# andrei-ace/EdgeStyle

Hardware: AMD Instinct MI355X
Metric: 512x512 try-on images/sec @ 50 DDIM steps (6-cond ControlNet) (higher is better)
Workload: dtype f16; 1 GPU; BASELINE configs[1]: full 6-cond edgestyle_multicontrolnet + controllora, 512x512, 50 DDIM steps, CFG 7.5, batch=1/GPU, hipGraph-captured step, cond embedding + VAE decode included; images_per_gpu=1, ddim_steps=50, parallelism=dp1 (independent images, one RCCL gather)

## Files before the change

### edgestyle_amd/csrc/builder.hip

```cpp
#include <hip/hip_runtime.h>
#include <math.h>
#include <stdio.h>
#include <stdlib.h>
#include <string.h>

#include <algorithm>
#include <deque>
#include <functional>
#include <map>
#include <memory>
#include <stdexcept>
#include <string>
#include <thread>
#include <unordered_map>
#include <vector>

#include "../../include/edgestyle_hip.h"
#include "plan.h"

extern "C" void es_set_error(const char* msg);
extern "C" int es_plan_set_dry(int on);

namespace {

// ... 175 lines not shown
  ~Blk() { if (heap) heap->release(off, bytes); }
};

struct T {
  unsigned long long p = 0;
  int n = 0, h = 0, w = 0, c = 0;
  long long ld = 0;
  int es = 2;
  std::shared_ptr<Blk> b;
  unsigned long long lo = 0;
  std::shared_ptr<Blk> lo_b;
  unsigned long long gnp = 0;
  std::shared_ptr<Blk> gnp_b;
  int gnp_groups = 0;
  explicit operator bool() const { return p != 0; }
  long long hw() const { return (long long)h * w; }
  long long numel() const { return (long long)n * h * w * c; }
  bool contig() const { return ld == c; }
  long long bstride() const { return hw() * ld; }
  size_t bytes() const { return (size_t)numel() * es; }
  T batch(int a, int cnt = -1) const {
    T t = *this;
    t.p += (unsigned long long)a * (unsigned long long)bstride() * es;
    if (t.lo) t.lo += (unsigned long long)a * (unsigned long long)bstride() * es;
    t.gnp = 0; t.gnp_b.reset(); t.gnp_groups = 0;
    t.n = cnt < 0 ? n - a : cnt;
    if (a < 0 || t.n < 0 || a + t.n > n) fail("builder: batch slice out of range");
    return t;
  }
  T chan(int c0, int cn) const {
    T t = *this;
    if (c0 < 0 || c0 + cn > c) fail("builder: channel slice out of range");
    t.p += (unsigned long long)c0 * es;
    t.lo = 0; t.lo_b.reset();
    t.gnp = 0; t.gnp_b.reset(); t.gnp_groups = 0;
    t.c = cn;
    return t;
  }
  T view(int n2, int h2, int w2, int c2) const {
    if (!contig() || (long long)n2 * h2 * w2 * c2 != numel()) fail("builder: view of a non-contiguous or differently sized tensor");
    T t = *this;
    t.n = n2; t.h = h2; t.w = w2; t.c = c2; t.ld = c2;
    return t;
  }
  void* ptr() const { return (void*)p; }
};

struct PW {
  unsigned long long w = 0, bias = 0, ln_colsum = 0;
  int cout = 0, cin = 0, ksize = 1, bn = 128, rows_padded = 0, kpad = 0, ctail = 0, korder = 0;
  bool geglu = false;
  float ln_eps = 1e-5f;
  const uint16_t* host_w = nullptr;
  long long w_numel() const { return (long long)rows_padded * kpad; }
};
using PWs = std::vector<const PW*>;
struct Norm { unsigned long long g = 0, b = 0; };

struct CA {
  int stride = 1, pad = -1;
  bool upsample = false;
  T x2, temb, residual, out, out_scale_dev;
  long long temb_stride = 0;
  int act = ES_ACT_NONE;
  float out_scale = 1.f;
  int out_h = 0, out_w = 0;
  std::vector<int> group_n;
  std::vector<T> tails;
  int x_rep = 1;
  bool wide = false;
  int gn_groups = 0;
};

#pragma clang fp contract(off)
constexpr double PLAN_T160 = 1.25, PLAN_ALONE = 0.9, PLAN_TFIX = 2.0, PLAN_RED_FIX = 12.0, PLAN_SLAB_BYTES_PER_UNIT = 4.0e6;
constexpr double PLAN_T320 = 2.3, PLAN_T320_FIX = 3.0;
constexpr double PLAN_T256 = 2.6, PLAN_T256_FIX = 6.0, PLAN_T256_GEGLU = 7.0, PLAN_LN_TK = 1.55, PLAN_T256_MARGIN = 0.93;
constexpr int PLAN_BIG_MIN_M = 2048, PLAN_BIG_MIN_NK = 16;
constexpr double PLAN_T64_ALONE = 0.5, PLAN_T64 = 0.16, PLAN_T64_LONG = 1.5;
constexpr int PLAN_SMALL_MAX_M = 16384, PLAN_MIN_SLICE = 12, PLAN_NK_NOSPLIT = 10, PLAN_RESIDENT = 512;

double plan_env(const char* name, double dflt) { const char* e = getenv(name); return e && *e ? atof(e) : dflt; }
bool plan_gemm(long long M, int rows_padded, int kpad, bool geglu, const int* bns, int nb, bool allow_split, int* o_bn, int* o_sk, int* o_st) {
  static const double PLAN_T320 = plan_env("ES_PLAN_T320", ::PLAN_T320), PLAN_T256_MARGIN = plan_env("ES_PLAN_T256_MARGIN", ::PLAN_T256_MARGIN);
  static const int PLAN_BIG_MIN_NK = (int)plan_env("ES_PLAN_BIG_MIN_NK", ::PLAN_BIG_MIN_NK);
  int others[8], no = 0;
  bool has256 = false;
  for (int bi = 0; bi < nb; ++bi) { if (bns[bi] == 256) has256 = true; else if (no < 8) others[no++] = bns[bi]; }
  if (has256) {
    const int nk = kpad / BK;
    int obn = 0, osk = 1, ost = 2;
    const bool have_other = no > 0 && plan_gemm(M, rows_padded, kpad, geglu, others, no, allow_split, &obn, &osk, &ost);
    if (rows_padded % 256) { if (!have_other) return false; *o_bn = obn; *o_sk = osk; *o_st = ost; return true; }
    const long long t256 = ((M + 255) / 256) * (rows_padded / 256);
    const double c256 = (double)((t256 + 255) / 256) * ((double)nk * PLAN_T256 + PLAN_T256_FIX + (geglu ? PLAN_T256_GEGLU : 0.0));
    bool take = !have_other;
    if (have_other && M >= PLAN_BIG_MIN_M && nk >= PLAN_BIG_MIN_NK && osk == 1 && obn != 64) {
      const long long to = ((M + BM - 1) / BM) * (rows_padded / obn);
      const double co = (double)((to + PLAN_RESIDENT - 1) / PLAN_RESIDENT) * ((double)nk * PLAN_LN_TK * (obn == 160 ? PLAN_T160 : 1.0) + PLAN_T256_FIX);
      take = c256 < PLAN_T256_MARGIN * co;
    }
    if (take) { *o_bn = 256; *o_sk = 1; *o_st = 2; } else { *o_bn = obn; *o_sk = osk; *o_st = ost; }
    return true;
  }
  if (geglu) { *o_bn = 128; *o_sk = 1; *o_st = 2; return true; }
  const int nk = kpad / BK;
  bool have = false;
  double bt = 0; int bbn = 0, bsk = 0; long long bwgs = 0;
  for (int bi = 0; bi < nb; ++bi) {
    const int bn = bns[bi];
    if (rows_padded % bn) continue;
    if (bn == 320 && (M < PLAN_BIG_MIN_M || nk < PLAN_BIG_MIN_NK) && nb > 1) continue;
    if (bn == 64 && M > PLAN_SMALL_MAX_M && nb > 1) continue;
    const int bm = bn == 320 ? 256 : (bn == 64 ? 64 : BM);
    const int resident = bn == 320 ? PLAN_RESIDENT / 2 : (bn == 64 ? 2 * PLAN_RESIDENT : PLAN_RESIDENT);
    const long long tiles = ((M + bm - 1) / bm) * (rows_padded / bn);
    int last = 1;
    if (allow_split && tiles < resident / 2 && nk > PLAN_NK_NOSPLIT) last = std::max(1, std::min(nk / PLAN_MIN_SLICE, 32));
    for (int sk = 1; sk <= last; ++sk) {
      const long long wgs = tiles * sk;
      double tk;
      if (bn == 320) tk = PLAN_T320;
      else if (bn == 64) {
        if (sk > 1 && wgs > PLAN_RESIDENT) continue;
        const double w = (double)wgs / (double)(PLAN_RESIDENT / 2);
        const double ex = std::max(0.0, w - 1.0);
        tk = (PLAN_T64_ALONE + PLAN_T64 * (ex * ex)) * (nk <= 40 ? 1.0 : PLAN_T64_LONG);
      } else tk = (bn == 160 ? PLAN_T160 : 1.0) * (wgs <= PLAN_RESIDENT / 2 ? PLAN_ALONE : 1.0);
      const double rounds = bn == 320 ? std::max((double)wgs / 256.0, 0.9) : (double)((wgs + resident - 1) / resident);
      double t = rounds * (((double)nk / (double)sk) * tk + (bn == 320 ? PLAN_T320_FIX : PLAN_TFIX));
      if (sk > 1) t += PLAN_RED_FIX + (double)sk * (double)M * (double)rows_padded * 8.0 / PLAN_SLAB_BYTES_PER_UNIT;
      if (!have || t < bt) { have = true; bt = t; bbn = bn; bsk = sk; bwgs = wgs; }
    }
  }
  if (!have) return false;
  *o_bn = bbn; *o_sk = bsk;
  if (bbn == 64) *o_st = (bwgs <= PLAN_RESIDENT && nk / bsk >= 6) ? 4 : 2;
  else *o_st = (bbn != 320 && bwgs <= PLAN_RESIDENT / 2 && nk / bsk >= 6) ? 4 : 2;
  return true;
}

constexpr int XS_TARGET_WGS = 256, XS_MIN_M = 8192;
bool xs_shape_fits(int ksize, int kpad, int cin, int ctail, int cout, bool geglu) {
  if (ksize != 1 || (kpad != 320 && kpad != 640) || cin != kpad || ctail) return false;
  const int ch = kpad == 320 ? 64 : 32;
  const int line = ch * (128 / (geglu ? ch : 2 * ch));
  return !(cout % line || cout < 4 * line);
}
bool xs_shape_ok(long long M, int ksize, int kpad, int cin, int ctail, int cout, bool geglu) {
  if (!xs_shape_fits(ksize, kpad, cin, ctail, cout, geglu)) return false;
  if (M < XS_MIN_M || (M < 4 * XS_MIN_M && cout < (kpad == 320 ? 960 : 1920))) return false;
  return true;
}
bool gn_fold_on() { static const bool on = [] { const char* e = getenv("ES_GN_FOLD"); return !e || std::string(e) == "1"; }(); return on; }
int choose_bn(int cout) { return (cout % 160 == 0 && cout % 128 != 0) ? 160 : 128; }
bool big_tile_256() { static const bool on = [] { const char* e = getenv("ES_BIG_TILE_256"); return !e || e[0] != '0'; }(); return on; }

struct Builder {
  Heap heap;
  unsigned long long ws_bytes = 0;
  int dt = ES_F16;
  std::vector<std::pair<unsigned long long, std::vector<char>>> uploads;
  std::deque<PW> pws;
  std::map<std::string, const PW*> pack_cache;
  std::map<const void*, unsigned long long> vec_cache;
  std::map<std::pair<int, int>, unsigned long long> gn_partials, fusion_scratch;
  std::map<int, unsigned long long> zero_bias;

  T empty(int n, int h, int w, int c, int es = 2) {
    T t; t.n = n; t.h = h; t.w = w; t.c = c; t.ld = c; t.es = es;
    auto blk = std::make_shared<Blk>();
    blk->heap = &heap; blk->bytes = std::max<size_t>(t.bytes(), 1); blk->off = heap.alloc(blk->bytes);
    t.b = blk; t.p = FAKE_HEAP + blk->off;
    return t;
  }
  unsigned long long persistent(size_t bytes) { return FAKE_HEAP + heap.alloc(std::max<size_t>(bytes, 1)); }
  T persistent_t(int n, int h, int w, int c, int es = 2) {
    T t; t.n = n; t.h = h; t.w = w; t.c = c; t.ld = c; t.es = es;
    t.p = persistent(t.bytes());
    return t;
  }
  char* staged(unsigned long long addr, size_t bytes) {
    uploads.emplace_back(addr, std::vector<char>(bytes, 0));
    return uploads.back().second.data();
  }
  unsigned long long upload_f32(const std::vector<float>& v) {
    const unsigned long long a = persistent(v.size() * 4);
    memcpy(staged(a, v.size() * 4), v.data(), v.size() * 4);
    return a;
  }
  unsigned long long workspace(unsigned long long bytes) { ws_bytes = std::max(ws_bytes, bytes); return FAKE_WS; }
// ... 60 lines not shown
    }
    return &p;
  }
  const PW* pack_ln(const std::vector<float>& w, int rows, int C, const std::vector<float>* bias, const std::vector<float>& gamma, const std::vector<float>& beta,
                    float eps, bool geglu) {
    std::vector<float> wg((size_t)rows * C), fb((size_t)rows);
    parallel_for(rows, [&](long long a, long long b) {
      for (long long r = a; r < b; ++r) {
        double acc = 0.0;
        for (int j = 0; j < C; ++j) { wg[r * C + j] = w[r * C + j] * gamma[j]; acc += (double)w[r * C + j] * (double)beta[j]; }
        if (bias) acc += (double)(*bias)[r];
        fb[r] = (float)acc;
      }
    });
    PW* p = const_cast<PW*>(pack(wg, rows, C, 1, &fb, geglu));
    const uint16_t* pk = p->host_w;
    std::vector<float> cs((size_t)p->rows_padded);
    for (int r = 0; r < p->rows_padded; ++r) {
      double acc = 0.0;
      for (int j = 0; j < p->kpad; ++j) acc += (double)dec(pk[(size_t)r * p->kpad + j]);
      cs[r] = (float)acc;
    }
    p->ln_colsum = upload_f32(cs);
    p->ln_eps = eps;
    return p;
  }
  unsigned long long norm_vec(const Weights& W, const std::string& key, long long n) {
    const es_tensor* id = nullptr;
    std::vector<float> v = W.vec(key, n, &id);
    auto it = vec_cache.find(id->data);
    if (it != vec_cache.end()) return it->second;
    return vec_cache[id->data] = upload_f32(v);
  }
  Norm norm(const Weights& W, const std::string& p, long long n) { return {norm_vec(W, p + ".weight", n), norm_vec(W, p + ".bias", n)}; }

  const PW* conv(const Weights& W, const std::string& p, int cin_pad = 0, bool geglu = false, int cout_pad = 0) {
    const es_tensor* wt = W.get(p + ".weight");
    if (wt->ndim != 2 && wt->ndim != 4) fail("es_load_weights: '" + p + ".weight' is neither a Linear nor a Conv2d weight");
    const int cout = (int)wt->shape[0], cin = (int)wt->shape[1], k = wt->ndim == 4 ? (int)wt->shape[2] : 1;
    if (wt->ndim == 4 && (wt->shape[3] != k || (k != 1 && k != 3))) fail("es_load_weights: '" + p + ".weight': only 1x1 and 3x3 kernels");
    const es_tensor* bt = W.find(p + ".bias");
    std::string key;
    if (!W.lora(p)) {
      char buf[128];
      snprintf(buf, sizeof(buf), "%p|%p|%d|%d|%d", wt->data, bt ? bt->data : nullptr, (int)geglu, cin_pad, cout_pad);
      key = buf;
      auto it = pack_cache.find(key);
      if (it != pack_cache.end()) return it->second;
    }
    std::vector<float> w = W.matrix(p), b;
    if (bt) b = W.vec(p + ".bias", cout);
    const PW* pw = pack(w, cout, cin, k, bt ? &b : nullptr, geglu, cin_pad, cout_pad);
    if (!key.empty()) pack_cache[key] = pw;
    return pw;
  }
  void stack(const Weights& W, const std::vector<std::string>& ps, bool bias, std::vector<float>& w, std::vector<float>& b, int& rows, int& cols) {
    rows = 0; cols = -1;
    for (const auto& p : ps) {
      const es_tensor* t = W.get(p + ".weight");
      if (t->ndim != 2 || (cols >= 0 && t->shape[1] != cols)) fail("es_load_weights: '" + p + ".weight' does not stack with its neighbours");
      cols = (int)t->shape[1];
      std::vector<float> m = W.matrix(p);
      w.insert(w.end(), m.begin(), m.end());
      if (bias) { std::vector<float> v = W.vec(p + ".bias", t->shape[0]); b.insert(b.end(), v.begin(), v.end()); }
      rows += (int)t->shape[0];
    }
  }
  const PW* cat(const Weights& W, const std::vector<std::string>& ps, bool bias) {
    std::vector<float> w, b; int rows, cols;
    stack(W, ps, bias, w, b, rows, cols);
    return pack(w, rows, cols, 1, bias ? &b : nullptr);
  }
  const PW* cat_ln(const Weights& W, const std::vector<std::string>& ps, bool bias, const std::string& ln, bool geglu = false) {
    std::vector<float> w, b; int rows, cols;
    stack(W, ps, bias, w, b, rows, cols);
    return pack_ln(w, rows, cols, bias ? &b : nullptr, W.vec(ln + ".weight", cols), W.vec(ln + ".bias", cols), 1e-5f, geglu);
  }
  const PW* conv_tail(const Weights& W, const std::string& p, const std::string& pt) {
    const es_tensor* wt = W.get(p + ".weight");
    const es_tensor* tt = W.get(pt + ".weight");
    char buf[96];
    snprintf(buf, sizeof(buf), "%p|%p|tail", wt->data, tt->data);
    auto it = pack_cache.find(buf);
    if (it != pack_cache.end()) return it->second;
    const int cout = (int)wt->shape[0], cin = (int)wt->shape[1], k = (int)wt->shape[2], ct = (int)tt->shape[1];
    if (wt->ndim != 4 || cin % BK || ct % BK || tt->shape[0] != cout) fail("es_load_weights: conv2 + conv_shortcut fold needs 64-aligned channels ('" + p + "')");
    std::vector<float> w = W.matrix(p), tw = W.matrix(pt), b = W.vec(p + ".bias", cout), b2 = W.vec(pt + ".bias", cout);
    for (int i = 0; i < cout; ++i) b[i] = b[i] + b2[i];
    const PW* pw = pack(w, cout, cin, k, &b, false, 0, 0, &tw, ct);
    pack_cache[buf] = pw;
    return pw;
  }

  static void ok(int rc, const char* what) { if (rc) fail(std::string(what) + ": " + es_last_error()); }

  struct GnFront { unsigned long long part = 0; std::vector<Norm> nl; int groups = 0, nchunk = 0, hw = 0; float eps = 0.f; };
  T linear_xs(const T& x, const PWs& pl, long long M, const T& out, const std::vector<long long>& group_rows, const T& residual = T(),
              const GnFront* gn = nullptr) {
    const PW* pw = pl[0];
    const int K = pw->kpad, ch = K == 320 ? 64 : 32;
    const int pline = 128 / (pw->geglu ? ch : 2 * ch);
    const int total = pw->cout / ch, lines = total / pline;
    const long long rbs = (M + 255) / 256;
    const int want = (int)std::max<long long>(1, std::min<long long>(lines, XS_TARGET_WGS / rbs));
    const int lps = cdiv(lines, want), nslices = cdiv(lines, lps);
    es_xs_desc d;
// ... 32 lines not shown

  T conv_gemm(const T& x, const PWs& pl, const CA& a = CA()) {
    const PW* pw = pl[0];
    const bool grouped = pl.size() > 1;
    int N = x.n;
    const int H = x.h, Wd = x.w, C1 = x.c, nsrc = x.n;
    if (!x.contig()) fail("conv_gemm: the source must be contiguous");
    if (a.x_rep > 1) { if (a.x2 || !a.tails.empty()) fail("conv_gemm: x_rep needs a single source"); N *= a.x_rep; }
    const int C2 = a.x2 ? a.x2.c : 0;
    if (C1 + C2 != pw->cin) fail("conv_gemm: input channels " + std::to_string(C1) + "+" + std::to_string(C2) + " != packed " + std::to_string(pw->cin));
    int tsum = 0;
    for (const auto& t : a.tails) tsum += t.c;
    if (tsum != pw->ctail || a.tails.size() > 2) fail("conv_gemm: tail channels do not match the packed weights");
    const int k = pw->ksize, pad = a.pad < 0 ? (k == 3 ? 1 : 0) : a.pad;
    const int Hin = a.upsample ? H * 2 : H, Win = a.upsample ? Wd * 2 : Wd;
    const int Hout = a.out_h ? a.out_h : (Hin + 2 * pad - k) / a.stride + 1, Wout = a.out_w ? a.out_w : (Win + 2 * pad - k) / a.stride + 1;
    const int act_i = pw->geglu ? ES_ACT_GEGLU : a.act;
    const int cstore = pw->geglu ? pw->cout / 2 : pw->cout;
    T out = a.out ? a.out : empty(N, Hout, Wout, cstore);
    if (out.numel() != (long long)N * Hout * Wout * cstore || !out.contig()) fail("conv_gemm: output buffer of another size");
    const long long M = (long long)N * Hout * Wout, hw = (long long)Hout * Wout;
    static const bool xs_residual = [] { const char* e = getenv("ES_XS_RESIDUAL"); return !e || std::string(e) == "1"; }();
    const bool xs_res = !a.residual || (xs_residual && pw->kpad == 320 && !pw->geglu && !pw->ln_colsum && a.residual.contig() &&
                                        a.residual.numel() == (long long)N * Hout * Wout * cstore && !(a.wide && wide_stream()));
    const bool plain = k == 1 && a.stride == 1 && !a.upsample && !a.x2 && !a.temb && xs_res && a.tails.empty() && a.x_rep == 1 &&
                       a.act == ES_ACT_NONE && a.out_scale == 1.f && !a.out_scale_dev;
    if (plain && xs_shape_ok(M, pw->ksize, pw->kpad, pw->cin, pw->ctail, pw->cout, pw->geglu)) {
      bool e = true;
      if (grouped) {
        if (pl.size() > 4) e = false;
        for (int n : a.group_n) if ((n * hw) % 256) e = false;
        for (const PW* q : pl) if ((q->ln_colsum == 0) != (pw->ln_colsum == 0)) e = false;
      }
      if (e) {
        std::vector<long long> rows;
        for (int n : a.group_n) rows.push_back(n * hw);
        T xo = out;
        linear_xs(x, grouped ? pl : PWs{pw}, M, xo, rows, a.residual);
        return out;
      }
    }
    bool big_ok = C1 % BK == 0 && C2 % BK == 0 && !pw->geglu && !pw->ln_colsum;
    if (big_ok && grouped) for (int n : a.group_n) if ((n * hw) % 256) big_ok = false;
    bool ln256_ok = big_tile_256() && (pw->geglu || pw->ln_colsum) && k == 1 && a.stride == 1 && !a.upsample && !a.x2 && a.tails.empty() && !a.temb &&
                    a.x_rep == 1 && C1 % BK == 0 && pw->rows_padded % 256 == 0 && pw->cout % 8 == 0 && !(pw->geglu && a.residual) && !a.wide && a.gn_groups == 0;
    if (ln256_ok && grouped) for (int n : a.group_n) if ((n * hw) % 256) ln256_ok = false;
    const bool small_ok = C1 % BK == 0 && C2 % BK == 0 && !pw->geglu;
    int cand[5], nc = 0;
    if (ln256_ok) cand[nc++] = 256;
    if (big_ok) cand[nc++] = 320;
    cand[nc++] = 160; cand[nc++] = 128;
    if (small_ok) cand[nc++] = 64;
    int bn, splitk, stages;
    if (!plan_gemm(M, pw->rows_padded, pw->kpad, pw->geglu, cand, nc, pw->ln_colsum == 0, &bn, &splitk, &stages)) fail("plan_gemm: rows_padded fits no N tile");
    if (bn == 320 && splitk == 1 && !es_conv_gemm8p_form_ok(act_i, pw->cout, a.temb ? 1 : 0, hw, a.residual ? 1 : 0)) {
      if (!plan_gemm(M, pw->rows_padded, pw->kpad, pw->geglu, cand + 1, nc - 1, pw->ln_colsum == 0, &bn, &splitk, &stages)) fail("plan_gemm: rows_padded fits no N tile");
    }
    es_gemm_desc d;
    memset(&d, 0, sizeof(d));
    d.x = x.ptr(); d.x2 = a.x2 ? a.x2.ptr() : nullptr; d.w = (const void*)pw->w; d.bias = (const float*)pw->bias;
    d.temb = a.temb ? a.temb.ptr() : nullptr; d.residual = a.residual ? a.residual.ptr() : nullptr;
    d.out_scale_dev = a.out_scale_dev ? (const float*)a.out_scale_dev.ptr() : nullptr; d.out = out.ptr();
    d.N = N; d.Hsrc = H; d.Wsrc = Wd; d.C1 = C1; d.C2 = C2; d.Hout = Hout; d.Wout = Wout; d.Cout = pw->cout;
    d.rows_padded = pw->rows_padded; d.Kpad = pw->kpad; d.ksize = k; d.stride = a.stride; d.pad = pad; d.upsample = a.upsample;
    d.temb_stride = a.temb ? (int)a.temb_stride : 0;
    d.act = act_i; d.splitk = splitk; d.bn = bn; d.dtype = dt; d.out_scale = a.out_scale; d.stages = stages;
    const long long src_numel = x.numel() * a.x_rep + (a.x2 ? a.x2.numel() : 0);
    d.xcd_m_fastest = (!grouped && splitk == 1 && M <= 2048 && pw->w_numel() > src_numel) ? 1 : 0;
    d.x_nmod = a.x_rep > 1 ? nsrc : 0;
    d.korder = pw->korder;
    if (a.gn_groups > 0 && gn_handover(hw, cstore, a.gn_groups) && !pw->geglu && !pw->ln_colsum && pw->cout / a.gn_groups <= (bn == 320 ? 160 : bn)) {
      T part = empty(N, (int)(2 * (hw / 64)), 1, a.gn_groups * 2, 4);
      d.gn_part = (float*)part.ptr(); d.gn_groups = a.gn_groups;
      out.gnp = part.p; out.gnp_b = part.b; out.gnp_groups = a.gn_groups;
    }
    if (a.wide && a.residual && wide_stream() && cstore % 8 == 0 && !pw->geglu) {
      if (a.residual.lo) d.residual_lo = (const void*)a.residual.lo;
      T lo = empty(N, Hout, Wout, cstore);
      d.out_lo = lo.ptr();
      out.lo = lo.p; out.lo_b = lo.b;
    }
    if (k == 1 && M <= 65536 && C1 % BK == 0 && C2 % BK == 0 && bn != 64 && bn != 320 && bn != 256 && !(stages == 4 && bn != 128) && stages != 3) d.waves = 8;
    if (splitk > 1) d.workspace = (float*)workspace((unsigned long long)splitk * M * pw->rows_padded * 4);
    if (pw->ln_colsum) {
      for (const PW* q : pl) if (!q->ln_colsum) fail("LayerNorm-folded weights need a plain linear launch (all groups folded)");
      if (a.x2 || k != 1) fail("LayerNorm-folded weights need a plain linear launch");
      d.ln_colsum = (const float*)pw->ln_colsum; d.ln_eps = pw->ln_eps;
    }
    if (!a.tails.empty()) {
      for (const auto& t : a.tails) if (t.n != N || t.h != Hout || t.w != Wout || !t.contig()) fail("conv_gemm: tail sources must be contiguous [N,Hout,Wout,C]");
      d.t1 = a.tails[0].ptr(); d.Ct1 = a.tails[0].c;
      if (a.tails.size() == 2) { d.t2 = a.tails[1].ptr(); d.Ct2 = a.tails[1].c; }
    }
    if (grouped) {
      const int gran = bn == 320 ? 256 : BM;
      int sum = 0;
      for (int n : a.group_n) { sum += n; if ((n * hw) % gran) fail("grouped conv_gemm: groups must cover N in whole tiles"); }
      if (pl.size() > 4 || a.group_n.size() != pl.size() || sum != N) fail("grouped conv_gemm: bad group table");
      d.ngroups = (int)pl.size();
      long long acc = 0;
      for (size_t g = 0; g < pl.size(); ++g) {
        const PW* q = pl[g];
        if (q->rows_padded != pw->rows_padded || q->kpad != pw->kpad || q->cout != pw->cout || q->cin != pw->cin || q->ksize != pw->ksize ||
            q->geglu != pw->geglu || q->ctail != pw->ctail || q->korder != pw->korder) fail("grouped conv_gemm: weight geometry differs between groups");
        acc += a.group_n[g] * hw / BM;
        d.mt_end[g] = (int)acc; d.w_g[g] = (const void*)q->w; d.bias_g[g] = (const float*)q->bias; d.ln_colsum_g[g] = (const float*)q->ln_colsum;
// ... 223 lines not shown
    conv_in = B.conv(W, "conv_in", in_pad);
    t1 = B.conv(W, "time_embedding.linear_1"); t2 = B.conv(W, "time_embedding.linear_2");
    std::vector<std::string> names;
    for (int i = 0; i < c.nb; ++i) for (int j = 0; j < c.lpb; ++j) names.push_back("down_blocks." + std::to_string(i) + ".resnets." + std::to_string(j));
    names.push_back("mid_block.resnets.0"); names.push_back("mid_block.resnets.1");
    names.insert(names.end(), extra_resnets.begin(), extra_resnets.end());
    int o = 0;
    std::vector<std::string> tp;
    for (const auto& nm : names) { temb_offs[nm] = o; o += (int)W.shaped(nm + ".time_emb_proj.weight", {-1, 4 * c.ch[0]})->shape[0]; tp.push_back(nm + ".time_emb_proj"); }
    tproj = B.cat(W, tp, true);
    for (int i = 0; i < c.nb; ++i) {
      down.emplace_back();
      for (int j = 0; j < c.lpb; ++j) {
        const std::string r = "down_blocks." + std::to_string(i) + ".resnets." + std::to_string(j);
        int ti = -1;
        Resnet rs(B, W, r, c.groups, c.eps, temb_offs[r]);
        if (c.has_attn[i]) { tr.emplace_back(B, W, "down_blocks." + std::to_string(i) + ".attentions." + std::to_string(j), c.heads, c.groups); ti = (int)tr.size() - 1; }
        down.back().emplace_back(rs, ti);
      }
      downsample.push_back(i != c.nb - 1 ? B.conv(W, "down_blocks." + std::to_string(i) + ".downsamplers.0.conv") : nullptr);
    }
    mid0 = Resnet(B, W, "mid_block.resnets.0", c.groups, c.eps, temb_offs["mid_block.resnets.0"]);
    tr.emplace_back(B, W, "mid_block.attentions.0", c.heads, c.groups); mid_attn = (int)tr.size() - 1;
    mid1 = Resnet(B, W, "mid_block.resnets.1", c.groups, c.eps, temb_offs["mid_block.resnets.1"]);
    n_enc_tr = (int)tr.size();
  }
  int tproj_width() const { return tproj->cout; }
  T time_proj(Builder& B, const T& t, int n) const {
    T e = B.timestep_embedding(t, n, cfg.ch[0]);
    CA s; s.act = ES_ACT_SILU;
    e = B.linear(e, t1, s);
    e = B.linear(e, t2, s);
    return B.linear(e, tproj);
  }
};

struct UNet : Encoder {
  std::vector<std::vector<std::pair<Resnet, int>>> up;
  std::vector<const PW*> upsample;
  Norm norm_out; const PW* conv_out;
  void init(Builder& B, const Weights& W, const UCfg& c) {
    std::vector<std::string> extra;
    for (int i = 0; i < c.nb; ++i) for (int j = 0; j < c.lpb + 1; ++j) extra.push_back("up_blocks." + std::to_string(i) + ".resnets." + std::to_string(j));
    Encoder::init(B, W, c, extra);
    for (int i = 0; i < c.nb; ++i) {
      up.emplace_back();
      for (int j = 0; j < c.lpb + 1; ++j) {
        const std::string r = "up_blocks." + std::to_string(i) + ".resnets." + std::to_string(j);
        int ti = -1;
        Resnet rs(B, W, r, c.groups, c.eps, temb_offs[r]);
        if (c.has_attn[c.nb - 1 - i]) { tr.emplace_back(B, W, "up_blocks." + std::to_string(i) + ".attentions." + std::to_string(j), c.heads, c.groups); ti = (int)tr.size() - 1; }
        up.back().emplace_back(rs, ti);
      }
      upsample.push_back(i != c.nb - 1 ? B.conv(W, "up_blocks." + std::to_string(i) + ".upsamplers.0.conv") : nullptr);
    }
    W.shaped("conv_out.weight", {c.out_ch, c.ch[0], 3, 3});
    norm_out = B.norm(W, "conv_norm_out", c.ch[0]);
    conv_out = B.conv(W, "conv_out");
  }
};

struct ControlNet : Encoder {
  std::vector<const PW*> zero; const PW* zero_mid = nullptr;
  std::vector<const PW*> cond;
  bool uses_vae = false;
  void init(Builder& B, const Weights& W, const UCfg& c, bool uses_vae_) {
    Encoder::init(B, W, c, {});
    uses_vae = uses_vae_;
    std::vector<int> rc{c.ch[0]};
    for (int i = 0; i < c.nb; ++i) { for (int j = 0; j < c.lpb; ++j) rc.push_back(c.ch[i]); if (i != c.nb - 1) rc.push_back(c.ch[i]); }
    for (size_t i = 0; i < rc.size(); ++i) {
      W.shaped("controlnet_down_blocks." + std::to_string(i) + ".weight", {rc[i], rc[i], 1, 1});
      zero.push_back(B.conv(W, "controlnet_down_blocks." + std::to_string(i)));
    }
    W.shaped("controlnet_mid_block.weight", {c.ch[c.nb - 1], c.ch[c.nb - 1], 1, 1});
    zero_mid = B.conv(W, "controlnet_mid_block");
    if (!uses_vae) {
      const std::string p = "controlnet_cond_embedding";
      W.shaped(p + ".conv_in.weight", {c.ce[0], c.cond_ch, 3, 3});
      W.shaped(p + ".conv_out.weight", {c.ch[0], c.ce[c.nce - 1], 3, 3});
      cond.push_back(B.conv(W, p + ".conv_in", 8));
      for (int i = 0; i < 2 * (c.nce - 1); ++i) cond.push_back(B.conv(W, p + ".blocks." + std::to_string(i)));
      cond.push_back(B.conv(W, p + ".conv_out"));
    }
  }
  T embed_cond(Builder& B, const T& img) const {
    CA s; s.act = ES_ACT_SILU;
    T h = B.conv_gemm(img, cond[0], s);
    for (size_t i = 1; i + 1 < cond.size(); ++i) { CA a; a.act = ES_ACT_SILU; a.stride = ((i - 1) % 2 == 1) ? 2 : 1; h = B.conv_gemm(h, cond[i], a); }
    return B.conv_gemm(h, cond.back());
  }
};

struct FusionParams { unsigned long long w1, b1, g1, be1, w2, b2, g2, be2, w3, b3; int c, s; };

struct VAE {
  VCfg cfg; int lat_pad = 8;
  struct Mid { Resnet r0, r1; Norm gn; const PW *qkv, *o; };
  const PW *e_in, *e_out, *quant, *post_quant_scaled, *d_in, *d_out;
  std::vector<std::pair<std::vector<Resnet>, const PW*>> e_down, d_up;
  Mid e_mid, d_mid; Norm e_norm, d_norm;
  Mid mid(Builder& B, const Weights& W, const std::string& side) {
    const std::string a = side + ".mid_block.attentions.0";
    const int c = cfg.ch[cfg.nb - 1];
    Mid m;
    m.r0 = Resnet(B, W, side + ".mid_block.resnets.0", cfg.groups, cfg.eps, -1);
    m.gn = B.norm(W, a + ".group_norm", c);
    m.qkv = B.cat(W, {a + ".to_q", a + ".to_k", a + ".to_v"}, true);
    m.o = B.conv(W, a + ".to_out.0");
    m.r1 = Resnet(B, W, side + ".mid_block.resnets.1", cfg.groups, cfg.eps, -1);
    return m;
  }
  void init(Builder& B, const Weights& W, const VCfg& c) {
    cfg = c;
    lat_pad = round_up(c.latent, 8);
    const int n = c.nb;
    W.shaped("encoder.conv_in.weight", {c.ch[0], 3, 3, 3}); W.shaped("encoder.conv_out.weight", {2 * c.latent, c.ch[n - 1], 3, 3});
    W.shaped("quant_conv.weight", {2 * c.latent, 2 * c.latent, 1, 1}); W.shaped("post_quant_conv.weight", {c.latent, c.latent, 1, 1});
    W.shaped("decoder.conv_in.weight", {c.ch[n - 1], c.latent, 3, 3}); W.shaped("decoder.conv_out.weight", {3, c.ch[0], 3, 3});
    for (const char* side : {"encoder", "decoder"})
      for (const char* q : {".to_q", ".to_k", ".to_v", ".to_out.0"}) W.shaped(std::string(side) + ".mid_block.attentions.0" + q + ".weight", {c.ch[n - 1], c.ch[n - 1]});
    e_in = B.conv(W, "encoder.conv_in", 8);
    for (int i = 0; i < n; ++i) {
      std::vector<Resnet> rs;
      for (int j = 0; j < c.lpb; ++j) rs.emplace_back(B, W, "encoder.down_blocks." + std::to_string(i) + ".resnets." + std::to_string(j), c.groups, c.eps, -1);
      e_down.emplace_back(rs, i != n - 1 ? B.conv(W, "encoder.down_blocks." + std::to_string(i) + ".downsamplers.0.conv") : nullptr);
    }
    e_mid = mid(B, W, "encoder");
    e_norm = B.norm(W, "encoder.conv_norm_out", c.ch[n - 1]);
    e_out = B.conv(W, "encoder.conv_out");
    quant = B.conv(W, "quant_conv");
    {
      const es_tensor* wt = W.get("post_quant_conv.weight");
      std::vector<float> w = W.matrix("post_quant_conv"), b;
      for (auto& v : w) v = (float)((double)v / (double)c.scaling);
      const bool hb = W.has("post_quant_conv.bias");
      if (hb) b = W.vec("post_quant_conv.bias", wt->shape[0]);
      post_quant_scaled = B.pack(w, (int)wt->shape[0], (int)wt->shape[1], 1, hb ? &b : nullptr, false, lat_pad, 8);
    }
    d_in = B.conv(W, "decoder.conv_in", 8);
    d_mid = mid(B, W, "decoder");
    for (int i = 0; i < n; ++i) {
      std::vector<Resnet> rs;
      for (int j = 0; j < c.lpb + 1; ++j) rs.emplace_back(B, W, "decoder.up_blocks." + std::to_string(i) + ".resnets." + std::to_string(j), c.groups, c.eps, -1);
      d_up.emplace_back(rs, i != n - 1 ? B.conv(W, "decoder.up_blocks." + std::to_string(i) + ".upsamplers.0.conv") : nullptr);
    }
    d_norm = B.norm(W, "decoder.conv_norm_out", c.ch[0]);
    d_out = B.conv(W, "decoder.conv_out");
  }
  T run_mid(Builder& B, const Mid& m, T h) const {
    h = m.r0.run(B, h, T());
    const int N = h.n, H = h.h, Wd = h.w, C = h.c;
    T n = B.group_norm(h, m.gn, cfg.groups, cfg.eps, false).view(N, H * Wd, 1, C);
    T qkv = B.linear(n, m.qkv);
    T a = B.attention(qkv.chan(0, C), qkv.chan(C, C), qkv.chan(2 * C, C), 1);
    CA r; r.residual = h.view(N, H * Wd, 1, C);
    h = B.linear(a, m.o, r).view(N, H, Wd, C);
    return m.r1.run(B, h, T());
  }
  T encode_moments(Builder& B, const T& img) const {
    T h = B.conv_gemm(img, e_in);
    for (const auto& blk : e_down) {
      for (const auto& r : blk.first) h = r.run(B, h, T());
      if (blk.second) { CA a; a.stride = 2; a.pad = 0; a.out_h = h.h / 2; a.out_w = h.w / 2; h = B.conv_gemm(h, blk.second, a); }
    }
    h = run_mid(B, e_mid, h);
    h = B.group_norm(h, e_norm, cfg.groups, cfg.eps, true);
    h = B.conv_gemm(h, e_out);
    return B.conv_gemm(h, quant);
  }
  T decode(Builder& B, const T& z) const {
    T h = B.conv_gemm(z, post_quant_scaled);
    h = B.conv_gemm(h, d_in);
    h = run_mid(B, d_mid, h);
    for (const auto& blk : d_up) {
      for (const auto& r : blk.first) h = r.run(B, h, T());
      if (blk.second) { CA a; a.upsample = true; h = B.conv_gemm(h, blk.second, a); }
    }
    h = B.group_norm(h, d_norm, cfg.groups, cfg.eps, true);
    return B.conv_gemm(h, d_out);
  }
};

struct Model {
  Builder B;
  UCfg ucfg; VCfg vcfg;
  es_ctx_geometry geo;
  Dict d_unet, d_vae, d_fusion, d_cn[6];
  UNet unet;
  VAE vae;
  std::vector<std::unique_ptr<ControlNet>> nets;
  std::vector<int> net_of_cond;
  std::vector<std::pair<int, std::vector<int>>> groups;
  std::vector<FusionParams> fusion;
  std::vector<std::pair<int, int>> table;
  std::vector<const Encoder*> encs; std::vector<int> counts; int ntot = 0, width = 0, ncn = 0;
  int B_ = 1, N = 2, T_ = 50, h = 64, w = 64, nn = 6, kmax = 3;
  T latents, model_in, noise, ehs, step_idx, t_rows, scales_cur, t_table, scale_table, coef, ts_dev, image;
  std::vector<T> conds, cond_img, cond_noise, gbufs, hist;
  std::vector<T> ctx_grouped, ctx_unet; std::vector<std::vector<T>> ctx_nets;
  T cond_cat, tproj_table, tproj_cur, tproj_gen;
  std::vector<T> fused_zero, fz_zero, fz_u;
  bool guess = false;
  int Bc = 2;
  std::vector<std::vector<T>> ctx_guess;

  std::vector<Norm> norms(const std::vector<const Resnet*>& rs, int which) const { std::vector<Norm> v; for (auto r : rs) v.push_back(which == 1 ? r->n1 : r->n2); return v; }

  T g_resnet(const std::vector<const Resnet*>& rs, const T& x, const T& tproj) {
    const Resnet* r0 = rs[0];
    T hh = B.group_norm(x, norms(rs, 1), r0->groups, r0->eps, true, T(), counts);
    PWs c1, c2, c2s, sh; bool all_s = true;
    for (auto r : rs) { c1.push_back(r->conv1); c2.push_back(r->conv2); c2s.push_back(r->conv2s); sh.push_back(r->shortc); if (!r->conv2s) all_s = false; }
    CA a; a.temb = tproj.chan(r0->temb_off, tproj.c - r0->temb_off); a.temb_stride = tproj.ld; a.group_n = counts; a.gn_groups = r0->groups;
    hh = B.conv_gemm(hh, c1, a);
    hh = B.group_norm(hh, norms(rs, 2), r0->groups, r0->eps, true, T(), counts);
    if (all_s) { CA t; t.tails.push_back(x); t.group_n = counts; t.gn_groups = r0->groups; return B.conv_gemm(hh, c2s, t); }
    for (auto r : rs) if (r->conv2s) fail("builder: grouped resnets must fold conv_shortcut all alike");
    T xs = x;
    if (r0->shortc) { CA s; s.group_n = counts; xs = B.conv_gemm(x, sh, s); }
    CA r; r.residual = xs; r.group_n = counts; r.wide = true; r.gn_groups = r0->groups;
    return B.conv_gemm(hh, c2, r);
  }
  T g_transformer(const std::vector<const Transformer*>& ts, const T& x, const T& kv) {
    const Transformer* t0 = ts[0];
    const int Nn = x.n, H = x.h, Wd = x.w, C = x.c;
    std::vector<int> rows;
    for (int n : counts) rows.push_back(n * H * Wd);
    std::vector<Norm> nl; PWs pin, qkv, o1, q2, o2, ff1, ffo;
    for (auto t : ts) { nl.push_back(t->norm); pin.push_back(t->proj_in); qkv.push_back(t->qkv_ln); o1.push_back(t->o1); q2.push_back(t->q2_ln); o2.push_back(t->o2); ff1.push_back(t->ff1_ln); ffo.push_back(t->ffo); }
// ... 121 lines not shown
    const int c0 = unet.conv_in->cout;
    T h0 = B.empty(ntot, x.h, x.w, c0);
    {
      PWs ci; for (auto e : encs) ci.push_back(e->conv_in);
      CA a; a.residual = cond_cat; a.group_n = counts; a.out = h0; a.x_rep = ntot / N; a.wide = true; a.gn_groups = ucfg.groups;
      h0 = B.conv_gemm(x, ci, a);
    }
    T tproj;
    if (table_driven) {
      B.gather_row(tproj_table, T_, step_idx, tproj_cur, (int)((long long)ntot * width * 2 / 4));
      tproj = tproj_cur;
    } else tproj = time_proj_generic();
    std::vector<T> skips; T mid;
    g_run(h0, tproj, skips, mid);
    h0 = T();
    std::vector<T> srcs = skips; srcs.push_back(mid);
    std::vector<T> enc;
    for (const auto& s : srcs) enc.push_back(s.batch(ncn));
    std::vector<T> fused;
    if (nn == 1) {
      const ControlNet* cn = (const ControlNet*)encs[0];
      for (size_t lvl = 0; lvl < srcs.size(); ++lvl) {
        CA a; a.residual = enc[lvl]; a.out_scale = 1.f; a.out_scale_dev = scales_cur.chan(0, 1);
        fused.push_back(B.conv_gemm(srcs[lvl].batch(0, ncn), lvl + 1 < srcs.size() ? cn->zero[lvl] : cn->zero_mid, a));
      }
    } else {
    std::vector<int> cn_counts(counts.begin(), counts.end() - 1);
    std::vector<T> res;
    for (size_t lvl = 0; lvl < srcs.size(); ++lvl) {
      PWs z; for (size_t e = 0; e + 1 < encs.size(); ++e) { const ControlNet* cn = (const ControlNet*)encs[e]; z.push_back(lvl + 1 < srcs.size() ? cn->zero[lvl] : cn->zero_mid); }
      CA a; a.group_n = cn_counts;
      res.push_back(B.conv_gemm(srcs[lvl].batch(0, ncn), z, a));
    }
    std::vector<int> first(nn, 0);
    { int a = 0; for (const auto& g : groups) for (int p : g.second) { first[p] = a; a += N; } }
    std::vector<std::vector<T>> rpn(nn);
    for (int i = 0; i < nn; ++i) for (size_t k = 0; k < srcs.size(); ++k) rpn[i].push_back(res[k].batch(first[i]));
    fused = fuse(rpn, N, &enc);
    }
    srcs.clear(); skips.clear(); enc.clear(); mid = T();
    unet_decoder(fused, tproj.batch(ncn));
  }
  void unet_decoder(std::vector<T>& fused, const T& tp) {
    T hh = fused.back();
    fused.pop_back();
    int ci = unet.n_enc_tr;
    for (size_t i = 0; i < unet.up.size(); ++i) {
      for (const auto& ra : unet.up[i]) {
        T skip = fused.back();
        fused.pop_back();
        hh = ra.first.run(B, hh, tp, skip);
        if (ra.second >= 0) { hh = transformer(unet.tr[ra.second], hh, ctx_unet[ci]); ++ci; }
      }
      if (unet.upsample[i]) { CA a; a.upsample = true; hh = B.conv_gemm(hh, unet.upsample[i], a); }
    }
    hh = B.group_norm(hh, unet.norm_out, ucfg.groups, ucfg.eps, true);
    CA o; o.out = noise;
    B.conv_gemm(hh, unet.conv_out, o);
  }
  void enc_run(const Encoder& e, T hh, const T& tp, const std::vector<T>& ctx, std::vector<T>& skips, T& mid) {
    skips.push_back(hh);
    int ci = 0;
    for (size_t i = 0; i < e.down.size(); ++i) {
      for (size_t j = 0; j < e.down[i].size(); ++j) {
        hh = e.down[i][j].first.run(B, hh, tp);
        if (e.down[i][j].second >= 0) { hh = transformer(e.tr[e.down[i][j].second], hh, ctx[ci]); ++ci; }
        skips.push_back(hh);
      }
      if (e.downsample[i]) { CA a; a.stride = 2; a.gn_groups = ucfg.groups; hh = B.conv_gemm(hh, e.downsample[i], a); skips.push_back(hh); }
    }
    hh = e.mid0.run(B, hh, tp);
    hh = transformer(e.tr[e.mid_attn], hh, ctx[ci]);
    mid = e.mid1.run(B, hh, tp);
  }
  void set_context_guess() {
    for (size_t ti = 0; ti < unet.tr.size(); ++ti) unet.tr[ti].context(B, ehs, ctx_unet[ti], 1);
    const T ehs_c = ehs.batch(N - Bc);
    size_t gi = 0;
    for (const auto& g : groups) {
      const ControlNet& net = *nets[g.first];
      for (int ti = 0; ti < net.n_enc_tr; ++ti) net.tr[ti].context(B, ehs_c, ctx_guess[gi][ti], (int)g.second.size());
      ++gi;
    }
  }
  static std::vector<float> guess_level_scales(int n) {
    std::vector<float> ls((size_t)n);
    const double step = (0.0 - (-1.0)) / (double)(n - 1);
    for (int i = 0; i < n; ++i) ls[i] = (float)(i < n / 2 ? pow(10.0, -1.0 + step * (double)i) : pow(10.0, 0.0 - step * (double)(n - i - 1)));
    return ls;
  }
  void step_guess() {
    const T& x = model_in;
    const int Bh = N - Bc;
    const T xc = x.batch(Bh);
    const std::vector<float> ls = guess_level_scales((int)table.size());
    std::vector<std::vector<T>> rpn(nn);
    size_t gi = 0;
    for (const auto& g : groups) {
      const ControlNet& cn = *nets[g.first];
      const int k = (int)g.second.size();
      T tp = cn.time_proj(B, t_rows, k * Bc);
      const int c0 = cn.conv_in->cout;
      T h0 = B.empty(k * Bc, x.h, x.w, c0);
      for (int i = 0; i < k; ++i) { CA a; a.residual = conds[g.second[i]]; a.out = h0.batch(i * Bc, Bc); B.conv_gemm(xc, cn.conv_in, a); }
      std::vector<T> skips; T mid;
      enc_run(cn, h0, tp, ctx_guess[gi], skips, mid);
      std::vector<T> res;
// ... 66 lines not shown
          B.memcpy_t(conds[i], B.conv_gemm(z, net.conv_in));
        }
      } else {
        T emb = nets[g.net]->embed_cond(B, x8);
        for (size_t k = 0; k < g.idx.size(); ++k) {
          const int i = g.idx[k];
          T e = emb.batch((int)k * B_, B_);
          B.memcpy_t(conds[i].batch(0, B_), e);
          if (rep > 1) B.memcpy_t(conds[i].batch(B_, B_), e);
        }
      }
    }
  }

  void pack_fusion(const Weights& W) {
    for (size_t i = 0; i < table.size(); ++i) {
      const std::string p = i + 1 < table.size() ? "multi_controlnet_down_blocks." + std::to_string(i) : "multi_controlnet_mid_block";
      const int c = table[i].first, s = table[i].second, hw = s * s;
      FusionParams f; f.c = c; f.s = s;
      f.w1 = B.upload_f32(to_f32(W.shaped(p + ".first_conv.weight", {3 * c, 2, 1, 1})));
      f.b1 = B.upload_f32(to_f32(W.shaped(p + ".first_conv.bias", {3 * c})));
      f.w2 = B.upload_f32(to_f32(W.shaped(p + ".second_conv.weight", {c, 3, 1, 1})));
      f.b2 = B.upload_f32(to_f32(W.shaped(p + ".second_conv.bias", {c})));
      f.w3 = B.upload_f32(to_f32(W.shaped(p + ".third_conv.weight", {c, 1, 1, 1})));
      f.b3 = B.upload_f32(to_f32(W.shaped(p + ".third_conv.bias", {c})));
      auto plane = [&](const std::string& key, int per) {
        const std::vector<float> t = to_f32(W.shaped(key, {(long long)per * c, s, s}));
        const unsigned long long a = B.persistent((size_t)hw * c * per * 2);
        uint16_t* d = (uint16_t*)B.staged(a, (size_t)hw * c * per * 2);
        parallel_for(hw, [&](long long x0, long long x1) {
          for (long long px = x0; px < x1; ++px)
            for (int cc = 0; cc < c * per; ++cc) d[(size_t)px * c * per + cc] = B.enc(t[(size_t)cc * hw + px]);
        });
        return a;
      };
      f.g1 = plane(p + ".first_normalization.weight", 3); f.be1 = plane(p + ".first_normalization.bias", 3);
      f.g2 = plane(p + ".second_normalization.weight", 1); f.be2 = plane(p + ".second_normalization.bias", 1);
      fusion.push_back(f);
    }
  }
};

struct Recording {
  es_plan* p;
  explicit Recording(es_plan* pl) : p(pl) { if (es_plan_begin_record(p)) fail(std::string("es_load_weights: ") + es_last_error()); es_plan_set_dry(1); }
  ~Recording() { es_plan_set_dry(0); es_plan_end_record(p); }
};

}

extern "C" int es_plan_gemm_choice(long long M, int rows_padded, int kpad, int geglu, const int* bns, int n_bns, int allow_split, int* bn, int* splitk, int* stages) {
  if (!bns || n_bns < 1 || !bn || !splitk || !stages) { es_set_error("es_plan_gemm_choice: null argument"); return -1; }
  if (!plan_gemm(M, rows_padded, kpad, geglu != 0, bns, n_bns, allow_split != 0, bn, splitk, stages)) { es_set_error("es_plan_gemm_choice: rows_padded fits no N tile"); return -1; }
  return 0;
}
extern "C" int es_linear_xs_eligible(long long M, int ksize, int kpad, int cin, int ctail, int cout, int geglu) {
  return xs_shape_ok(M, ksize, kpad, cin, ctail, cout, geglu != 0) ? 1 : 0;
}

extern "C" int es_load_weights(const es_weights* wts, const es_model_config* mc, const es_ctx_geometry* g, int device, es_ctx** out) {
  if (!wts || !mc || !g || !out) { es_set_error("es_load_weights: null argument"); return -1; }
  es_ctx* ctx = nullptr;
  es_plan* plans[ES_PLAN_COUNT] = {};
  void* arena = nullptr;
  try {
    auto m = std::make_unique<Model>();
    Model& M = *m;
    Builder& B = M.B;
    if (mc->n_blocks < 2 || mc->n_blocks > 4 || mc->vae_n_blocks < 2 || mc->vae_n_blocks > 4) fail("es_load_weights: 2..4 resolution levels");
    if (g->n_conds != 6 && g->n_conds != 1) fail("es_load_weights: n_conds is 6 (the reference's fused multi-ControlNet model, MC:66-114) or 1 (a single ControlNet, PL:338-351)");
    if (g->n_conds == 1 && wts->n_controlnets != 1) fail("es_load_weights: a single-ControlNet context takes exactly one ControlNet");
    if (g->dtype != ES_F16 && g->dtype != ES_BF16) fail("es_load_weights: dtype must be ES_F16 or ES_BF16");
    if (g->B < 1 || g->h < 1 || g->w < 1 || g->n_steps < 1) fail("es_load_weights: bad geometry");
    if (wts->n_controlnets < 1 || wts->n_controlnets > 6) fail("es_load_weights: 1..6 distinct ControlNets");
    UCfg& u = M.ucfg;
    u.in_ch = mc->in_channels; u.out_ch = mc->out_channels; u.nb = mc->n_blocks; u.lpb = mc->layers_per_block; u.heads = mc->num_heads;
    u.cross = mc->cross_attention_dim; u.groups = mc->norm_num_groups; u.eps = mc->norm_eps; u.nce = mc->n_cond_embed; u.cond_ch = mc->conditioning_channels;
    for (int i = 0; i < 4; ++i) { u.ch[i] = mc->block_out_channels[i]; u.has_attn[i] = mc->down_has_attn[i]; u.ce[i] = mc->cond_embed_channels[i]; }
    VCfg& v = M.vcfg;
    v.nb = mc->vae_n_blocks; v.lpb = mc->vae_layers_per_block; v.latent = mc->vae_latent_channels; v.groups = mc->vae_norm_num_groups;
    v.eps = mc->vae_norm_eps; v.scaling = mc->vae_scaling_factor;
    for (int i = 0; i < 4; ++i) v.ch[i] = mc->vae_block_out_channels[i];
    if (u.in_ch != v.latent) fail("es_load_weights: the UNet's in_channels must equal the VAE's latent_channels");
    if (u.cond_ch != 3 || u.nce < 2 || u.nce > 4) fail("es_load_weights: conditioning embedding of 3 input channels, 2..4 widths");
    M.geo = *g;
    B.dt = g->dtype;
    M.B_ = g->B; M.N = g->cfg ? 2 * g->B : g->B; M.T_ = g->n_steps; M.h = g->h; M.w = g->w; M.nn = g->n_conds;
    M.guess = g->guess_mode != 0;
    M.Bc = M.guess ? g->B : M.N;
    const int N = M.N, TS = M.T_, h = g->h, w = g->w, Bn = g->B, NN = g->n_conds, Nc = M.Bc;
    if (!M.guess) {
      int cnt[6] = {};
      for (int p = 0; p < NN; ++p) {
        const int ni = wts->net_of_cond[p];
        if (ni < 0 || ni >= wts->n_controlnets) fail("es_load_weights: net_of_cond names a ControlNet that was not given");
        ++cnt[ni];
      }
      const int hw_min = (h >> (u.nb - 1)) * (w >> (u.nb - 1));
      for (int i = 0; i <= wts->n_controlnets; ++i) {
        const long long n = (i < wts->n_controlnets ? (long long)cnt[i] : 1) * N;
        if (n && (n * hw_min) % BM) fail("es_load_weights: the groups of the lockstep pass do not tile in 128-pixel units at this latent size (the Python host falls back to serial chains; this builder does not)");
      }
    }
    M.d_unet.init(wts->unet, "UNet"); M.d_vae.init(wts->vae, "VAE"); M.d_fusion.init(wts->fusion, "fusion");
    for (int i = 0; i < wts->n_controlnets; ++i) M.d_cn[i].init(wts->controlnet[i], ("ControlNet " + std::to_string(i)).c_str());
    Weights Wu; Wu.own = &M.d_unet; Wu.who = "UNet";
// ... 203 lines not shown
```

### edgestyle_amd/csrc/gemm_conv.hip

```cpp
#ifndef ES_WT_STORES
#define ES_WT_STORES 1
#endif
#include "common.h"
#include "../../include/edgestyle_hip.h"
#include "plan.h"

#ifndef ES_W_AUX
#define ES_W_AUX 0
#endif

int es_conv_gemm8p_launch(const es_gemm_desc& d, hipStream_t st);
bool es_conv_gemm8p_takes(const es_gemm_desc& d);

unsigned long long es_operand_limit_v = 0x7FFFFFFFull;

namespace {

constexpr int BK = 64;

#ifndef ES_ABLATE
#define ES_ABLATE 0
#endif
#ifndef ES_STAMPS
#define ES_STAMPS 0
#endif

typedef __attribute__((address_space(3))) void* lptr_t;

template <typename T>
ES_DEVICE void store_elems(T* o, const float* v, int n) {
  for (int r = 0; r < n; ++r) o[r] = from_f32<T>(v[r]);
}

template <int XI>
ES_DEVICE void row_offsets_fn(unsigned (&voff)[XI], const int (&iy0)[XI], const int (&ix0)[XI], const int (&nb)[XI],
                              const int tp, const int cs, const int chan, const int ksize, const int KK, const int pad,
                              const int Hin, const int Win, const int upsample, const int Wsrc) {
  int ky = 0, kx = 0;
  if (ksize == 3) { ky = (tp * 11) >> 5; kx = tp - ky * 3; }
  if (tp >= KK) { ky = pad; kx = pad; }
#pragma unroll
  for (int i = 0; i < XI; ++i) {
    const int iy = iy0[i] + ky, ix = ix0[i] + kx;
    const bool ok = (unsigned)iy < (unsigned)Hin && (unsigned)ix < (unsigned)Win;
    const int pix = nb[i] + (iy >> upsample) * Wsrc + (ix >> upsample);
    voff[i] = ok ? (unsigned)(((size_t)pix * cs + chan) * 2) : 0xFFFFFF00u;
  }
}

template <typename T, int BM, int BN, bool ALIGNED, int STAGES, int FM = 4 ,
          bool LN = false ,
          bool KO = false >
__global__ __launch_bounds__(BM * 8 / FM, (STAGES == 2 && BM == 128) ? (FM == 2 ? 4 : 2) : 1) void conv_gemm_kernel(
    const es_gemm_desc p, const int M, const int nk, const void* const tail1, const void* const tail2, const int tailC1,
    const int tailC2) {
  constexpr int BKT = BK;
  constexpr int RB = BKT * 2;
  constexpr int CPR = BKT / 8;
  constexpr int RPP = 1024 / RB;
  constexpr int WM = BM / (16 * FM);
  constexpr int NW = WM * 2;
  constexpr int NT = NW * 64;
  constexpr int XI = (BM / RPP) / NW;
  constexpr int FN = BN / 32;
  constexpr int WP = BN / RPP;
  constexpr int WI = (WP + NW - 1) / NW;
  constexpr int XT = BM * RB;
  constexpr int WT = BN * RB;
  static_assert((size_t)BM * (BN * 2 + 16) <= (size_t)STAGES * (BM + BN) * RB, "the epilogue tile must fit the stage ring");
  static_assert(LN || (size_t)BM * (BN * 2 + 16) + (size_t)(BM / 8 + BM / 64) * BN * 8 <= (size_t)STAGES * (BM + BN) * RB,
                "the GroupNorm-statistics scratch (gn_emit_partials) must fit behind the epilogue tile");
  constexpr int BNP = BN;
  constexpr int EROW = BNP * 2 + 16;
  constexpr int NI = XI + WI;
  extern __shared__ __attribute__((aligned(16))) char smem[];

  const int tid = threadIdx.x;
  const int lane = tid & 63;
  const int wave = __builtin_amdgcn_readfirstlane(tid >> 6);
  const int wm = wave % WM, wn = wave / WM;
  int tile_m, tile_n, z;
  {
    const int tm = (M + BM - 1) / BM, tn = p.rows_padded / BN;
    const int nwg = gridDim.x, b = blockIdx.x;
    const int q = nwg >> 3, r = nwg & 7, xcd = b & 7;
    const int w = (xcd < r ? xcd * (q + 1) : r * (q + 1) + (xcd - r) * q) + (b >> 3);
    const float inv_tm = __builtin_amdgcn_rcpf((float)tm), inv_tn = __builtin_amdgcn_rcpf((float)tn);
    if (p.xcd_m_fastest) { const int t = fast_div(w, tm, inv_tm); tile_m = w - t * tm; z = fast_div(t, tn, inv_tn); tile_n = t - z * tn; }
    else                 { const int t = fast_div(w, tn, inv_tn); tile_n = w - t * tn; z = fast_div(t, tm, inv_tm); tile_m = t - z * tm; }
  }
#if ES_STAMPS
  const int sblk = blockIdx.x == 40 ? 0 : (blockIdx.x == 333 ? 1 : -1);
  auto stamp = [&](int ks, int what) __attribute__((always_inline)) {
    if (p.prof && sblk >= 0 && lane == 0 && wave < 4 && ks >= 8 && ks < 16)
      p.prof[((sblk * 4 + wave) * 8 + (ks - 8)) * 4 + what] = __builtin_amdgcn_s_memtime();
  };
  auto pstamp = [&](int what) __attribute__((always_inline)) {
    if (p.prof && tid == 0 && (blockIdx.x == 0 || blockIdx.x == gridDim.x - 1))
      p.prof[256 + (blockIdx.x == 0 ? 0 : 1) * 8 + what] = __builtin_amdgcn_s_memtime();
  };
  pstamp(0);
#else
  if (p.prof && tid == 0) atomicMin(p.prof, (unsigned long long)__builtin_amdgcn_s_memrealtime());
#endif

  int ks0 = 0, ks1 = nk;
  if (p.splitk > 1) {
    const float inv_sk = __builtin_amdgcn_rcpf((float)p.splitk);
    ks0 = fast_div(nk * z, p.splitk, inv_sk);
    ks1 = fast_div(nk * (z + 1), p.splitk, inv_sk);
  }

  const int lrow = lane / CPR;
  const int lslot = lane % CPR;
  const int kc = lslot ^ (lrow & 7);
  const int Ctot = p.C1 + p.C2;
  const int KK = p.ksize * p.ksize;
  const int pC1 = p.C1, pC2 = p.C2, pCt1 = tailC1, pCt2 = tailC2;
  const bool has_tail = tail1 != nullptr;
  const int Ctail = has_tail ? pCt1 + pCt2 : 0;
  const int Ktrue = KK * Ctot + Ctail;
  const int Hin = p.Hsrc << p.upsample, Win = p.Wsrc << p.upsample;
  const int HWout = p.Hout * p.Wout;

  constexpr unsigned OOB = 0xFFFFFF00u;
  int iy0[XI], ix0[XI], nb[XI];
  const bool small_m = M < (1 << 24);
  const float inv_hw = __builtin_amdgcn_rcpf((float)HWout), inv_w = __builtin_amdgcn_rcpf((float)p.Wout);
#pragma unroll
  for (int i = 0; i < XI; ++i) {
    const int m = tile_m * BM + RPP * (wave * XI + i) + lrow;
    iy0[i] = -(1 << 20); ix0[i] = -(1 << 20); nb[i] = 0;
    if (m < M) {
      int n, oy, ox;
      if (HWout == 1) {
        n = m; oy = 0; ox = 0;
      } else if (small_m) {
        n = fast_div(m, HWout, inv_hw);
        const int rem = m - n * HWout;
        oy = fast_div(rem, p.Wout, inv_w);
        ox = rem - oy * p.Wout;
      } else {
        n = m / HWout;
        const int rem = m - n * HWout;
        oy = rem / p.Wout; ox = rem - oy * p.Wout;
      }
      iy0[i] = oy * p.stride - p.pad;
      ix0[i] = ox * p.stride - p.pad;
      if (p.x_nmod) n -= (n / p.x_nmod) * p.x_nmod;
      nb[i] = n * p.Hsrc * p.Wsrc;
    }
  }
  int pix0[KO ? XI : 1];
  unsigned tmask[KO ? XI : 1];
  if constexpr (KO) {
#pragma unroll
    for (int i = 0; i < XI; ++i) {
      const int ay = iy0[i], ax = ix0[i];
      unsigned vy = 0, vx = 0;
#pragma unroll
      for (int k = 0; k < 3; ++k) {
        vy |= ((unsigned)(ay + k) < (unsigned)Hin ? 1u : 0u) << k;
        vx |= ((unsigned)(ax + k) < (unsigned)Win ? 1u : 0u) << k;
      }
      unsigned mk = ((vy & 1) ? vx : 0u) | ((vy & 2) ? vx << 3 : 0u) | ((vy & 4) ? vx << 6 : 0u);
      mk |= ay > -(1 << 19) ? 1u << 9 : 0u;
      mk |= (unsigned)(ay & p.upsample) << 10 | (unsigned)(ax & p.upsample) << 11;
      tmask[i] = mk;
      pix0[i] = nb[i] + (ay >> p.upsample) * p.Wsrc + (ax >> p.upsample);
    }
  }
  int grp = 0;
  if (p.ngroups > 1) {
    const int t128 = (tile_m * BM) / 128;
    grp = (t128 >= p.mt_end[0]) + (t128 >= p.mt_end[1]) + (t128 >= p.mt_end[2]);
  }
  const void* wsel = p.ngroups > 1 ? p.w_g[grp] : p.w;
  const float* bsel = p.ngroups > 1 ? p.bias_g[grp] : p.bias;
  const float* lnsel = LN ? (p.ngroups > 1 ? p.ln_colsum_g[grp] : p.ln_colsum) : nullptr;
  const auto rW = __builtin_amdgcn_make_buffer_rsrc(
      (void*)wsel, (short)0, (int)((size_t)p.rows_padded * p.Kpad * 2), 0x00020000);
  const int Nsrc = p.x_nmod ? p.x_nmod : p.N;
  const auto rX1 = __builtin_amdgcn_make_buffer_rsrc(
      (void*)p.x, (short)0, (int)((size_t)Nsrc * p.Hsrc * p.Wsrc * p.C1 * 2), 0x00020000);
  const void* const pt1 = tail1 ? tail1 : p.x;
  const void* const pt2 = tail2 ? tail2 : p.x;
  const void* const px = p.x;
  const void* const px2 = p.x2 ? p.x2 : p.x;
  const int nX1 = (int)((size_t)Nsrc * p.Hsrc * p.Wsrc * pC1 * 2);
  const int nX2 = (int)((size_t)Nsrc * p.Hsrc * p.Wsrc * (p.x2 ? pC2 : pC1) * 2);
  const int nT1 = has_tail ? (int)((size_t)p.N * p.Hout * p.Wout * pCt1 * 2) : 0;
  const int nT2 = tail2 ? (int)((size_t)p.N * p.Hout * p.Wout * pCt2 * 2) : 0;
  unsigned woff[WI];
#pragma unroll
  for (int i = 0; i < WI; ++i) {
    const int piece = wave * WI + i;
    woff[i] = piece < WP ? (unsigned)(((size_t)(tile_n * BN + RPP * piece + lrow) * p.Kpad + kc * 8) * 2) : OOB;
  }

  int tap, cpos;
  {
    const int kg = ks0 * BKT + (ALIGNED ? 0 : kc * 8);
    tap = kg == 0 ? 0 : fast_div(kg, Ctot, __builtin_amdgcn_rcpf((float)Ctot));
    cpos = kg - tap * Ctot;
    if (ALIGNED && tap >= KK) { tap = KK; cpos = kg - KK * Ctot; }
    if constexpr (KO) {
      const int kt = (KK * Ctot) / BKT;
      if (ks0 >= kt) { tap = KK; cpos = (ks0 - kt) * BKT; }
      else { const int ch = fast_div(ks0, 9, 1.0f / 9.0f); tap = ks0 - ch * 9; cpos = ch * BKT; }
    }
  }
  unsigned voff[XI];
#pragma unroll
  for (int i = 0; i < XI; ++i) voff[i] = OOB;
  const void* xbase = p.x;
  int xrec = 0, soff_x = 0, seg_left = 0;
  const int ks_tail = (KK * Ctot) / BKT;
  const int pk_ksize = p.ksize, pk_pad = p.pad, pk_up = p.upsample, pk_wsrc = p.Wsrc;
#define row_offsets(tp, cs, chan) \
  row_offsets_fn<XI>(voff, iy0, ix0, nb, (tp), (cs), (chan), pk_ksize, KK, pk_pad, Hin, Win, pk_up, pk_wsrc)
  auto issue_tile = [&](int ks, int stage) __attribute__((always_inline)) {
    char* xs = smem + stage * (XT + WT);
    char* ws = xs + XT;
    const int soff_w = ks * RB;
#pragma unroll
    for (int i = 0; i < WI; ++i)
      if (!(ES_ABLATE & 32) && wave * WI + i < WP)
        __builtin_amdgcn_raw_ptr_buffer_load_lds(rW, (lptr_t)(ws + (wave * WI + i) * 1024), 16,
                                                 (ES_ABLATE & 64) ? (int)OOB : (int)woff[i], soff_w, 0, ES_W_AUX);
    if constexpr ((ES_ABLATE & 16) != 0) {
    } else if constexpr (ALIGNED) {
      bool fast = false;
      if constexpr (!KO) fast = seg_left > 0;
      if (fast) {
        soff_x += 128; --seg_left;
      } else {
      const bool tail = KO ? ks >= ks_tail : tap >= KK;
      int q0 = pC1, q1 = pC2, q2 = pCt1, q3 = pCt2;
      asm("" : "+s"(q0), "+s"(q1), "+s"(q2), "+s"(q3));
      const int c1 = tail ? q2 : q0;
      const int second = cpos >= c1 ? 1 : 0;
      const int cs = second ? (tail ? q3 : q1) : c1;
      const int cc = second ? cpos - c1 : cpos;
      if constexpr (KO) {
        int ky = (tap * 11) >> 5, kx = tap - ky * 3;
        if (tail) { ky = pk_pad; kx = pk_pad; }
        const unsigned tb = 1u << tap, cs2 = (unsigned)cs * 2u;
        const int dsc = ky * pk_wsrc + kx;
#pragma unroll
        for (int i = 0; i < XI; ++i) {
          int pix = pix0[i] + dsc;
          if (pk_up) pix = pix0[i] + ((int)(((tmask[i] >> 10) & 1) + ky) >> 1) * pk_wsrc + ((int)(((tmask[i] >> 11) & 1) + kx) >> 1);
          voff[i] = (tmask[i] & tb) ? __umul24((unsigned)pix, cs2) + (unsigned)(kc * 16) : 0xFFFFFF00u;
        }
      } else {
        row_offsets(tap, cs, kc * 8);
      }
#if ES_ABLATE & 64
#pragma unroll
      for (int i = 0; i < XI; ++i) voff[i] = OOB;
#endif
      const void *b0 = px, *b1 = px2, *b2 = pt1, *b3 = pt2;
      int n0 = nX1, n1 = nX2, n2 = nT1, n3 = nT2;
      asm("" : "+s"(b0), "+s"(b1), "+s"(b2), "+s"(b3), "+s"(n0), "+s"(n1), "+s"(n2), "+s"(n3));
      xbase = tail ? (second ? b3 : b2) : (second ? b1 : b0);
      xrec = tail ? (second ? n3 : n2) : (second ? n1 : n0);
      soff_x = cc * 2;
      if constexpr (KO) {
        if (tap < KK) {
          if (++tap == KK) { cpos += BKT; if (cpos >= Ctot) cpos = 0; else tap = 0; }
        } else {
// ... 263 lines not shown
          if constexpr (FN % 2 == 0) {
#pragma unroll
            for (int i = 0; i < FN; i += 2) {
              typename Traits<T>::vec4 pk;
#pragma unroll
              for (int r = 0; r < 4; ++r) {
                float ah = acc[i][j][r], ag = acc[i + 1][j][r];
                if constexpr (LN) {
                  ah = ln_rstd * (ah - ln_mean * lncs[i][r]);
                  ag = ln_rstd * (ag - ln_mean * lncs[i + 1][r]);
                }
                const float hv = ah + bias[i][r], gv = ag + bias[i + 1][r];
                pk[r] = from_f32<T>(hv * gelu_f(gv) * scale);
              }
              *(typename Traits<T>::vec4*)(et + (prow + j * 16) * EROW + ((wn * (BN / 2) + i * 16) / 2 + fq * 4) * 2) = pk;
            }
          }
        } else {
#pragma unroll
          for (int i = 0; i < FN; ++i) {
            const int c = tile_n * BN + pcol + i * 16;
            float tv[4] = {0.f, 0.f, 0.f, 0.f};
            if (p.temb && c < p.Cout) {
              const T* tp = (const T*)p.temb + (size_t)n * p.temb_stride + c;
              if (c + 3 < p.Cout) {
                const auto t4 = *(const typename Traits<T>::vec4*)tp;
#pragma unroll
                for (int r = 0; r < 4; ++r) tv[r] = to_f32(t4[r]);
              } else {
                for (int r = 0; r < 4 && c + r < p.Cout; ++r) tv[r] = to_f32(tp[r]);
              }
            }
            typename Traits<T>::vec4 pk;
#pragma unroll
            for (int r = 0; r < 4; ++r) {
              float a = acc[i][j][r];
              if constexpr (LN) a = ln_rstd * (a - ln_mean * lncs[i][r]);
              float x = a + bias[i][r] + tv[r];
              if (p.act == ES_ACT_SILU) x = silu_f(x);
              pk[r] = from_f32<T>(x * scale);
            }
            *(typename Traits<T>::vec4*)(et + (prow + j * 16) * EROW + (pcol + i * 16) * 2) = pk;
          }
        }
      }
    }
    __syncthreads();

    const int BNo = geglu ? BN / 2 : BNP;
    const int c_tile = tile_n * (geglu ? BN / 2 : BN);
    if (vec_store) {
      const int CH = BNo / 8;
      const float inv_ch = __builtin_amdgcn_rcpf((float)CH);
      auto store_rows = [&](auto mode_c) __attribute__((always_inline)) {
        constexpr int MODE = decltype(mode_c)::value;
#pragma unroll
        for (int k = 0; k < RPF; ++k) {
          const int idx = tid + k * NT;
          const int row = fast_div(idx, CH, inv_ch), ch = idx - row * CH;
          const int m = tile_m * BM + row, c = c_tile + ch * 8;
          if (idx < BM * CH && m < M && c < Cstore) {
            auto v = as_vec8<T>(*(const u32x4*)(et + row * EROW + ch * 16));
            const size_t o = (size_t)m * Cstore + c;
            if constexpr (MODE >= 2) {
              const auto rv = as_vec8<T>(rpre[k]);
              typename Traits<T>::vec8 lv, lo;
              if constexpr (MODE == 3) lv = as_vec8<T>(*(const u32x4*)((const T*)p.residual_lo + o));
#pragma unroll
              for (int e = 0; e < 8; ++e) {
                float sum = to_f32(v[e]) + to_f32(rv[e]);
                if constexpr (MODE == 3) sum += to_f32(lv[e]);
                v[e] = from_f32<T>(sum);
                lo[e] = from_f32<T>(sum - to_f32(v[e]));
              }
              store16((T*)p.out_lo + o, __builtin_bit_cast(u32x4, lo));
            } else if constexpr (MODE == 1) {
              const auto rv = as_vec8<T>(rpre[k]);
#pragma unroll
              for (int e = 0; e < 8; ++e) v[e] = from_f32<T>(to_f32(v[e]) + to_f32(rv[e]));
            }
            store16(outp + o, __builtin_bit_cast(u32x4, v));
            if (p.gn_part) *(u32x4*)(et + row * EROW + ch * 16) = __builtin_bit_cast(u32x4, v);
          }
        }
      };
      if (p.out_lo) { if (p.residual_lo) store_rows(std::integral_constant<int, 3>{}); else store_rows(std::integral_constant<int, 2>{}); }
      else if (resp) store_rows(std::integral_constant<int, 1>{});
      else store_rows(std::integral_constant<int, 0>{});
      if (p.gn_part) {
        __syncthreads();
        gn_emit_partials<T, NT>(et, EROW, BM, BNo, (float*)(et + BM * EROW), p.gn_part, tile_m * BM, M, c_tile, Cstore, HWout, p.gn_groups, tid);
      }
    } else {
      const float inv_bno = __builtin_amdgcn_rcpf((float)BNo);
      for (int idx = tid; idx < BM * BNo; idx += NT) {
        const int row = fast_div(idx, BNo, inv_bno), cc = idx - row * BNo;
        const int m = tile_m * BM + row, c = c_tile + cc;
        if (m < M && c < Cstore) {
          float x = to_f32(*(const T*)(et + row * EROW + cc * 2));
          if (resp) x += to_f32(resp[(size_t)m * Cstore + c]);
          outp[(size_t)m * Cstore + c] = from_f32<T>(x);
        }
      }
    }
  }
#if !ES_STAMPS
  if (p.prof && tid == 0) atomicMax(p.prof + 1, (unsigned long long)__builtin_amdgcn_s_memrealtime());
#else
  pstamp(4);
#endif
}

template <typename T>
__global__ __launch_bounds__(256) void splitk_reduce_kernel(const es_gemm_desc p, const int M) {
  const int oct = p.rows_padded / 8;
  const int idx = blockIdx.x * 256 + threadIdx.x;
// ... 12 lines not shown
  }
  float bv[8] = {0.f, 0.f, 0.f, 0.f, 0.f, 0.f, 0.f, 0.f}, tv[8] = {0.f, 0.f, 0.f, 0.f, 0.f, 0.f, 0.f, 0.f};
  float rv[8] = {0.f, 0.f, 0.f, 0.f, 0.f, 0.f, 0.f, 0.f};
  if (bsel) {
    const f32x4 b0 = *(const f32x4*)(bsel + c0), b1 = *(const f32x4*)(bsel + c0 + 4);
#pragma unroll
    for (int r = 0; r < 4; ++r) { bv[r] = b0[r]; bv[4 + r] = b1[r]; }
  }
  if (p.temb) {
    const T* tp = (const T*)p.temb + (size_t)n * p.temb_stride + c0;
    if (full && (p.temb_stride & 7) == 0 && (((size_t)p.temb) & 15) == 0) {
      const auto t8 = as_vec8<T>(*(const u32x4*)tp);
#pragma unroll
      for (int r = 0; r < 8; ++r) tv[r] = to_f32(t8[r]);
    } else {
      for (int r = 0; r < nv; ++r) tv[r] = to_f32(tp[r]);
    }
  }
  if (p.residual) {
    const T* rp = (const T*)p.residual + (size_t)m * p.Cout + c0;
    if (full) {
      const auto r8 = as_vec8<T>(*(const u32x4*)rp);
#pragma unroll
      for (int r = 0; r < 8; ++r) rv[r] = to_f32(r8[r]);
    } else {
      for (int r = 0; r < nv; ++r) rv[r] = to_f32(rp[r]);
    }
  }
  float scale = p.out_scale;
  if (p.out_scale_dev) scale *= *p.out_scale_dev;
  f32x4 s0 = {0.f, 0.f, 0.f, 0.f}, s1 = {0.f, 0.f, 0.f, 0.f};
  const size_t zstride = (size_t)M * p.rows_padded;
  const float* w = p.workspace + (size_t)m * p.rows_padded + c0;
  int z = 0;
  for (; z + 4 <= p.splitk; z += 4) {
    f32x4 a[4], b[4];
#pragma unroll
    for (int u = 0; u < 4; ++u) { a[u] = *(const f32x4*)(w + (z + u) * zstride); b[u] = *(const f32x4*)(w + (z + u) * zstride + 4); }
#pragma unroll
    for (int u = 0; u < 4; ++u) { s0 += a[u]; s1 += b[u]; }
  }
  for (; z < p.splitk; ++z) {
    s0 += *(const f32x4*)(w + z * zstride);
    s1 += *(const f32x4*)(w + z * zstride + 4);
  }
  float v[8] = {s0[0], s0[1], s0[2], s0[3], s1[0], s1[1], s1[2], s1[3]};
#pragma unroll
  for (int r = 0; r < 8; ++r) {
    float x = v[r] + bv[r] + tv[r];
    if (p.act == ES_ACT_SILU) x = silu_f(x);
    x = to_f32(from_f32<T>(x * scale));
    v[r] = x + rv[r];
  }
  T* o = (T*)p.out + (size_t)m * p.Cout + c0;
  if (full && p.out_lo) {
    typename Traits<T>::vec8 pk, lo;
    if (p.residual_lo) {
      const auto l8 = as_vec8<T>(*(const u32x4*)((const T*)p.residual_lo + (size_t)m * p.Cout + c0));
#pragma unroll
      for (int r = 0; r < 8; ++r) v[r] += to_f32(l8[r]);
    }
#pragma unroll
    for (int r = 0; r < 8; ++r) { pk[r] = from_f32<T>(v[r]); lo[r] = from_f32<T>(v[r] - to_f32(pk[r])); }
    store16(o, __builtin_bit_cast(u32x4, pk));
    store16((T*)p.out_lo + (size_t)m * p.Cout + c0, __builtin_bit_cast(u32x4, lo));
  } else if (full) {
    typename Traits<T>::vec8 pk;
#pragma unroll
    for (int r = 0; r < 8; ++r) pk[r] = from_f32<T>(v[r]);
    store16(o, __builtin_bit_cast(u32x4, pk));
  } else {
    store_elems<T>(o, v, nv);
  }
}

template <typename T, int CB>
__global__ __launch_bounds__(64 * (CB / 8)) void splitk_reduce_gn_kernel(const es_gemm_desc p, const int M) {
  constexpr int OCT = CB / 8, NTH = 64 * OCT, ITEMS = 1, EROW = CB * 2 + 16;
  __shared__ __attribute__((aligned(16))) char smem[64 * EROW + (8 + 1) * CB * 8];
  const int tid = threadIdx.x;
  const int nct = p.rows_padded / CB;
  const int mb = blockIdx.x / nct, ct = blockIdx.x - mb * nct;
  const int HW = p.Hout * p.Wout;
  float scale = p.out_scale;
  if (p.out_scale_dev) scale *= *p.out_scale_dev;
  const size_t zstride = (size_t)M * p.rows_padded;
#pragma unroll
  for (int it = 0; it < ITEMS; ++it) {
    const int idx = tid + it * NTH;
    const int row = idx / OCT, o = idx - row * OCT;
    const int m = mb * 64 + row, c0 = ct * CB + o * 8;
    u32x4 res = {0u, 0u, 0u, 0u};
    if (c0 < p.Cout) {
      const int n = m / HW;
      const float* bsel = p.bias;
      if (p.ngroups > 1) {
        const int tm = m >> 7;
        bsel = p.bias_g[(tm >= p.mt_end[0]) + (tm >= p.mt_end[1]) + (tm >= p.mt_end[2])];
      }
      float bv[8] = {0.f, 0.f, 0.f, 0.f, 0.f, 0.f, 0.f, 0.f}, tv[8] = {0.f, 0.f, 0.f, 0.f, 0.f, 0.f, 0.f, 0.f};
      float rv[8] = {0.f, 0.f, 0.f, 0.f, 0.f, 0.f, 0.f, 0.f};
      if (bsel) {
        const f32x4 b0 = *(const f32x4*)(bsel + c0), b1 = *(const f32x4*)(bsel + c0 + 4);
#pragma unroll
        for (int r = 0; r < 4; ++r) { bv[r] = b0[r]; bv[4 + r] = b1[r]; }
      }
      if (p.temb) {
// ... 106 lines not shown
    else if (stages == 3) ES_LAUNCH(128, BNV, true, 3);                                                     \
    else ES_LAUNCH(128, BNV, true, 4);                                                                      \
  } while (0)
  if (d.bn == 256) { if (es_conv_gemm8p_launch(d, st)) return -2; }
  else if (d.ln_colsum) {
    const bool w8 = d.waves == 8;
    if (d.bn == 64)            { if (stages == 4) ES_LAUNCH_LN(64, 64, 4, 2); else ES_LAUNCH_LN(64, 64, 2, 2); }
    else if (d.bn == 128 && w8) { if (stages == 4) ES_LAUNCH_LN(128, 128, 4, 2); else ES_LAUNCH_LN(128, 128, 2, 2); }
    else if (d.bn == 128)       { if (stages == 4) ES_LAUNCH_LN(128, 128, 4, 4); else ES_LAUNCH_LN(128, 128, 2, 4); }
    else if (w8)                { ES_LAUNCH_LN(128, 160, 2, 2); }
    else                        { if (stages == 4) ES_LAUNCH_LN(128, 160, 4, 4); else ES_LAUNCH_LN(128, 160, 2, 4); }
  }
  else if (d.bn == 64)  { if (stages == 4) ES_LAUNCH_F(64, 64, true, 4, 2); else ES_LAUNCH_F(64, 64, true, 2, 2); }
  else if (d.bn == 320) { if (es_conv_gemm8p_launch(d, st)) return -2; }
  else if (d.bn == 128) { if (aligned) ES_LAUNCH_ST(128); else ES_LAUNCH(128, 128, false, 2); }
  else                  { if (aligned) ES_LAUNCH_ST(160); else ES_LAUNCH(128, 160, false, 2); }
#undef ES_LAUNCH_ST
#undef ES_LAUNCH
#undef ES_LAUNCH_F
#undef ES_LAUNCH_K
#undef ES_LAUNCH_LN
  if (d.splitk > 1 && d.gn_part) {
    const int cb = (d.bn == 320 || d.bn == 160) ? 80 : (d.bn == 128 ? 128 : 64);
    dim3 grid((unsigned)((M / 64) * (d.rows_padded / cb)));
    if (cb == 80) hipLaunchKernelGGL((splitk_reduce_gn_kernel<T, 80>), grid, dim3(64 * 10), 0, st, d, M);
    else if (cb == 128) hipLaunchKernelGGL((splitk_reduce_gn_kernel<T, 128>), grid, dim3(64 * 16), 0, st, d, M);
    else hipLaunchKernelGGL((splitk_reduce_gn_kernel<T, 64>), grid, dim3(64 * 8), 0, st, d, M);
  } else if (d.splitk > 1) {
    const long long total = (long long)M * (d.rows_padded / 8);
    hipLaunchKernelGGL(splitk_reduce_kernel<T>, dim3((unsigned)((total + 255) / 256)), dim3(256), 0, st, d, M);
  }
  return hipGetLastError() == hipSuccess ? 0 : -2;
}

#define ES_OPERAND_LIMIT es_operand_limit_v

unsigned long long sample_bytes(const es_gemm_desc& d) {
  const unsigned long long cs = d.act == ES_ACT_GEGLU ? d.Cout / 2 : d.Cout;
  unsigned long long b = d.x_nmod ? 0ull : (unsigned long long)d.Hsrc * d.Wsrc * (d.C1 > d.C2 ? d.C1 : d.C2) * 2;
  const unsigned long long o = (unsigned long long)d.Hout * d.Wout * cs * 2;
  b = b > o ? b : o;
  if (d.t1) { const unsigned long long t = (unsigned long long)d.Hout * d.Wout * (d.Ct1 > d.Ct2 ? d.Ct1 : d.Ct2) * 2; b = b > t ? b : t; }
  return b;
}

bool oversize(const es_gemm_desc& d) {
  if (sample_bytes(d) * (unsigned long long)d.N >= ES_OPERAND_LIMIT) return true;
  if (d.x_nmod && (unsigned long long)d.x_nmod * d.Hsrc * d.Wsrc * d.C1 * 2 >= ES_OPERAND_LIMIT) return true;
  return d.splitk > 1 && (long long)d.N * d.Hout * d.Wout * (d.rows_padded / 8) >= (1ll << 31);
}

int launch_in_chunks(const es_gemm_desc& d0, hipStream_t st, const char** why, bool dry) {
  const long long hw = (long long)d0.Hout * d0.Wout;
  const unsigned long long per = sample_bytes(d0);
  if (d0.gn_part) { *why = "es_conv_gemm: a launch larger than 2 GiB per operand cannot hand GroupNorm statistics over (gn_part)"; return -1; }
  if (d0.x_nmod && (unsigned long long)d0.x_nmod * d0.Hsrc * d0.Wsrc * d0.C1 * 2 >= ES_OPERAND_LIMIT) { *why = "es_conv_gemm: source larger than 2 GiB (32-bit buffer offsets)"; return -1; }
  long long ns = (long long)((ES_OPERAND_LIMIT - 1) / (per ? per : 1));
  if (d0.splitk > 1) { const long long cap = ((1ll << 31) - 1) / (hw * (d0.rows_padded / 8)); ns = ns < cap ? ns : cap; }
  if (hw == 1 && ns >= 256) ns -= ns % 256;
  if (d0.x_nmod) ns -= ns % d0.x_nmod;
  if (ns < 1) { *why = "es_conv_gemm: one sample's operands exceed 2 GiB (32-bit buffer offsets)"; return -1; }
  const int ng = d0.ngroups > 1 ? d0.ngroups : 1;
  const long long cs = d0.act == ES_ACT_GEGLU ? d0.Cout / 2 : d0.Cout;
  long long g0 = 0;
  for (int g = 0; g < ng; ++g) {
    long long g1 = d0.N;
    if (d0.ngroups > 1) {
      const long long px = (long long)d0.mt_end[g] * 128;
      if (px % hw) { *why = "es_conv_gemm: a grouped launch larger than 2 GiB per operand needs groups of whole samples"; return -1; }
      g1 = px / hw;
    }
    if (d0.x_nmod && g0 % d0.x_nmod) { *why = "es_conv_gemm: a launch larger than 2 GiB per operand needs groups that start on a multiple of x_nmod"; return -1; }
    for (long long n0 = g0; n0 < g1; n0 += ns) {
      es_gemm_desc s = d0;
      s.N = (int)((g1 - n0) < ns ? (g1 - n0) : ns);
      if (d0.ngroups > 1) {
        s.w = d0.w_g[g]; s.bias = d0.bias_g[g];
        if (d0.ln_colsum) s.ln_colsum = d0.ln_colsum_g[g];
      }
      s.ngroups = 0;
      for (int k = 0; k < 4; ++k) s.mt_end[k] = 0x7FFFFFFF;
      auto adv = [](const void* p, long long bytes) -> const void* { return p ? (const void*)((const char*)p + bytes) : nullptr; };
      const long long src_px = n0 * d0.Hsrc * d0.Wsrc, out_px = n0 * hw;
      if (!d0.x_nmod) s.x = adv(d0.x, src_px * d0.C1 * 2);
      s.x2 = adv(d0.x2, src_px * d0.C2 * 2);
      s.t1 = adv(d0.t1, out_px * d0.Ct1 * 2);
      s.t2 = adv(d0.t2, out_px * d0.Ct2 * 2);
      s.temb = adv(d0.temb, n0 * d0.temb_stride * 2);
      s.residual = adv(d0.residual, out_px * cs * 2);
      s.residual_lo = adv(d0.residual_lo, out_px * cs * 2);
      s.out = (void*)adv(d0.out, out_px * cs * 2);
      s.out_lo = (void*)adv(d0.out_lo, out_px * cs * 2);
      if (dry) continue;
      const int rc = s.dtype == ES_F16 ? launch<f16>(s, st) : launch<bf16>(s, st);
      if (rc) { *why = "es_conv_gemm: launch failed"; return rc; }
    }
    g0 = g1;
  }
  return 0;
}

}

extern "C" void es_set_error(const char* msg);

extern "C" unsigned long long es_set_operand_limit(unsigned long long bytes) {
  const unsigned long long prev = es_operand_limit_v;
  es_operand_limit_v = bytes && bytes < 0x7FFFFFFFull ? bytes : 0x7FFFFFFFull;
  return prev;
}

extern "C" size_t es_conv_gemm_workspace_bytes(const es_gemm_desc* d) {
  if (d->splitk <= 1) return 0;
  return (size_t)d->splitk * d->N * d->Hout * d->Wout * d->rows_padded * sizeof(float);
}

extern "C" int es_conv_gemm(const es_gemm_desc* d, void* stream) {
  const int Ctot = d->C1 + d->C2;
  const int Ktrue = d->ksize * d->ksize * Ctot + (d->t1 ? d->Ct1 + d->Ct2 : 0);
  if (!d->x || !d->out || (d->ngroups <= 1 && !d->w)) { es_set_error("es_conv_gemm: null pointer"); return -1; }
  if (d->ngroups > 4) { es_set_error("es_conv_gemm: at most 4 groups"); return -1; }
  if (d->ngroups > 1) {
    const int tm = (d->N * d->Hout * d->Wout + 127) / 128;
    for (int g = 0; g < d->ngroups; ++g)
      if (!d->w_g[g] || d->mt_end[g] <= (g ? d->mt_end[g - 1] : 0)) { es_set_error("es_conv_gemm: bad group table"); return -1; }
    if (d->mt_end[d->ngroups - 1] != tm || (d->N * d->Hout * d->Wout) % 128) { es_set_error("es_conv_gemm: groups must tile M in whole 128-pixel tiles"); return -1; }
    if (d->bn == 320 || d->bn == 256)
      for (int g = 0; g < d->ngroups; ++g)
        if (d->mt_end[g] & 1) { es_set_error("es_conv_gemm: 256-pixel tiles need groups of whole 256-pixel tiles"); return -1; }
  }
  if (d->bn != 64 && d->bn != 128 && d->bn != 160 && d->bn != 320 && d->bn != 256) { es_set_error("es_conv_gemm: bn must be 64, 128, 160, 256 or 320"); return -1; }
  if (d->bn == 256 && (d->C1 % BK || d->C2 % BK || (d->stages != 0 && d->stages != 2) || d->waves == 8 || d->korder || d->temb)) {
    es_set_error("es_conv_gemm: bn=256 is the 256-pixel phase-interleaved tile of the LayerNorm-folded / GEGLU linear layers: 64-aligned channels, 2 stages, tap-major K, no time embedding"); return -1; }
  if (d->bn == 64 && (d->C1 % BK || d->C2 % BK || d->stages == 3 || d->waves == 8 || d->act == ES_ACT_GEGLU)) {
    es_set_error("es_conv_gemm: bn=64 is the 64x64 tile: 64-aligned channels, 2 or 4 stages, no GEGLU"); return -1; }
  if (d->bn == 320 && (d->C1 % BK || d->C2 % BK || (d->stages != 0 && d->stages != 2) || d->act == ES_ACT_GEGLU || d->waves == 8)) {
    es_set_error("es_conv_gemm: bn=320 is the 256-pixel phase-interleaved tile: 64-aligned channels, 2 stages, no GEGLU"); return -1; }
  if (d->rows_padded % d->bn || d->rows_padded < d->Cout) { es_set_error("es_conv_gemm: bad rows_padded"); return -1; }
  if (d->Kpad % BK || d->Kpad < Ktrue) { es_set_error("es_conv_gemm: bad Kpad"); return -1; }
  if (d->C1 % 8 || d->C2 % 8 || (d->C2 && !d->x2)) { es_set_error("es_conv_gemm: channels must be multiples of 8"); return -1; }
  if (d->C2 && (d->C1 % BK || d->C2 % BK)) { es_set_error("es_conv_gemm: concatenated sources need C1, C2 multiples of 64"); return -1; }
  if ((size_t)d->rows_padded * d->Kpad * 2 >= 0x7FFFFFFFull) { es_set_error("es_conv_gemm: weights larger than 2 GiB (32-bit buffer offsets)"); return -1; }
  if (d->N < 1 || d->Hout < 1 || d->Wout < 1 || d->Cout < 1) { es_set_error("es_conv_gemm: empty problem"); return -1; }
  const bool chunked = oversize(*d);
  if (chunked) {
    const char* why = nullptr;
    if (launch_in_chunks(*d, nullptr, &why, true)) { es_set_error(why); return -1; }
  }
  if (d->ksize != 1 && d->ksize != 3) { es_set_error("es_conv_gemm: ksize must be 1 or 3"); return -1; }
  if (d->t1 && (d->stride != 1 || d->upsample || d->C1 % BK || d->C2 % BK || d->Ct1 % BK || d->Ct2 % BK || d->Ct1 < BK ||
                (d->Ct2 && !d->t2) || d->ln_colsum || d->Hout != d->Hsrc || d->Wout != d->Wsrc ||
                false)) {
    es_set_error("es_conv_gemm: 1x1 tail sources need stride 1, no upsample, same-size output, 64-aligned channels"); return -1; }
  if (!d->t1 && (d->t2 || d->Ct1 || d->Ct2)) { es_set_error("es_conv_gemm: tail fields set without t1"); return -1; }
  if (d->x_nmod < 0 || (d->x_nmod && (d->x2 || d->t1 || d->x_nmod > d->N))) { es_set_error("es_conv_gemm: x_nmod needs a single source and 0 < x_nmod <= N"); return -1; }
  if (d->out_lo && (!d->residual || (d->Cout & 7) || d->act == ES_ACT_GEGLU)) {
    es_set_error("es_conv_gemm: out_lo (wide residual stream) needs a residual and an output width that is a multiple of 8"); return -1; }
  if (d->residual_lo && !d->out_lo) { es_set_error("es_conv_gemm: residual_lo without out_lo"); return -1; }
  if (d->gn_part) {
    const int hw = d->Hout * d->Wout;
    if (d->gn_groups < 1 || d->Cout % d->gn_groups || (d->Cout & 7) || hw % 64 || d->act == ES_ACT_GEGLU || d->ln_colsum ||
        d->Cout / d->gn_groups > (d->bn == 320 ? 160 : d->bn) || (d->splitk > 1 && d->Cout / d->gn_groups > 64)) {
      es_set_error("es_conv_gemm: gn_part needs H*W % 64 == 0, Cout % 8 == 0 and whole GroupNorm groups no wider than the N tile"); return -1; }
  }
  if (d->korder != 0 && (d->korder != 1 || d->ksize != 3 || d->C1 % BK || d->C2 % BK || d->ln_colsum)) {
    es_set_error("es_conv_gemm: korder 1 (chunk-major K) needs ksize 3 and 64-aligned C1, C2"); return -1; }
  if (d->splitk < 1 || d->splitk > d->Kpad / BK) { es_set_error("es_conv_gemm: bad splitk"); return -1; }
  if (d->splitk > 1 && (!d->workspace || d->act == ES_ACT_GEGLU)) { es_set_error("es_conv_gemm: splitk needs workspace and no GEGLU"); return -1; }
  if (d->act == ES_ACT_GEGLU && ((d->bn != 128 && d->bn != 256) || d->Cout % 32)) { es_set_error("es_conv_gemm: GEGLU needs bn=128 | 256, Cout%32==0"); return -1; }
  if (d->stages != 0 && (d->stages < 2 || d->stages > 4)) { es_set_error("es_conv_gemm: stages must be 0 (auto), 2, 3 or 4"); return -1; }
  if (d->waves != 0 && d->waves != 4 && d->waves != 8) { es_set_error("es_conv_gemm: waves must be 0 (auto), 4 or 8"); return -1; }
  if (d->ln_colsum && (d->ksize != 1 || d->stride != 1 || d->C2 || d->C1 % BK || d->Kpad != d->C1 || d->splitk != 1 ||
                       d->bn == 320 || d->upsample || d->temb || d->stages == 3)) {
    es_set_error("es_conv_gemm: LayerNorm fold needs a plain linear layer: ksize 1, one source, K = C1 (multiple of 64), splitk 1, bn 64|128|160"); return -1; }
  if (d->ln_colsum && d->ngroups > 1)
    for (int g = 0; g < d->ngroups; ++g)
      if (!d->ln_colsum_g[g]) { es_set_error("es_conv_gemm: grouped LayerNorm fold needs ln_colsum_g for every group"); return -1; }
  if (d->waves == 8 && (d->bn == 320 || d->C1 % BK || d->C2 % BK || d->stages == 3 ||
                        (d->stages == 4 && d->bn != 128))) {
    es_set_error("es_conv_gemm: waves=8 is the 128-pixel tile on 8 waves: 64-aligned channels, 2 stages (4 with bn=128)"); return -1; }
  ES_PLAN_RECORD(ES_OP_CONV_GEMM, d, sizeof(*d));
  hipStream_t st = (hipStream_t)stream;
  es_gemm_desc dd = *d;
  for (int g = dd.ngroups > 1 ? dd.ngroups : 0; g < 4; ++g) dd.mt_end[g] = 0x7FFFFFFF;
  if (chunked) {
    const char* why = "es_conv_gemm: launch failed";
    const int rc = launch_in_chunks(*d, st, &why, false);
    if (rc) es_set_error(why);
    return rc;
  }
  int rc = dd.dtype == ES_F16 ? launch<f16>(dd, st) : launch<bf16>(dd, st);
  if (rc) es_set_error("es_conv_gemm: launch failed");
  return rc;
}
```

### edgestyle_amd/engine.py

```python
import os
import weakref
from typing import Dict, List, Optional, Sequence, Tuple

import torch

from . import lib as L
from . import ops
from .config import UNetConfig, VAEConfig

SD = Dict[str, torch.Tensor]


def fold_lora(sd: SD) -> SD:
    out = {k: v for k, v in sd.items() if ".lora_layer." not in k}
    for k in sd:
        if k.endswith(".lora_layer.down.weight"):
            base = k[: -len(".lora_layer.down.weight")]
            up = sd[base + ".lora_layer.up.weight"].double()
            out[base + ".weight"] = (sd[base + ".weight"].double() + up @ sd[k].double()).float()
    return out


_PACK_CACHE = {}


class _Packer:

    def __init__(self, sd: SD, dtype, device):
        self.sd, self.dtype, self.device = sd, dtype, device

    def t(self, key):
        return self.sd[key].to(self.device, torch.float32)

    def conv(self, p: str, cin_pad: Optional[int] = None, geglu=False, cout_pad=None) -> ops.PackedWeight:
        w = self.sd[p + ".weight"]
        b = self.sd.get(p + ".bias")
        key = (id(w), None if b is None else id(b), str(self.dtype), str(self.device), geglu, cin_pad, cout_pad)
        hit = _PACK_CACHE.get(key)
        if hit is not None and hit[0]() is w and (b is None or hit[1]() is b):
            return hit[2]
        pw = ops.pack_weight(self.t(p + ".weight"), None if b is None else b.to(self.device), self.dtype,
                             self.device, geglu=geglu, cin_pad=cin_pad, cout_pad=cout_pad)
        _PACK_CACHE[key] = (weakref.ref(w), None if b is None else weakref.ref(b), pw)
        return pw

    def conv_tail(self, p: str, pt: str) -> ops.PackedWeight:
        w, wt = self.sd[p + ".weight"], self.sd[pt + ".weight"]
        key = (id(w), id(wt), str(self.dtype), str(self.device), "tail")
        hit = _PACK_CACHE.get(key)
        if hit is not None and hit[0]() is w and hit[1]() is wt:
            return hit[2]
        pw = ops.pack_weight_tail(self.t(p + ".weight"), self.t(pt + ".weight"), self.t(p + ".bias") + self.t(pt + ".bias"),
                                  self.dtype, self.device)
        _PACK_CACHE[key] = (weakref.ref(w), weakref.ref(wt), pw)
        return pw

    def cat(self, ps: Sequence[str], bias: bool) -> ops.PackedWeight:
        w = torch.cat([self.t(p + ".weight") for p in ps], 0)
        b = torch.cat([self.t(p + ".bias") for p in ps], 0) if bias else None
        return ops.pack_weight(w, b, self.dtype, self.device)

    def norm(self, p: str) -> Tuple[torch.Tensor, torch.Tensor]:
        return self.t(p + ".weight").contiguous(), self.t(p + ".bias").contiguous()

    def cat_ln(self, ps: Sequence[str], bias: bool, ln: str, geglu: bool = False) -> ops.PackedWeight:
        w = torch.cat([self.t(p + ".weight") for p in ps], 0)
        b = torch.cat([self.t(p + ".bias") for p in ps], 0) if bias else None
        return ops.pack_weight_ln(w, b, self.t(ln + ".weight"), self.t(ln + ".bias"), 1e-5, self.dtype, self.device,
                                  geglu=geglu)


SHORTCUT_FOLD = os.environ.get("ES_SHORTCUT_FOLD", "1") == "1"
FFO_FOLD = os.environ.get("ES_FFO_FOLD", "1") == "1"
LN_FOLD = os.environ.get("ES_LN_FOLD", "1") in ("1", "qk")
LN_FOLD_FF = os.environ.get("ES_LN_FOLD", "1") == "1"


class Resnet:
    def __init__(self, pk: _Packer, p: str, groups: int, eps: float, temb_off: Optional[int]):
        self.n1, self.n2 = pk.norm(p + ".norm1"), pk.norm(p + ".norm2")
        self.conv1, self.conv2 = pk.conv(p + ".conv1"), pk.conv(p + ".conv2")
        self.short = pk.conv(p + ".conv_shortcut") if (p + ".conv_shortcut.weight") in pk.sd else None
        self.groups, self.eps, self.temb_off = groups, eps, temb_off
        self.cout = self.conv1.cout
        self.conv2s = None
        w2, ws_ = pk.sd[p + ".conv2.weight"], pk.sd.get(p + ".conv_shortcut.weight")
        if SHORTCUT_FOLD and ws_ is not None and w2.shape[1] % 64 == 0 and ws_.shape[1] % 64 == 0:
            self.conv2s = pk.conv_tail(p + ".conv2", p + ".conv_shortcut")

    def __call__(self, x, tproj, x2=None):
        h = ops.group_norm(x, self.n1[0], self.n1[1], self.groups, self.eps, True, x2=x2)
        temb = None if self.temb_off is None else tproj[:, self.temb_off:]
        h = ops.conv_gemm(h, self.conv1, temb=temb, gn_groups=self.groups)
        h = ops.group_norm(h, self.n2[0], self.n2[1], self.groups, self.eps, True)
        if self.conv2s is not None and (x2 is None or (x.shape[3] % 64 == 0 and x2.shape[3] % 64 == 0)):
            return ops.conv_gemm(h, self.conv2s, tail=(x, x2), gn_groups=self.groups)
# ... 89 lines not shown
        out = [a for blk in self.down for (_, a) in blk if a is not None]
        return out + [self.mid_attn]

    def context(self, ehs, outs: Optional[List[torch.Tensor]] = None) -> List[torch.Tensor]:
        tr = self.transformers()
        if outs is not None and outs[0].shape[0] == ehs.shape[0]:
            return [t.context(ehs, o) for t, o in zip(tr, outs)]
        return [t.context(ehs) for t in tr]

    def time_proj(self, t_dev: torch.Tensor, step_idx: Optional[torch.Tensor] = None) -> torch.Tensor:
        e = ops.timestep_embedding(t_dev, self.cfg.block_out_channels[0], self.dtype)
        e = ops.linear(e, self.t1, act=L.ACT_SILU)
        e = ops.linear(e, self.t2, act=L.ACT_SILU)
        return ops.linear(e, self.tproj)

    @property
    def tproj_width(self) -> int:
        return self.tproj.cout

    def run(self, h, tproj, ctx: List[torch.Tensor]):
        skips = [h]
        ci = 0
        for i, blk in enumerate(self.down):
            for r, a in blk:
                h = r(h, tproj)
                if a is not None:
                    h = a(h, ctx[ci]); ci += 1
                skips.append(h)
            if self.downsample[i] is not None:
                h = ops.conv_gemm(h, self.downsample[i], stride=2, gn_groups=self.cfg.norm_num_groups)
                skips.append(h)
        h = self.mid0(h, tproj)
        h = self.mid_attn(h, ctx[ci])
        h = self.mid1(h, tproj)
        return skips, h


class UNet(Encoder):
    def __init__(self, sd: SD, cfg: UNetConfig, dtype, device):
        n = len(cfg.block_out_channels)
        extra = [f"up_blocks.{i}.resnets.{j}" for i in range(n) for j in range(cfg.layers_per_block + 1)]
        super().__init__(sd, cfg, dtype, device, extra_resnets=extra)
        pk, g, eps, heads = self.pk, cfg.norm_num_groups, cfg.norm_eps, cfg.num_heads
        self.up: List[List[Tuple[Resnet, Optional[Transformer]]]] = []
        self.upsample: List[Optional[ops.PackedWeight]] = []
        for i in range(n):
            blk = []
            for j in range(cfg.layers_per_block + 1):
                nm = f"up_blocks.{i}.resnets.{j}"
                r = Resnet(pk, nm, g, eps, self.temb_offs[nm])
                a = Transformer(pk, f"up_blocks.{i}.attentions.{j}", heads, g) if cfg.up_has_attn[i] else None
                blk.append((r, a))
            self.up.append(blk)
            self.upsample.append(pk.conv(f"up_blocks.{i}.upsamplers.0.conv") if i != n - 1 else None)
        self.norm_out = pk.norm("conv_norm_out")
        self.conv_out = pk.conv("conv_out")
        del self.pk

    def transformers(self):
        return super().transformers() + [a for blk in self.up for (_, a) in blk if a is not None]

    def encode(self, x, tproj, ctx):
        h = ops.conv_gemm(x, self.conv_in, gn_groups=self.cfg.norm_num_groups)
        return self.run(h, tproj, ctx)

    def forward(self, x, tproj, ctx, down_res: Optional[Sequence] = None, mid_res=None, out=None, encoded=None,
                presummed: bool = False):
        skips, h = encoded if encoded is not None else self.encode(x, tproj, ctx)
        skips = list(skips)
        if presummed:
            skips = [r.reshape(s.shape) for s, r in zip(skips, down_res)]
            h = mid_res.reshape(h.shape)
        else:
            if down_res is not None:
                skips = [ops.add(s, r.reshape(s.shape)) for s, r in zip(skips, down_res)]
            if mid_res is not None:
                h = ops.add(h, mid_res.reshape(h.shape))
        ci = len(super().transformers())
        cfg = self.cfg
        for i, blk in enumerate(self.up):
            for r, a in blk:
                h = r(h, tproj, x2=skips.pop())
                if a is not None:
                    h = a(h, ctx[ci]); ci += 1
            if self.upsample[i] is not None:
                h = ops.conv_gemm(h, self.upsample[i], upsample=True)
        h = ops.group_norm(h, self.norm_out[0], self.norm_out[1], cfg.norm_num_groups, cfg.norm_eps, True)
        return ops.conv_gemm(h, self.conv_out, out=out)


class ControlNet(Encoder):

    def __init__(self, sd: SD, cfg: UNetConfig, dtype, device, uses_vae: bool = False):
        super().__init__(sd, cfg, dtype, device)
        pk = self.pk
        table = cfg.residual_table()
        self.zero = [pk.conv(f"controlnet_down_blocks.{i}") for i in range(len(table) - 1)]
        self.zero_mid = pk.conv("controlnet_mid_block")
        self.uses_vae = uses_vae
        self.cond = None
        if not uses_vae and "controlnet_cond_embedding.conv_in.weight" in pk.sd:
            ce = cfg.conditioning_embedding_out_channels
            p = "controlnet_cond_embedding"
            self.cond = [pk.conv(p + ".conv_in", cin_pad=8)]
            self.cond += [pk.conv(f"{p}.blocks.{i}") for i in range(2 * (len(ce) - 1))]
            self.cond.append(pk.conv(p + ".conv_out"))
        del self.pk

    def embed_cond(self, img):
        h = ops.conv_gemm(img, self.cond[0], act=L.ACT_SILU)
        for i, pw in enumerate(self.cond[1:-1]):
            h = ops.conv_gemm(h, pw, stride=2 if i % 2 == 1 else 1, act=L.ACT_SILU)
        return ops.conv_gemm(h, self.cond[-1])

    def embed_latent(self, z, out=None):
        return ops.conv_gemm(z, self.conv_in, out=out)

    def forward(self, x, tproj, ctx, conds: Sequence[torch.Tensor], out_scale: float = 1.0,
                out_scale_dev=None, level_scales: Optional[Sequence[float]] = None):
        k = len(conds)
        N, H, W, _ = x.shape
        c0 = self.conv_in.cout
        h0 = torch.empty((k * N, H, W, c0), dtype=x.dtype, device=x.device)
        for i, c in enumerate(conds):
            ops.conv_gemm(x, self.conv_in, residual=c, out=h0[i * N:(i + 1) * N])
        skips, h = self.run(h0, tproj, ctx)
        ls = list(level_scales) if level_scales is not None else [1.0] * (len(self.zero) + 1)
        res = [ops.conv_gemm(s, z, out_scale=out_scale * ls[i], out_scale_dev=out_scale_dev)
               for i, (s, z) in enumerate(zip(skips, self.zero))]
        res.append(ops.conv_gemm(h, self.zero_mid, out_scale=out_scale * ls[-1], out_scale_dev=out_scale_dev))
        return res


class Fusion:

    def __init__(self, sd: SD, cfg: UNetConfig, dtype, device, sample_size: Optional[int] = None):
        self.table = cfg.residual_table(sample_size)
        self.params = []
        for i in range(len(self.table)):
            p = f"multi_controlnet_down_blocks.{i}" if i < len(self.table) - 1 else "multi_controlnet_mid_block"
            self.params.append(ops.pack_fusion_params(sd, p, dtype, device))

    def forward(self, res_per_net: Sequence[Sequence[torch.Tensor]], bs: Sequence[Sequence[int]], N: int,
                scales: Sequence[float], scales_dev=None, addends=None, first_level: int = 0):
        nl = len(res_per_net[0])
        table = self.table[first_level:first_level + nl]
        blocks = [([res_per_net[i][k] for i in range(6)], [bs[i][k] for i in range(6)], self.params[first_level + k], s * s, c)
                  for k, (c, s) in enumerate(table)]
        outs = ops.fusion_blocks(blocks, N, scales, scales_dev, addends=addends, first_block=first_level)
        return [o.reshape(N, s, s, c) for o, (c, s) in zip(outs, table)]


class VAE:
    def __init__(self, sd: SD, cfg: VAEConfig, dtype, device, decoder: bool = True, encoder: bool = True):
        self.cfg, self.dtype, self.device = cfg, dtype, device
        pk = _Packer(sd, dtype, device)
        g, eps = cfg.norm_num_groups, cfg.norm_eps
        ch = cfg.block_out_channels
        n = len(ch)
        self.lat_pad = (cfg.latent_channels + 7) // 8 * 8

        def mid(side):
            a = f"{side}.mid_block.attentions.0"
            return dict(r0=Resnet(pk, f"{side}.mid_block.resnets.0", g, eps, None),
                        gn=pk.norm(a + ".group_norm"),
                        qkv=pk.cat([a + ".to_q", a + ".to_k", a + ".to_v"], bias=True),
                        o=pk.conv(a + ".to_out.0"),
                        r1=Resnet(pk, f"{side}.mid_block.resnets.1", g, eps, None))
        if encoder:
            self.e_in = pk.conv("encoder.conv_in", cin_pad=8)
            self.e_down = []
            for i in range(n):
                rs = [Resnet(pk, f"encoder.down_blocks.{i}.resnets.{j}", g, eps, None)
                      for j in range(cfg.layers_per_block)]
                ds = pk.conv(f"encoder.down_blocks.{i}.downsamplers.0.conv") if i != n - 1 else None
                self.e_down.append((rs, ds))
            self.e_mid = mid("encoder")
            self.e_norm = pk.norm("encoder.conv_norm_out")
            self.e_out = pk.conv("encoder.conv_out")
            self.quant = pk.conv("quant_conv")
        if decoder:
            self.post_quant = pk.conv("post_quant_conv", cin_pad=self.lat_pad, cout_pad=8)
            b = sd.get("post_quant_conv.bias")
            self.post_quant_scaled = ops.pack_weight(
                (pk.t("post_quant_conv.weight").double() / cfg.scaling_factor).float(), None if b is None else b.to(device), dtype,
                device, cin_pad=self.lat_pad, cout_pad=8)
            self.d_in = pk.conv("decoder.conv_in", cin_pad=8)
            self.d_mid = mid("decoder")
            self.d_up = []
            for i in range(n):
                rs = [Resnet(pk, f"decoder.up_blocks.{i}.resnets.{j}", g, eps, None)
                      for j in range(cfg.layers_per_block + 1)]
                us = pk.conv(f"decoder.up_blocks.{i}.upsamplers.0.conv") if i != n - 1 else None
                self.d_up.append((rs, us))
            self.d_norm = pk.norm("decoder.conv_norm_out")
            self.d_out = pk.conv("decoder.conv_out")

    def _mid(self, m, h):
        cfg = self.cfg
        h = m["r0"](h, None)
        N, H, W, C = h.shape
        n = ops.group_norm(h, m["gn"][0], m["gn"][1], cfg.norm_num_groups, cfg.norm_eps, False).reshape(N, H * W, C)
        qkv = ops.linear(n, m["qkv"])
        a = ops.attention(qkv[:, :, :C], qkv[:, :, C:2 * C], qkv[:, :, 2 * C:], 1)
        h = ops.linear(a, m["o"], residual=h.reshape(N, H * W, C)).reshape(N, H, W, C)
        return m["r1"](h, None)

    def encode_moments(self, img):
        cfg = self.cfg
        h = ops.conv_gemm(img, self.e_in)
        for rs, ds in self.e_down:
            for r in rs:
                h = r(h, None)
            if ds is not None:
                h = ops.conv_gemm(h, ds, stride=2, pad=0, out_hw=(h.shape[1] // 2, h.shape[2] // 2))
        h = self._mid(self.e_mid, h)
        h = ops.group_norm(h, self.e_norm[0], self.e_norm[1], cfg.norm_num_groups, cfg.norm_eps, True)
        h = ops.conv_gemm(h, self.e_out)
        return ops.conv_gemm(h, self.quant)

    def decode(self, z, unscaled_latents: bool = False):
        cfg = self.cfg
        h = ops.conv_gemm(z, self.post_quant_scaled if unscaled_latents else self.post_quant)
        h = ops.conv_gemm(h, self.d_in)
        h = self._mid(self.d_mid, h)
        for rs, us in self.d_up:
            for r in rs:
                h = r(h, None)
            if us is not None:
                h = ops.conv_gemm(h, us, upsample=True)
        h = ops.group_norm(h, self.d_norm[0], self.d_norm[1], cfg.norm_num_groups, cfg.norm_eps, True)
        return ops.conv_gemm(h, self.d_out)


class GroupedEncoder:

    def __init__(self, encoders: Sequence[Encoder], counts: Sequence[int]):
        self.encs, self.counts = list(encoders), list(counts)
        e0 = self.encs[0]
        self.cfg = e0.cfg
        for e in self.encs[1:]:
            if e.cfg.block_out_channels != e0.cfg.block_out_channels or e.cfg.layers_per_block != e0.cfg.layers_per_block:
                raise L.EdgeStyleHipError("grouped encoders must share the architecture")
        self.ntot = sum(self.counts)
        self.width = max(e.tproj_width for e in self.encs)

    def groupable(self, hw_min: int) -> bool:
        return len(self.encs) <= 4 and all((n * hw_min) % ops.BM == 0 for n in self.counts)

    def time_proj(self, t_rows: torch.Tensor, out: Optional[torch.Tensor] = None) -> torch.Tensor:
        if out is None:
            out = torch.zeros((self.ntot, self.width), dtype=self.encs[0].dtype, device=t_rows.device)
        es = out.element_size()
        a = 0
        for e, n in zip(self.encs, self.counts):
            proj = e.time_proj(t_rows[:n])
            ops.memcpy2d(out[a].data_ptr(), self.width * es, proj.data_ptr(), e.tproj_width * es, e.tproj_width * es, n)
            a += n
        return out

    def _resnet(self, rs, x, tproj):
        c = self.counts
        r0 = rs[0]
        h = ops.group_norm(x, [r.n1[0] for r in rs], [r.n1[1] for r in rs], r0.groups, r0.eps, True, group_n=c)
        h = ops.conv_gemm(h, [r.conv1 for r in rs], temb=tproj[:, r0.temb_off:], group_n=c, gn_groups=r0.groups)
        h = ops.group_norm(h, [r.n2[0] for r in rs], [r.n2[1] for r in rs], r0.groups, r0.eps, True, group_n=c)
        if all(r.conv2s is not None for r in rs):
            return ops.conv_gemm(h, [r.conv2s for r in rs], tail=(x,), group_n=c, gn_groups=r0.groups)
        xs = ops.conv_gemm(x, [r.short for r in rs], group_n=c) if r0.short is not None else x
        return ops.conv_gemm(h, [r.conv2 for r in rs], residual=xs, group_n=c, wide=True, gn_groups=r0.groups)

    def _transformer(self, ts, x, kv):
        c = self.counts
        t0 = ts[0]
        N, H, W, C = x.shape
        rows = [n * H * W for n in c]
        tok = ops.gn_proj_in(x, [t.norm[0] for t in ts], [t.norm[1] for t in ts], t0.groups, 1e-6, [t.proj_in for t in ts], group_n=c).reshape(N, H * W, C)
        fold = all(t.ln_fold for t in ts)

        def ln_linear(k, plain, folded):
            if fold and folded is not None:
                return ops.linear(tok, [getattr(t, folded) for t in ts], group_n=rows)
            n = ops.layer_norm(tok, [getattr(t, k)[0] for t in ts], [getattr(t, k)[1] for t in ts], group_rows=rows)
# ... 32 lines not shown
```

### edgestyle_amd/lib.py

```python
import ctypes as C
import os

_HERE = os.path.dirname(os.path.abspath(__file__))
LIB_PATH = os.environ.get("ES_HIP_LIB") or os.path.join(_HERE, "lib", "libedgestyle_hip.so")

ES_F16, ES_BF16, ES_F32 = 0, 1, 2
ABI_VERSION = 7
ACT_NONE, ACT_SILU, ACT_GEGLU = 0, 1, 2


class GemmDesc(C.Structure):
    _fields_ = [
        ("x", C.c_void_p), ("x2", C.c_void_p), ("w", C.c_void_p), ("bias", C.c_void_p), ("temb", C.c_void_p),
        ("residual", C.c_void_p), ("out_scale_dev", C.c_void_p), ("out", C.c_void_p), ("workspace", C.c_void_p),
        ("prof", C.c_void_p),
        ("N", C.c_int32), ("Hsrc", C.c_int32), ("Wsrc", C.c_int32), ("C1", C.c_int32), ("C2", C.c_int32),
        ("Hout", C.c_int32), ("Wout", C.c_int32), ("Cout", C.c_int32),
        ("rows_padded", C.c_int32), ("Kpad", C.c_int32),
        ("ksize", C.c_int32), ("stride", C.c_int32), ("pad", C.c_int32),
        ("upsample", C.c_int32), ("temb_stride", C.c_int32), ("act", C.c_int32), ("splitk", C.c_int32),
        ("bn", C.c_int32), ("dtype", C.c_int32),
        ("ngroups", C.c_int32), ("mt_end", C.c_int32 * 4), ("w_g", C.c_void_p * 4), ("bias_g", C.c_void_p * 4),
        ("stages", C.c_int32), ("xcd_m_fastest", C.c_int32), ("waves", C.c_int32),
        ("out_scale", C.c_float),
# ... 126 lines not shown
    "es_fusion_block": (C.c_int, [C.POINTER(FusionDesc), _P]),
    "es_fusion_scratch_bytes": (C.c_size_t, [_I]),
    "es_fusion_blocks": (C.c_int, [C.POINTER(FusionDesc), _I, _P]),
    "es_timestep_embedding": (C.c_int, [_P, _P, _I, _I, _I, _P]),
    "es_cfg_ddim_step": (C.c_int, [_P, _P, _P, _P, _P, _F, _I, _I, _I, _I, _I, _I, _I, _P]),
    "es_cfg_unipc_step": (C.c_int, [_P, _P, _P, _P, _P, _P, _P, _P, _F, _I, _I, _I, _I, _I, _I, _I, _P]),
    "es_nchw_f32_to_nhwc": (C.c_int, [_P, _P, _I, _I, _I, _I, _I, _P]),
    "es_nhwc_to_nchw_f32": (C.c_int, [_P, _P, _I, _I, _I, _I, _F, _F, _I, _I, _P]),
    "es_add": (C.c_int, [_P, _P, _P, _L, _I, _P]),
    "es_vae_sample": (C.c_int, [_P, _P, _P, _I, _I, _I, _I, _F, _I, _P]),
    "es_incr": (C.c_int, [_P, _P]),
    "es_clock_probe": (C.c_int, [_P, C.c_uint, _P]),
    "es_gather_row": (C.c_int, [_P, _P, _P, _I, _I, _P]),
    "es_layer_norm_grouped": (C.c_int, [C.POINTER(LnDesc), _P]),
    "es_latents_to_input": (C.c_int, [_P, _P, _I, _I, _I, _I, _I, _I, _P]),
    "es_memcpy": (C.c_int, [_P, _P, C.c_size_t, _P]),
    "es_memcpy2d": (C.c_int, [_P, C.c_size_t, _P, C.c_size_t, C.c_size_t, C.c_size_t, _P]),
    "es_fill_f32": (C.c_int, [_P, _F, C.c_size_t, _P]),
    "es_plan_create": (_P, []),
    "es_plan_destroy": (None, [_P]),
    "es_plan_begin_record": (C.c_int, [_P]),
    "es_plan_end_record": (C.c_int, [_P]),
    "es_plan_size": (C.c_int, [_P]),
    "es_plan_count": (C.c_int, [_P, _I]),
    "es_plan_launch": (C.c_int, [_P, _P]),
    "es_ctx_create": (C.c_int, [_I, C.POINTER(_P)]),
    "es_ctx_destroy": (None, [_P]),
    "es_ctx_set_geometry": (C.c_int, [_P, C.POINTER(CtxGeometry)]),
    "es_ctx_set_plan": (C.c_int, [_P, _I, _P]),
    "es_ctx_bind": (C.c_int, [_P, _I, _P, C.c_size_t]),
    "es_ctx_buffer": (_P, [_P, _I, C.POINTER(C.c_size_t)]),
    "es_ctx_arena_bytes": (C.c_size_t, [_P]),
    "es_ctx_set_options": (C.c_int, [_P, C.POINTER(C.c_float), _F, _F, _I]),
    "es_ctx_set_scheduler": (C.c_int, [_P, _I]),
    "es_ctx_set_alphas_cumprod_f64": (C.c_int, [_P, C.POINTER(C.c_double), _I]),
    "es_unipc_coef_table": (C.c_int, [C.POINTER(C.c_double), _I, C.POINTER(C.c_float), _I, C.POINTER(C.c_float)]),
    "es_ctx_set_alphas_cumprod": (C.c_int, [_P, C.POINTER(C.c_float), _I]),
    "es_ctx_plan_size": (C.c_int, [_P, _I]),
    "es_ctx_plan": (_P, [_P, _I]),
    "es_ctx_load": (C.c_int, [C.c_char_p, _I, C.POINTER(_P)]),
    "es_ctx_save": (C.c_int, [_P, C.c_char_p]),
    "es_plan_export": (C.c_size_t, [_P, _P, C.c_size_t]),
    "es_plan_import": (_P, [_P, C.c_size_t]),
    "es_plan_pointer_fields": (C.c_int, [_I, C.POINTER(C.c_int32), C.POINTER(C.c_int32), _I, C.POINTER(C.c_int32)]),
    "es_ctx_launch_plan": (C.c_int, [_P, _I, C.POINTER(C.c_float), _P]),
    "es_ddim_coef_table": (C.c_int, [C.POINTER(C.c_float), _I, C.POINTER(C.c_float), _I, C.POINTER(C.c_float)]),
    "es_denoise_step": (C.c_int, [_P, _P, _F, _P, C.POINTER(_P), C.POINTER(C.c_float), _P, _P]),
    "es_denoise_loop": (C.c_int, [_P, _P, _P, _F, C.POINTER(C.c_float), _I, _P]),
    "es_vae_decode": (C.c_int, [_P, _P, _P, _P]),
    "es_prepare_conds": (C.c_int, [_P, C.POINTER(_P), C.POINTER(_P), _P]),
    "es_load_weights": (C.c_int, [C.POINTER(Weights), C.POINTER(ModelConfig), C.POINTER(CtxGeometry), _I, C.POINTER(_P)]),
    "es_plan_gemm_choice": (C.c_int, [C.c_longlong, _I, _I, _I, C.POINTER(C.c_int), _I, _I, C.POINTER(C.c_int), C.POINTER(C.c_int),
                                      C.POINTER(C.c_int)]),
    "es_linear_xs_eligible": (C.c_int, [C.c_longlong, _I, _I, _I, _I, _I, _I]),
    "es_conv_gemm8p_form_ok": (C.c_int, [_I, _I, _I, C.c_longlong, _I]),
    "es_ctx_graph_hazard": (C.c_int, []),
    "es_plan_set_dry": (C.c_int, [_I]),
}

_lib = None


FUSION_MAX_BATCH = 13


class EdgeStyleHipError(RuntimeError):
    pass


def load():
    global _lib
    if _lib is not None:
        return _lib
    if not os.path.exists(LIB_PATH):
        raise EdgeStyleHipError(
            f"{LIB_PATH} not found: build it with `python -c 'import __graft_entry__ as g; g.build()'` "
            "(hipcc --offload-arch=gfx950). There is no CPU fallback for the product path.")
    lib = C.CDLL(LIB_PATH)
    for name, (res, args) in SYMBOLS.items():
        fn = getattr(lib, name)
        fn.restype = res
        fn.argtypes = args
    if lib.es_abi_version() != ABI_VERSION:
        raise EdgeStyleHipError("libedgestyle_hip.so ABI version mismatch")
    for i, st in enumerate((GemmDesc, AttnDesc, GnDesc, FusionDesc, LnDesc, XsDesc)):
        if lib.es_sizeof_desc(i) != C.sizeof(st):
            raise EdgeStyleHipError(f"descriptor layout mismatch for {st.__name__}: C {lib.es_sizeof_desc(i)} "
                                    f"vs ctypes {C.sizeof(st)}")
    _lib = lib
    return lib


def check(rc: int, what: str = ""):
    if rc != 0:
        msg = load().es_last_error()
        raise EdgeStyleHipError(f"{what} failed (rc={rc}): {msg.decode() if msg else ''}")
```

### edgestyle_amd/ops.py

```python
import ctypes as C
import math
import os as _os
from dataclasses import dataclass
from typing import Optional, Sequence

import torch

from . import lib as L

_DT = {torch.float16: L.ES_F16, torch.bfloat16: L.ES_BF16}
LANE = 0


class lane:

    def __init__(self, i: int):
        self.i = i

    def __enter__(self):
        global LANE
        self.prev, LANE = LANE, self.i

    def __exit__(self, *a):
        global LANE
# ... 23 lines not shown
        self.slots[:, 0] = 1 << 62
        self.slots[:, 1] = 0

    def next(self, meta) -> int:
        i = len(self.meta)
        if i >= self.slots.shape[0]:
            raise L.EdgeStyleHipError("Profiler capacity exceeded")
        self.meta.append(meta)
        return self.slots[i].data_ptr() if self.stamps else 0

    def replay_gemms(self, only_ksize: int = 0):
        lib = L.load()
        for d in self.descs:
            if only_ksize and (isinstance(d, L.XsDesc) or int(d.ksize) != only_ksize):
                continue
            fn = lib.es_linear_xs if isinstance(d, L.XsDesc) else lib.es_conv_gemm
            L.check(fn(C.byref(d), _stream()), "GEMM replay")

    def results(self, first: int = 0):
        s = self.slots[first:len(self.meta)].cpu().tolist()
        return [(m, (e - b) * 1e-8) for m, (b, e) in zip(self.meta[first:], s) if e > 0]
BK = 64
BM = 128


def _stream():
    return C.c_void_p(torch.cuda.current_stream().cuda_stream)


def _ptr(t: Optional[torch.Tensor]):
    return None if t is None else C.c_void_p(t.data_ptr())


def _dt(t: torch.Tensor) -> int:
    try:
        return _DT[t.dtype]
    except KeyError:
        raise L.EdgeStyleHipError(f"unsupported dtype {t.dtype}: the HIP path computes in fp16 or bf16")


@dataclass
class PackedWeight:
    w: torch.Tensor
    bias: Optional[torch.Tensor]
    cout: int
    cin: int
    ksize: int
    bn: int
    geglu: bool = False
    ln_colsum: Optional[torch.Tensor] = None
    ln_eps: float = 1e-5
    ctail: int = 0
    korder: int = 0

    @property
    def rows_padded(self):
        return self.w.shape[0]

    @property
    def kpad(self):
        return self.w.shape[1]


def choose_bn(cout: int) -> int:
    return 160 if (cout % 160 == 0 and cout % 128 != 0) else 128


CHUNK_MAJOR = _os.environ.get("ES_CHUNK_MAJOR", "0") == "1"


def choose_korder(k: int, cin_padded: int) -> int:
    return 1 if (CHUNK_MAJOR and k == 3 and cin_padded % BK == 0) else 0


def _chunk_major(w: torch.Tensor, k: int, cin: int) -> torch.Tensor:
    cout = w.shape[0]
    return w.reshape(cout, k * k, cin // BK, BK).permute(0, 2, 1, 3).reshape(cout, k * k * cin)


def pack_weight(weight: torch.Tensor, bias: Optional[torch.Tensor], dtype, device, geglu: bool = False,
                cin_pad: Optional[int] = None, cout_pad: Optional[int] = None) -> PackedWeight:
    if weight.dim() == 2:
        weight = weight[:, :, None, None]
    weight = weight.to(device=device, dtype=torch.float32)
    cout, cin, k, _ = weight.shape
    cp = cin_pad or ((cin + 7) // 8 * 8)
    w = weight.permute(0, 2, 3, 1)
    if cp != cin:
        w = torch.nn.functional.pad(w, (0, cp - cin))
    w = w.reshape(cout, k * k * cp)
    korder = choose_korder(k, cp)
    if korder:
        w = _chunk_major(w, k, cp)
    b = None if bias is None else bias.to(device=device, dtype=torch.float32)
    if geglu:
        inner = cout // 2
        assert inner % 16 == 0
        idx = torch.arange(cout, device=device)
        blk, within = idx // 32, idx % 32
        src = torch.where(within < 16, blk * 16 + within, inner + blk * 16 + (within - 16))
        w = w[src]
        if b is not None:
            b = b[src]
    cout_eff = cout_pad or cout
    bn = 128 if geglu else choose_bn(cout_eff)
    rows = (cout_eff + bn - 1) // bn * bn
    ktrue = w.shape[1]
    kpad = (ktrue + BK - 1) // BK * BK
    wp = torch.zeros(rows, kpad, dtype=dtype, device=device)
    wp[:cout, :ktrue] = w.to(dtype)
    bp = None
    if b is not None:
        bp = torch.zeros(rows, dtype=torch.float32, device=device)
        bp[:cout] = b
    return PackedWeight(wp, bp, cout_eff, cp, k, bn, geglu, korder=korder)


def pack_weight_tail(weight: torch.Tensor, tail_weight: torch.Tensor, bias: Optional[torch.Tensor], dtype, device) -> PackedWeight:
    weight = weight.to(device=device, dtype=torch.float32)
    tw = tail_weight.to(device=device, dtype=torch.float32).reshape(tail_weight.shape[0], -1)
    cout, cin, k, _ = weight.shape
    if cin % BK or tw.shape[1] % BK or tw.shape[0] != cout:
        raise L.EdgeStyleHipError("pack_weight_tail: conv and tail channels must be multiples of 64, equal Cout")
    korder = choose_korder(k, cin)
    wm = weight.permute(0, 2, 3, 1).reshape(cout, k * k * cin)
    w = torch.cat([_chunk_major(wm, k, cin) if korder else wm, tw], 1)
    bn = choose_bn(cout)
    rows = (cout + bn - 1) // bn * bn
    wp = torch.zeros(rows, w.shape[1], dtype=dtype, device=device)
    wp[:cout] = w.to(dtype)
    bp = None
    if bias is not None:
        bp = torch.zeros(rows, dtype=torch.float32, device=device)
        bp[:cout] = bias.to(device=device, dtype=torch.float32)
    return PackedWeight(wp, bp, cout, cin, k, bn, False, ctail=tw.shape[1], korder=korder)


def pack_weight_ln(weight: torch.Tensor, bias: Optional[torch.Tensor], gamma: torch.Tensor, beta: torch.Tensor,
                   eps: float, dtype, device, geglu: bool = False) -> PackedWeight:
    w = weight.to(device=device, dtype=torch.float32)
    if w.dim() == 4:
        w = w[:, :, 0, 0]
    g = gamma.to(device=device, dtype=torch.float32)
    b = beta.to(device=device, dtype=torch.float32)
    fb = w.double() @ b.double()
    if bias is not None:
        fb = fb + bias.to(device=device, dtype=torch.float64)
    pw = pack_weight(w * g[None, :], fb.float(), dtype, device, geglu=geglu)
    pw.ln_colsum = pw.w.double().sum(dim=1).float().contiguous()
    pw.ln_eps = float(eps)
    return pw


_workspace = {}
_workspace_retired = []


def _get_workspace(nbytes: int, device) -> torch.Tensor:
    device = (device, LANE)
    ws = _workspace.get(device)
    if ws is None or ws.numel() * 4 < nbytes:
        if torch.cuda.is_current_stream_capturing():
            raise L.EdgeStyleHipError("split-K workspace too small during graph capture; run one eager warm-up first")
        if ws is not None:
            _workspace_retired.append(ws)
        ws = torch.empty(max(nbytes // 4, 1 << 22), dtype=torch.float32, device=device[0])
        _workspace[device] = ws
    return ws
# ... 43 lines not shown
            return other
        t256 = ((M + 255) // 256) * (rows_padded // 256)
        c256 = float(-(-t256 // 256)) * (nk * PLAN_T256 + PLAN_T256_FIX + (PLAN_T256_GEGLU if geglu else 0.0))
        take = other is None
        if other is not None and M >= PLAN_BIG_MIN_M and nk >= PLAN_BIG_MIN_NK and other[1] == 1 and other[0] != 64:
            to = ((M + BM - 1) // BM) * (rows_padded // other[0])
            co = float(-(-to // PLAN_RESIDENT)) * (nk * PLAN_LN_TK * (PLAN_T160 if other[0] == 160 else 1.0) + PLAN_T256_FIX)
            take = c256 < PLAN_T256_MARGIN * co
        return (256, 1, 2) if take else other
    if geglu:
        return 128, 1, 2
    nk = kpad // BK
    best = None
    for bn in bns:
        if rows_padded % bn:
            continue
        if bn == 320 and (M < PLAN_BIG_MIN_M or nk < PLAN_BIG_MIN_NK) and len(bns) > 1:
            continue
        if bn == 64 and M > PLAN_SMALL_MAX_M and len(bns) > 1:
            continue
        bm = {320: 256, 64: 64}.get(bn, BM)
        resident = {320: PLAN_RESIDENT // 2, 64: 2 * PLAN_RESIDENT}.get(bn, PLAN_RESIDENT)
        tiles = ((M + bm - 1) // bm) * (rows_padded // bn)
        cands = [1]
        if allow_split and tiles < resident // 2 and nk > PLAN_NK_NOSPLIT:
            cands += list(range(2, min(nk // PLAN_MIN_SLICE, 32) + 1))
        for sk in cands:
            wgs = tiles * sk
            if bn == 320:
                tk = PLAN_T320
            elif bn == 64:
                if sk > 1 and wgs > PLAN_RESIDENT:
                    continue
                w = wgs / (PLAN_RESIDENT // 2)
                tk = (PLAN_T64_ALONE + PLAN_T64 * max(0.0, w - 1.0) ** 2) * (1.0 if nk <= 40 else PLAN_T64_LONG)
            else:
                tk = (PLAN_T160 if bn == 160 else 1.0) * (PLAN_ALONE if wgs <= PLAN_RESIDENT // 2 else 1.0)
            rounds = max(wgs / 256.0, 0.9) if bn == 320 else float(-(-wgs // resident))
            t = rounds * ((nk / sk) * tk + (PLAN_T320_FIX if bn == 320 else PLAN_TFIX))
            if sk > 1:
                t += PLAN_RED_FIX + sk * M * rows_padded * 8.0 / PLAN_SLAB_BYTES_PER_UNIT
            if best is None or t < best[0]:
                best = (t, bn, sk, wgs)
    if best is None:
        raise L.EdgeStyleHipError(f"plan_gemm: rows_padded {rows_padded} fits no N tile")
    _, bn, sk, wgs = best
    if bn == 64:
        stages = 4 if (DEEP_RING and LANE == 0 and wgs <= PLAN_RESIDENT and nk // sk >= 6) else 2
    else:
        stages = 4 if (bn != 320 and DEEP_RING and LANE == 0 and wgs <= PLAN_RESIDENT // 2 and nk // sk >= 6) else 2
    return bn, sk, stages


def choose_launch_bn(M: int, pw: "PackedWeight") -> int:
    return plan_gemm(M, pw.rows_padded, pw.kpad, pw.geglu)[0]


def choose_splitk(M: int, rows_padded: int, bn: int, kpad: int) -> int:
    return plan_gemm(M, rows_padded, kpad, bns=(bn,))[1]


def plan_launch(M: int, pw: "PackedWeight", bn: int):
    _, sk, st = plan_gemm(M, pw.rows_padded, pw.kpad, pw.geglu, bns=(bn,))
    return sk, st


XS_ENABLED = _os.environ.get("ES_XS", "1") == "1"
XS_RESIDUAL = _os.environ.get("ES_XS_RESIDUAL", "1") == "1"
XS_TARGET_WGS = 256
XS_FORCE_SLICES = 0
XS_MIN_M = int(_os.environ.get("ES_XS_MIN_M", "8192"))
_zero_bias = {}


def xs_shape_reference(M: int, pw: "PackedWeight", min_m: int) -> bool:
    if pw.ksize != 1 or pw.kpad not in (320, 640) or pw.cin != pw.kpad or pw.ctail:
        return False
    ch = 64 if pw.kpad == 320 else 32
    line = ch * (128 // (ch if pw.geglu else 2 * ch))
    if pw.cout % line or pw.cout < 4 * line:
        return False
    if min_m and (M < min_m or (M < 4 * min_m and pw.cout < (960 if pw.kpad == 320 else 1920))):
        return False
    return True


def xs_eligible(M: int, pw: "PackedWeight", pws, group_n, hw: int) -> bool:
    if not XS_ENABLED:
        return False
    if pws is not None:
        if len(pws) > 4 or any((n * hw) % 256 for n in group_n) or any((q.ln_colsum is None) != (pw.ln_colsum is None) for q in pws):
            return False
    if XS_MIN_M != 8192:
        return xs_shape_reference(M, pw, XS_MIN_M)
    return bool(L.load().es_linear_xs_eligible(int(M), int(pw.ksize), int(pw.kpad), int(pw.cin), int(pw.ctail), int(pw.cout), int(pw.geglu)))


def linear_xs(x: torch.Tensor, pw, M: int, out: torch.Tensor, group_rows=None, residual: Optional[torch.Tensor] = None,
              gn: Optional[dict] = None) -> torch.Tensor:
    pws = None
    if isinstance(pw, (list, tuple)):
        pws = list(pw) if len(pw) > 1 else None
        pw = pw[0]
    K = pw.kpad
    ch = 64 if K == 320 else 32
    pline = 128 // (ch if pw.geglu else 2 * ch)
# ... 41 lines not shown
            if (q.rows_padded, q.kpad, q.cout, q.geglu) != (pw.rows_padded, pw.kpad, pw.cout, pw.geglu):
                raise L.EdgeStyleHipError("grouped linear_xs: weight geometry differs between groups")
            acc += n // 128
            d.mt_end[g] = acc
            d.w_g[g] = q.w.data_ptr()
            d.bias_g[g] = bias_of(q)
    if PROFILE is not None:
        d.prof = PROFILE.next((2.0 * M * pw.cout * K, 1, (M, pw.cout, K, 1, 1, 0),
                               dict(N=M, H=1, W=1, C1=K, C2=0, cout=pw.cout, k=1, stride=1, pad=0, upsample=False,
                                    geglu=pw.geglu, splitk=1, Hout=1, Wout=1, residual=residual is not None, temb=False, bn=0, stages=3,
                                    group_n=list(group_rows) if pws is not None else None, ctail=0, kernel="linear_xs",
                                    algorithmic_bytes=_algorithmic_bytes(x, None, pw, pws, out, residual))))
        dd = L.XsDesc()
        C.memmove(C.byref(dd), C.byref(d), C.sizeof(L.XsDesc))
        dd.prof = None
        PROFILE.descs.append(dd)
    L.check(L.load().es_linear_xs(C.byref(d), _stream()), "es_linear_xs")
    return out


WIDE_STREAM = _os.environ.get("ES_WIDE_STREAM", "auto")


GN_HANDOVER = _os.environ.get("ES_GN_HANDOVER", "0") in ("1", "all")


def gn_handover(hw: int, c: int, groups: int) -> bool:
    if not GN_HANDOVER or c % 8 or hw % 64 or c % groups or c // groups > 64:
        return False
    return GN_HANDOVER_ALL or not L.load().es_group_norm_is_slab(hw, c, groups)


GN_HANDOVER_ALL = _os.environ.get("ES_GN_HANDOVER", "0") == "all"


def wide_stream(dtype) -> bool:
    return WIDE_STREAM == "1" or (WIDE_STREAM == "auto" and dtype == torch.bfloat16)


def carry_lo(dst: torch.Tensor, src: torch.Tensor, shape=None) -> torch.Tensor:
    lo = getattr(src, "_lo", None)
    if lo is not None:
        dst._lo = lo.reshape(dst.shape if shape is None else shape)
    return dst


def conv_gemm(x: torch.Tensor, pw: PackedWeight, *, stride: int = 1, pad: Optional[int] = None,
              upsample: bool = False, x2: Optional[torch.Tensor] = None, temb: Optional[torch.Tensor] = None,
              residual: Optional[torch.Tensor] = None, act: int = L.ACT_NONE, out_scale: float = 1.0,
              out_scale_dev: Optional[torch.Tensor] = None, out: Optional[torch.Tensor] = None,
              out_hw=None, splitk: Optional[int] = None, stages: int = 0,
              group_n: Optional[Sequence[int]] = None, tail: Optional[Sequence[torch.Tensor]] = None,
              x_rep: int = 1, wide: bool = False, out_lo: Optional[torch.Tensor] = None, gn_groups: int = 0,
              gn_part: Optional[torch.Tensor] = None):
    pws = None
    if isinstance(pw, (list, tuple)):
        pws = list(pw)
        pw = pws[0]
        if len(pws) == 1:
            pws = None
    N, H, W, C1 = x.shape
    nsrc = N
    if x_rep > 1:
        if x2 is not None or tail:
            raise L.EdgeStyleHipError("conv_gemm: x_rep needs a single source")
        N = N * x_rep
    C2 = 0 if x2 is None else x2.shape[3]
    if C1 + C2 != pw.cin:
        raise L.EdgeStyleHipError(f"conv_gemm: input channels {C1}+{C2} != packed {pw.cin}")
    tails = [t for t in (tail or ()) if t is not None]
    if sum(t.shape[3] for t in tails) != pw.ctail or len(tails) > 2:
        raise L.EdgeStyleHipError(f"conv_gemm: tail channels {[t.shape[3] for t in tails]} != packed {pw.ctail}")
    k = pw.ksize
    if pad is None:
        pad = 1 if k == 3 else 0
    Hin, Win = (H * 2, W * 2) if upsample else (H, W)
    if out_hw is None:
        Hout = (Hin + 2 * pad - k) // stride + 1
        Wout = (Win + 2 * pad - k) // stride + 1
    else:
        Hout, Wout = out_hw
    act_i = L.ACT_GEGLU if pw.geglu else act
    cstore = pw.cout // 2 if pw.geglu else pw.cout
    if out is None:
        out = torch.empty((N, Hout, Wout, cstore), dtype=x.dtype, device=x.device)
    M = N * Hout * Wout
    xs_res = residual is None or (XS_RESIDUAL and pw.kpad == 320 and not pw.geglu and pw.ln_colsum is None and residual.is_contiguous()
                                  and residual.numel() == M * cstore and not (wide and wide_stream(x.dtype)))
    if (k == 1 and stride == 1 and not upsample and x2 is None and temb is None and xs_res and not tails
            and x_rep == 1 and act == L.ACT_NONE and out_scale == 1.0 and out_scale_dev is None and splitk is None and FORCE_BN == 0
            and x.is_contiguous() and out.is_contiguous()
            and xs_eligible(M, pw, pws, group_n, Hout * Wout)):
        linear_xs(x.reshape(M, C1), pws if pws is not None else pw, M, out.reshape(M, cstore),
                  None if pws is None else [n * Hout * Wout for n in group_n], residual=residual)
        return out
    big_ok = BIG_TILE and C1 % BK == 0 and C2 % BK == 0 and not pw.geglu and pw.ln_colsum is None and \
        (group_n is None or all((n * Hout * Wout) % 256 == 0 for n in group_n))
    small_ok = SMALL_TILE and C1 % BK == 0 and C2 % BK == 0 and not pw.geglu and FORCE_WAVES != 8
    ln256_ok = BIG_TILE_256 and (pw.geglu or pw.ln_colsum is not None) and k == 1 and stride == 1 and not upsample and x2 is None \
        and not tails and temb is None and x_rep == 1 and C1 % BK == 0 and pw.rows_padded % 256 == 0 and pw.cout % 8 == 0 \
        and not (pw.geglu and residual is not None) and not wide and gn_groups == 0 and FORCE_WAVES != 8 \
        and (group_n is None or all((n * Hout * Wout) % 256 == 0 for n in group_n))
    cand = ((256,) if ln256_ok else ()) + ((320,) if big_ok else ()) + (160, 128) + ((64,) if small_ok else ())
    bn, auto_splitk, auto_stages = plan_gemm(M, pw.rows_padded, pw.kpad, pw.geglu,
                                             bns=cand if FORCE_BN == 0 else (FORCE_BN,), allow_split=pw.ln_colsum is None)
    if bn == 320 and FORCE_BN == 0 and (auto_splitk if splitk is None else splitk) == 1 and not L.load().es_conv_gemm8p_form_ok(
            int(act_i), int(pw.cout), int(temb is not None), int(Hout * Wout), int(residual is not None)):
        bn, auto_splitk, auto_stages = plan_gemm(M, pw.rows_padded, pw.kpad, pw.geglu, bns=tuple(b for b in cand if b != 320),
                                                 allow_split=pw.ln_colsum is None)
    if splitk is None:
        splitk = auto_splitk
        stages = stages or auto_stages
    d = L.GemmDesc()
    d.x, d.x2, d.w = x.data_ptr(), (x2.data_ptr() if x2 is not None else None), pw.w.data_ptr()
    d.bias = pw.bias.data_ptr() if pw.bias is not None else None
    d.temb = temb.data_ptr() if temb is not None else None
    d.residual = residual.data_ptr() if residual is not None else None
    d.out_scale_dev = out_scale_dev.data_ptr() if out_scale_dev is not None else None
    d.out = out.data_ptr()
    d.N, d.Hsrc, d.Wsrc, d.C1, d.C2 = N, H, W, C1, C2
    d.Hout, d.Wout, d.Cout = Hout, Wout, pw.cout
    d.rows_padded, d.Kpad = pw.rows_padded, pw.kpad
    d.ksize, d.stride, d.pad = k, stride, pad
    d.upsample = 1 if upsample else 0
    d.temb_stride = temb.stride(0) if temb is not None else 0
    d.act, d.splitk, d.bn, d.dtype, d.out_scale = act_i, splitk, bn, _dt(x), out_scale
    d.stages = stages or FORCE_STAGES
    d.korder = pw.korder
    if (gn_groups > 0 and gn_handover(Hout * Wout, cstore, gn_groups) and not pw.geglu and pw.ln_colsum is None
            and pw.cout // gn_groups <= (160 if bn == 320 else bn)):
        shape = (N, 2 * (Hout * Wout // 64), gn_groups, 2)
        part = gn_part if gn_part is not None else torch.empty(shape, dtype=torch.float32, device=x.device)
        if tuple(part.shape) != shape or part.dtype != torch.float32 or not part.is_contiguous():
            raise L.EdgeStyleHipError(f"conv_gemm: gn_part must be a contiguous fp32 {shape}")
        d.gn_part, d.gn_groups = part.data_ptr(), gn_groups
        out._gnp = (part, gn_groups)
    if wide and residual is not None and wide_stream(x.dtype) and cstore % 8 == 0 and not pw.geglu:
        lo_in = getattr(residual, "_lo", None)
        if lo_in is not None:
            if lo_in.numel() != residual.numel() or not lo_in.is_contiguous():
                raise L.EdgeStyleHipError("conv_gemm: the residual's low part does not match it")
            d.residual_lo = lo_in.data_ptr()
        if out_lo is None:
            out_lo = torch.empty_like(out)
        elif out_lo.shape != out.shape or out_lo.dtype != out.dtype or not out_lo.is_contiguous():
            raise L.EdgeStyleHipError("conv_gemm: out_lo must match out")
        d.out_lo = out_lo.data_ptr()
        out._lo = out_lo
    d.xcd_m_fastest = (1 if (pws is None and splitk == 1 and M <= 2048 and pw.w.numel() > x.numel() * x_rep + (x2.numel() if x2 is not None else 0)) else 0) \
        if XCD_ORDER < 0 else XCD_ORDER
    d.x_nmod = nsrc if x_rep > 1 else 0
    if FORCE_WAVES:
        d.waves = FORCE_WAVES
    elif EIGHT_WAVES and k == 1 and M <= 65536 and C1 % BK == 0 and C2 % BK == 0 and bn not in (64, 320, 256) \
            and not (int(d.stages) == 4 and bn != 128) and int(d.stages) != 3:
        d.waves = 8
# ... 379 lines not shown
```

### include/edgestyle_hip.h

```cpp
#ifndef EDGESTYLE_HIP_H
#define EDGESTYLE_HIP_H
#include <stddef.h>
#include <stdint.h>

#ifdef __cplusplus
extern "C" {
#endif

enum { ES_F16 = 0, ES_BF16 = 1, ES_F32 = 2  };
enum { ES_ACT_NONE = 0, ES_ACT_SILU = 1, ES_ACT_GEGLU = 2 };

#define ES_ABI_VERSION 7
int es_abi_version(void);
size_t es_sizeof_desc(int which);
const char* es_last_error(void);

typedef struct {
  const void* x;
  const void* x2;
  const void* w;
  const float* bias;
  const void* temb;
  const void* residual;
  const float* out_scale_dev;
// ... 187 lines not shown
  int32_t n_steps;
  int32_t dtype;
  int32_t guess_mode;
} es_ctx_geometry;
int es_ctx_create(int device, es_ctx** out);
void es_ctx_destroy(es_ctx* c);
int es_ctx_set_geometry(es_ctx* c, const es_ctx_geometry* g);
int es_ctx_set_plan(es_ctx* c, int which, es_plan* p);
int es_ctx_bind(es_ctx* c, int slot, void* dev, size_t bytes);
void* es_ctx_buffer(const es_ctx* c, int slot, size_t* bytes);
size_t es_ctx_arena_bytes(const es_ctx* c);
int es_ctx_set_options(es_ctx* c, const float* cond_scales, float control_guidance_start, float control_guidance_end,
                       int use_graphs);
int es_ctx_set_alphas_cumprod(es_ctx* c, const float* alphas_cumprod, int n);
int es_ctx_set_scheduler(es_ctx* c, int scheduler);
int es_ctx_set_alphas_cumprod_f64(es_ctx* c, const double* alphas_cumprod, int n);
int es_unipc_coef_table(const double* alphas_cumprod, int n_alphas, const float* timesteps, int n, float* out);
int es_ctx_plan_size(const es_ctx* c, int which);
es_plan* es_ctx_plan(es_ctx* c, int which);
int es_ctx_load(const char* path, int device, es_ctx** out);
int es_ctx_save(const es_ctx* c, const char* path);
typedef struct {
  const char* key;
  const void* data;
  int64_t shape[4];
  int32_t ndim;
  int32_t dtype;
} es_tensor;
typedef struct { const es_tensor* tensors; int32_t count; } es_state_dict;
enum { ES_NET_CONTROLNET = 0,
       ES_NET_CONTROL_LORA_VAE = 1,
       ES_NET_CONTROL_LORA = 2 };
typedef struct {
  es_state_dict unet, vae, fusion;
  es_state_dict controlnet[6];
  int32_t controlnet_kind[6];
  int32_t n_controlnets;
  int32_t net_of_cond[6];
} es_weights;
typedef struct {
  int32_t in_channels, out_channels;
  int32_t n_blocks, block_out_channels[4], down_has_attn[4];
  int32_t layers_per_block, num_heads, cross_attention_dim, norm_num_groups;
  float norm_eps;
  int32_t n_cond_embed, cond_embed_channels[4], conditioning_channels;
  int32_t text_tokens;
  int32_t vae_n_blocks, vae_block_out_channels[4], vae_layers_per_block, vae_latent_channels, vae_norm_num_groups;
  float vae_norm_eps, vae_scaling_factor;
} es_model_config;
int es_load_weights(const es_weights* w, const es_model_config* cfg, const es_ctx_geometry* g, int device, es_ctx** out);
int es_plan_gemm_choice(long long M, int rows_padded, int kpad, int geglu, const int* bns, int n_bns, int allow_split,
                        int* bn, int* splitk, int* stages);
int es_linear_xs_eligible(long long M, int ksize, int kpad, int cin, int ctail, int cout, int geglu);
int es_conv_gemm8p_form_ok(int act, int cout, int has_temb, long long out_hw, int has_residual);
int es_ctx_graph_hazard(void);
int es_plan_set_dry(int on);

int es_ctx_launch_plan(es_ctx* c, int which, const float* guidance_scale, void* stream);
int es_ddim_coef_table(const float* alphas_cumprod, int n_alphas, const float* timesteps, int n, float* out);
int es_denoise_step(es_ctx* c, const void* sample, float t, const void* ehs, const void* const* cond_embeds,
                    const float* scales, void* out_noise, void* stream);
int es_denoise_loop(es_ctx* c, float* latents_inout, const void* ehs, float guidance_scale, const float* timesteps,
                    int n_steps, void* stream);
int es_vae_decode(es_ctx* c, const float* latents, float* out_img, void* stream);
int es_prepare_conds(es_ctx* c, const float* const* images, const float* const* noise, void* stream);

#ifdef __cplusplus
}
#endif
#endif
```

Before: 2.229 images/s.

## Fold nearest-upsample + 3x3 conv into four 2x2 sub-pixel phase GEMMs

```diff
diff --git a/edgestyle_amd/csrc/builder.hip b/edgestyle_amd/csrc/builder.hip
--- a/edgestyle_amd/csrc/builder.hip
+++ b/edgestyle_amd/csrc/builder.hip
@@ -251,6 +251,7 @@
   bool geglu = false;
   float ln_eps = 1e-5f;
   const uint16_t* host_w = nullptr;
+  const struct PW* sub = nullptr;
   long long w_numel() const { return (long long)rows_padded * kpad; }
 };
 using PWs = std::vector<const PW*>;
@@ -259,6 +260,7 @@
 struct CA {
   int stride = 1, pad = -1;
   bool upsample = false;
+  bool subpixel = false;
   T x2, temb, residual, out, out_scale_dev;
   long long temb_stride = 0;
   int act = ES_ACT_NONE;
@@ -280,7 +282,7 @@
 constexpr int PLAN_SMALL_MAX_M = 16384, PLAN_MIN_SLICE = 12, PLAN_NK_NOSPLIT = 10, PLAN_RESIDENT = 512;
 
 double plan_env(const char* name, double dflt) { const char* e = getenv(name); return e && *e ? atof(e) : dflt; }
-bool plan_gemm(long long M, int rows_padded, int kpad, bool geglu, const int* bns, int nb, bool allow_split, int* o_bn, int* o_sk, int* o_st) {
+bool plan_gemm(long long M, int rows_padded, int kpad, bool geglu, const int* bns, int nb, bool allow_split, int* o_bn, int* o_sk, int* o_st, double* o_t = nullptr) {
   static const double PLAN_T320 = plan_env("ES_PLAN_T320", ::PLAN_T320), PLAN_T256_MARGIN = plan_env("ES_PLAN_T256_MARGIN", ::PLAN_T256_MARGIN);
   static const int PLAN_BIG_MIN_NK = (int)plan_env("ES_PLAN_BIG_MIN_NK", ::PLAN_BIG_MIN_NK);
   int others[8], no = 0;
@@ -334,8 +336,24 @@
   }
   if (!have) return false;
   *o_bn = bbn; *o_sk = bsk;
+  if (o_t) *o_t = bt;
   if (bbn == 64) *o_st = (bwgs <= PLAN_RESIDENT && nk / bsk >= 6) ? 4 : 2;
   else *o_st = (bbn != 320 && bwgs <= PLAN_RESIDENT / 2 && nk / bsk >= 6) ? 4 : 2;
+  return true;
+}
+
+constexpr double PLAN_SUBPIX_MARGIN = 0.9;
+bool subpixel_fits(long long M, int cin, int cout) { return M % 512 == 0 && cin >= BK && cin % BK == 0 && cout % 8 == 0 && M > 0; }
+bool plan_upsample(long long M, int rows_padded, int cin, int cout, const int* bns, int nb, int* o_sub, int* o_bn, int* o_sk, int* o_st) {
+  double td = 0, ts = 0;
+  int dbn = 0, dsk = 1, dst = 2, sbn = 0, ssk = 1, sst = 2;
+  if (!plan_gemm(M, rows_padded, round_up(9 * cin, BK), false, bns, nb, true, &dbn, &dsk, &dst, &td)) return false;
+  *o_sub = 0; *o_bn = dbn; *o_sk = dsk; *o_st = dst;
+  if (!subpixel_fits(M, cin, cout)) return true;
+  int sb[8], ns = 0;
+  for (int i = 0; i < nb; ++i) if (bns[i] != 320 && bns[i] != 256 && ns < 8) sb[ns++] = bns[i];
+  if (!ns || !plan_gemm(M, rows_padded, 4 * cin, false, sb, ns, true, &sbn, &ssk, &sst, &ts)) return true;
+  if (ts < PLAN_SUBPIX_MARGIN * td) { *o_sub = 1; *o_bn = sbn; *o_sk = ssk; *o_st = sst; }
   return true;
 }
 
@@ -502,6 +520,46 @@
     if (bt) b = W.vec(p + ".bias", cout);
     const PW* pw = pack(w, cout, cin, k, bt ? &b : nullptr, geglu, cin_pad, cout_pad);
     if (!key.empty()) pack_cache[key] = pw;
+    return pw;
+  }
+  const PW* pack_subpixel(const std::vector<float>& w, int cout, int cin, const PW* direct) {
+    if ((long long)w.size() != (long long)cout * cin * 9) fail("builder: sub-pixel pack of a weight that is not 3x3");
+    const int bn = choose_bn(cout), rows = round_up(cout, bn), kpad = 4 * cin;
+    if (cin % BK) fail("builder: sub-pixel pack needs 64-aligned input channels");
+    pws.emplace_back();
+    PW& p = pws.back();
+    p.cout = cout; p.cin = cin; p.ksize = 3; p.bn = bn; p.rows_padded = rows; p.kpad = kpad; p.bias = direct->bias;
+    p.w = persistent((size_t)4 * rows * kpad * 2);
+    uint16_t* dst = (uint16_t*)staged(p.w, (size_t)4 * rows * kpad * 2);
+    p.host_w = dst;
+    parallel_for(cout, [&](long long a, long long b) {
+      for (long long r = a; r < b; ++r) {
+        const float* s = w.data() + (size_t)r * cin * 9;
+        for (int ph = 0; ph < 4; ++ph) {
+          const int py = ph >> 1, px = ph & 1;
+          uint16_t* d = dst + ((size_t)ph * rows + r) * kpad;
+          for (int ty = 0; ty < 2; ++ty)
+            for (int tx = 0; tx < 2; ++tx)
+              for (int ci = 0; ci < cin; ++ci) {
+                double acc = 0.0;
+                for (int ky = 0; ky < 3; ++ky) {
+                  if (((py + ky + 1) >> 1) - 1 + (1 - py) != ty) continue;
+                  for (int kx = 0; kx < 3; ++kx)
+                    if (((px + kx + 1) >> 1) - 1 + (1 - px) == tx) acc += (double)s[(size_t)ci * 9 + ky * 3 + kx];
+                }
+                d[(ty * 2 + tx) * cin + ci] = enc((float)acc);
+              }
+        }
+      }
+    });
+    return &p;
+  }
+  const PW* conv_up(const Weights& W, const std::string& p) {
+    const PW* pw = conv(W, p);
+    if (pw->sub || pw->ksize != 3 || pw->cin % BK || pw->cout % 8 || pw->korder) return pw;
+    const es_tensor* wt = W.get(p + ".weight");
+    if ((int)wt->shape[1] != pw->cin) return pw;
+    const_cast<PW*>(pw)->sub = pack_subpixel(W.matrix(p), pw->cout, pw->cin, pw);
     return pw;
   }
   void stack(const Weights& W, const std::vector<std::string>& ps, bool bias, std::vector<float>& w, std::vector<float>& b, int& rows, int& cols) {
@@ -640,6 +698,23 @@
     cand[nc++] = 160; cand[nc++] = 128;
     if (small_ok) cand[nc++] = 64;
     int bn, splitk, stages;
+    if (a.upsample && a.subpixel && pw->sub && !grouped && k == 3 && a.stride == 1 && pad == 1 && !a.x2 && !a.temb && !a.residual && a.tails.empty() &&
+        a.x_rep == 1 && a.act == ES_ACT_NONE && a.out_scale == 1.f && !a.out_scale_dev && !a.out_h && a.gn_groups == 0) {
+      int sub = 0;
+      if (!plan_upsample(M, pw->rows_padded, pw->cin, pw->cout, cand, nc, &sub, &bn, &splitk, &stages)) fail("plan_gemm: rows_padded fits no N tile");
+      if (sub) {
+        const PW* q = pw->sub;
+        es_gemm_desc d;
+        memset(&d, 0, sizeof(d));
+        d.x = x.ptr(); d.w = (const void*)q->w; d.bias = (const float*)q->bias; d.out = out.ptr();
+        d.N = N; d.Hsrc = H; d.Wsrc = Wd; d.C1 = C1; d.Hout = Hout; d.Wout = Wout; d.Cout = q->cout;
+        d.rows_padded = q->rows_padded; d.Kpad = q->kpad; d.ksize = 3; d.stride = 1; d.pad = 1; d.upsample = 2;
+        d.act = ES_ACT_NONE; d.splitk = splitk; d.bn = bn; d.dtype = dt; d.out_scale = 1.f; d.stages = stages;
+        if (splitk > 1) d.workspace = (float*)workspace((unsigned long long)splitk * M * q->rows_padded * 4);
+        ok(es_conv_gemm(&d, nullptr), "es_conv_gemm");
+        return out;
+      }
+    }
     if (!plan_gemm(M, pw->rows_padded, pw->kpad, pw->geglu, cand, nc, pw->ln_colsum == 0, &bn, &splitk, &stages)) fail("plan_gemm: rows_padded fits no N tile");
     if (bn == 320 && splitk == 1 && !es_conv_gemm8p_form_ok(act_i, pw->cout, a.temb ? 1 : 0, hw, a.residual ? 1 : 0)) {
       if (!plan_gemm(M, pw->rows_padded, pw->kpad, pw->geglu, cand + 1, nc - 1, pw->ln_colsum == 0, &bn, &splitk, &stages)) fail("plan_gemm: rows_padded fits no N tile");
@@ -969,7 +1044,7 @@
         if (c.has_attn[c.nb - 1 - i]) { tr.emplace_back(B, W, "up_blocks." + std::to_string(i) + ".attentions." + std::to_string(j), c.heads, c.groups); ti = (int)tr.size() - 1; }
         up.back().emplace_back(rs, ti);
       }
-      upsample.push_back(i != c.nb - 1 ? B.conv(W, "up_blocks." + std::to_string(i) + ".upsamplers.0.conv") : nullptr);
+      upsample.push_back(i != c.nb - 1 ? B.conv_up(W, "up_blocks." + std::to_string(i) + ".upsamplers.0.conv") : nullptr);
     }
     W.shaped("conv_out.weight", {c.out_ch, c.ch[0], 3, 3});
     norm_out = B.norm(W, "conv_norm_out", c.ch[0]);
@@ -1060,7 +1135,7 @@
     for (int i = 0; i < n; ++i) {
       std::vector<Resnet> rs;
       for (int j = 0; j < c.lpb + 1; ++j) rs.emplace_back(B, W, "decoder.up_blocks." + std::to_string(i) + ".resnets." + std::to_string(j), c.groups, c.eps, -1);
-      d_up.emplace_back(rs, i != n - 1 ? B.conv(W, "decoder.up_blocks." + std::to_string(i) + ".upsamplers.0.conv") : nullptr);
+      d_up.emplace_back(rs, i != n - 1 ? B.conv_up(W, "decoder.up_blocks." + std::to_string(i) + ".upsamplers.0.conv") : nullptr);
     }
     d_norm = B.norm(W, "decoder.conv_norm_out", c.ch[0]);
     d_out = B.conv(W, "decoder.conv_out");
@@ -1092,7 +1167,7 @@
     h = run_mid(B, d_mid, h);
     for (const auto& blk : d_up) {
       for (const auto& r : blk.first) h = r.run(B, h, T());
-      if (blk.second) { CA a; a.upsample = true; h = B.conv_gemm(h, blk.second, a); }
+      if (blk.second) { CA a; a.upsample = true; a.subpixel = true; h = B.conv_gemm(h, blk.second, a); }
     }
     h = B.group_norm(h, d_norm, cfg.groups, cfg.eps, true);
     return B.conv_gemm(h, d_out);
@@ -1320,7 +1395,7 @@
         hh = ra.first.run(B, hh, tp, skip);
         if (ra.second >= 0) { hh = transformer(unet.tr[ra.second], hh, ctx_unet[ci]); ++ci; }
       }
-      if (unet.upsample[i]) { CA a; a.upsample = true; hh = B.conv_gemm(hh, unet.upsample[i], a); }
+      if (unet.upsample[i]) { CA a; a.upsample = true; a.subpixel = true; hh = B.conv_gemm(hh, unet.upsample[i], a); }
     }
     hh = B.group_norm(hh, unet.norm_out, ucfg.groups, ucfg.eps, true);
     CA o; o.out = noise;
@@ -1493,6 +1568,11 @@
 extern "C" int es_plan_gemm_choice(long long M, int rows_padded, int kpad, int geglu, const int* bns, int n_bns, int allow_split, int* bn, int* splitk, int* stages) {
   if (!bns || n_bns < 1 || !bn || !splitk || !stages) { es_set_error("es_plan_gemm_choice: null argument"); return -1; }
   if (!plan_gemm(M, rows_padded, kpad, geglu != 0, bns, n_bns, allow_split != 0, bn, splitk, stages)) { es_set_error("es_plan_gemm_choice: rows_padded fits no N tile"); return -1; }
+  return 0;
+}
+extern "C" int es_plan_upsample_choice(long long M, int rows_padded, int cin, int cout, const int* bns, int n_bns, int* subpixel, int* bn, int* splitk, int* stages) {
+  if (!bns || n_bns < 1 || !subpixel || !bn || !splitk || !stages || cin < 1) { es_set_error("es_plan_upsample_choice: null argument"); return -1; }
+  if (!plan_upsample(M, rows_padded, cin, cout, bns, n_bns, subpixel, bn, splitk, stages)) { es_set_error("es_plan_upsample_choice: rows_padded fits no N tile"); return -1; }
   return 0;
 }
 extern "C" int es_linear_xs_eligible(long long M, int ksize, int kpad, int cin, int ctail, int cout, int geglu) {
diff --git a/edgestyle_amd/csrc/gemm_conv.hip b/edgestyle_amd/csrc/gemm_conv.hip
--- a/edgestyle_amd/csrc/gemm_conv.hip
+++ b/edgestyle_amd/csrc/gemm_conv.hip
@@ -38,6 +38,7 @@
                               const int Hin, const int Win, const int upsample, const int Wsrc) {
   int ky = 0, kx = 0;
   if (ksize == 3) { ky = (tp * 11) >> 5; kx = tp - ky * 3; }
+  if (ksize == 2) { ky = tp >> 1; kx = tp & 1; }
   if (tp >= KK) { ky = pad; kx = pad; }
 #pragma unroll
   for (int i = 0; i < XI; ++i) {
@@ -120,8 +121,19 @@
   const bool has_tail = tail1 != nullptr;
   const int Ctail = has_tail ? pCt1 + pCt2 : 0;
   const int Ktrue = KK * Ctot + Ctail;
-  const int Hin = p.Hsrc << p.upsample, Win = p.Wsrc << p.upsample;
+  const int up = p.upsample & 1;
+  const int Hin = p.Hsrc << up, Win = p.Wsrc << up;
   const int HWout = p.Hout * p.Wout;
+  int grp = 0;
+  if (p.ngroups > 1) {
+    const int t128 = (tile_m * BM) / 128;
+    grp = (t128 >= p.mt_end[0]) + (t128 >= p.mt_end[1]) + (t128 >= p.mt_end[2]);
+  }
+  int sp_py = 0, sp_px = 0;
+  if (p.upsample & 2) {
+    const int ph = p.ngroups > 1 ? grp : (p.upsample >> 2) & 3;
+    sp_py = ph >> 1; sp_px = ph & 1;
+  }
 
   constexpr unsigned OOB = 0xFFFFFF00u;
   int iy0[XI], ix0[XI], nb[XI];
@@ -145,8 +157,8 @@
         const int rem = m - n * HWout;
         oy = rem / p.Wout; ox = rem - oy * p.Wout;
       }
-      iy0[i] = oy * p.stride - p.pad;
-      ix0[i] = ox * p.stride - p.pad;
+      iy0[i] = oy * p.stride - p.pad + sp_py;
+      ix0[i] = ox * p.stride - p.pad + sp_px;
       if (p.x_nmod) n -= (n / p.x_nmod) * p.x_nmod;
       nb[i] = n * p.Hsrc * p.Wsrc;
     }
@@ -165,15 +177,10 @@
       }
       unsigned mk = ((vy & 1) ? vx : 0u) | ((vy & 2) ? vx << 3 : 0u) | ((vy & 4) ? vx << 6 : 0u);
       mk |= ay > -(1 << 19) ? 1u << 9 : 0u;
-      mk |= (unsigned)(ay & p.upsample) << 10 | (unsigned)(ax & p.upsample) << 11;
+      mk |= (unsigned)(ay & up) << 10 | (unsigned)(ax & up) << 11;
       tmask[i] = mk;
-      pix0[i] = nb[i] + (ay >> p.upsample) * p.Wsrc + (ax >> p.upsample);
-    }
-  }
-  int grp = 0;
-  if (p.ngroups > 1) {
-    const int t128 = (tile_m * BM) / 128;
-    grp = (t128 >= p.mt_end[0]) + (t128 >= p.mt_end[1]) + (t128 >= p.mt_end[2]);
+      pix0[i] = nb[i] + (ay >> up) * p.Wsrc + (ax >> up);
+    }
   }
   const void* wsel = p.ngroups > 1 ? p.w_g[grp] : p.w;
   const float* bsel = p.ngroups > 1 ? p.bias_g[grp] : p.bias;
@@ -216,7 +223,7 @@
   const void* xbase = p.x;
   int xrec = 0, soff_x = 0, seg_left = 0;
   const int ks_tail = (KK * Ctot) / BKT;
-  const int pk_ksize = p.ksize, pk_pad = p.pad, pk_up = p.upsample, pk_wsrc = p.Wsrc;
+  const int pk_ksize = p.ksize, pk_pad = p.pad, pk_up = up, pk_wsrc = p.Wsrc;
 #define row_offsets(tp, cs, chan) \
   row_offsets_fn<XI>(voff, iy0, ix0, nb, (tp), (cs), (chan), pk_ksize, KK, pk_pad, Hin, Win, pk_up, pk_wsrc)
   auto issue_tile = [&](int ks, int stage) __attribute__((always_inline)) {
@@ -586,6 +593,18 @@
     if (vec_store) {
       const int CH = BNo / 8;
       const float inv_ch = __builtin_amdgcn_rcpf((float)CH);
+      int sp_phase = -1, sp_n0 = 0;
+      {
+        typedef const __attribute__((address_space(4))) es_gemm_desc* kdesc_t;
+        kdesc_t q = (kdesc_t)__builtin_amdgcn_kernarg_segment_ptr();
+        asm volatile("" : "+s"(q));
+        const int ups = q->upsample;
+        if (ups & 2) {
+          const int t128 = (tile_m * BM) / 128;
+          sp_phase = q->ngroups > 1 ? (t128 >= q->mt_end[0]) + (t128 >= q->mt_end[1]) + (t128 >= q->mt_end[2]) : (ups >> 2) & 3;
+          sp_n0 = sp_phase * q->x_nmod;
+        }
+      }
       auto store_rows = [&](auto mode_c) __attribute__((always_inline)) {
         constexpr int MODE = decltype(mode_c)::value;
 #pragma unroll
@@ -595,7 +614,15 @@
           const int m = tile_m * BM + row, c = c_tile + ch * 8;
           if (idx < BM * CH && m < M && c < Cstore) {
             auto v = as_vec8<T>(*(const u32x4*)(et + row * EROW + ch * 16));
-            const size_t o = (size_t)m * Cstore + c;
+            size_t o = (size_t)m * Cstore + c;
+            if (sp_phase >= 0) {
+              const int nn = small_m ? fast_div(m, HWout, inv_hw) : m / HWout;
+              const int rem = m - nn * HWout;
+              const int sy = small_m ? fast_div(rem, p.Wout, inv_w) : rem / p.Wout;
+              const int sx = rem - sy * p.Wout;
+              const int orow = ((nn - sp_n0) * 2 * p.Hout + 2 * sy + (sp_phase >> 1)) * 2 * p.Wout + 2 * sx + (sp_phase & 1);
+              o = (size_t)orow * Cstore + c;
+            }
             if constexpr (MODE >= 2) {
               const auto rv = as_vec8<T>(rpre[k]);
               typename Traits<T>::vec8 lv, lo;
@@ -714,7 +741,15 @@
     x = to_f32(from_f32<T>(x * scale));
     v[r] = x + rv[r];
   }
-  T* o = (T*)p.out + (size_t)m * p.Cout + c0;
+  size_t orow = (size_t)m;
+  if (p.upsample & 2) {
+    int ph = (p.upsample >> 2) & 3;
+    if (p.ngroups > 1) { const int tm = m >> 7; ph = (tm >= p.mt_end[0]) + (tm >= p.mt_end[1]) + (tm >= p.mt_end[2]); }
+    const int rem = m - n * (p.Hout * p.Wout);
+    const int sy = div_any(rem, p.Wout, 1.0f / (float)p.Wout, small), sx = rem - sy * p.Wout;
+    orow = (size_t)(((n - ph * p.x_nmod) * 2 * p.Hout + 2 * sy + (ph >> 1)) * 2 * p.Wout + 2 * sx + (ph & 1));
+  }
+  T* o = (T*)p.out + orow * p.Cout + c0;
   if (full && p.out_lo) {
     typename Traits<T>::vec8 pk, lo;
     if (p.residual_lo) {
@@ -927,13 +962,18 @@
 
 int launch_in_chunks(const es_gemm_desc& d0, hipStream_t st, const char** why, bool dry) {
   const long long hw = (long long)d0.Hout * d0.Wout;
-  const unsigned long long per = sample_bytes(d0);
+  const bool subpix = (d0.upsample & 2) != 0;
+  unsigned long long per = sample_bytes(d0);
+  if (subpix) {
+    const unsigned long long src = (unsigned long long)d0.Hsrc * d0.Wsrc * d0.C1 * 2;
+    per = per * 4 > src ? per * 4 : src;
+  }
   if (d0.gn_part) { *why = "es_conv_gemm: a launch larger than 2 GiB per operand cannot hand GroupNorm statistics over (gn_part)"; return -1; }
-  if (d0.x_nmod && (unsigned long long)d0.x_nmod * d0.Hsrc * d0.Wsrc * d0.C1 * 2 >= ES_OPERAND_LIMIT) { *why = "es_conv_gemm: source larger than 2 GiB (32-bit buffer offsets)"; return -1; }
+  if (!subpix && d0.x_nmod && (unsigned long long)d0.x_nmod * d0.Hsrc * d0.Wsrc * d0.C1 * 2 >= ES_OPERAND_LIMIT) { *why = "es_conv_gemm: source larger than 2 GiB (32-bit buffer offsets)"; return -1; }
   long long ns = (long long)((ES_OPERAND_LIMIT - 1) / (per ? per : 1));
   if (d0.splitk > 1) { const long long cap = ((1ll << 31) - 1) / (hw * (d0.rows_padded / 8)); ns = ns < cap ? ns : cap; }
   if (hw == 1 && ns >= 256) ns -= ns % 256;
-  if (d0.x_nmod) ns -= ns % d0.x_nmod;
+  if (d0.x_nmod && !subpix) ns -= ns % d0.x_nmod;
   if (ns < 1) { *why = "es_conv_gemm: one sample's operands exceed 2 GiB (32-bit buffer offsets)"; return -1; }
   const int ng = d0.ngroups > 1 ? d0.ngroups : 1;
   const long long cs = d0.act == ES_ACT_GEGLU ? d0.Cout / 2 : d0.Cout;
@@ -957,6 +997,16 @@
       for (int k = 0; k < 4; ++k) s.mt_end[k] = 0x7FFFFFFF;
       auto adv = [](const void* p, long long bytes) -> const void* { return p ? (const void*)((const char*)p + bytes) : nullptr; };
       const long long src_px = n0 * d0.Hsrc * d0.Wsrc, out_px = n0 * hw;
+      if (subpix) {
+        s.x_nmod = 0;
+        s.upsample = 2 | (g << 2);
+        s.x = adv(d0.x, (n0 - g0) * d0.Hsrc * d0.Wsrc * d0.C1 * 2);
+        s.out = (void*)adv(d0.out, (n0 - g0) * hw * 4 * cs * 2);
+        if (dry) continue;
+        const int rc = s.dtype == ES_F16 ? launch<f16>(s, st) : launch<bf16>(s, st);
+        if (rc) { *why = "es_conv_gemm: launch failed"; return rc; }
+        continue;
+      }
       if (!d0.x_nmod) s.x = adv(d0.x, src_px * d0.C1 * 2);
       s.x2 = adv(d0.x2, src_px * d0.C2 * 2);
       s.t1 = adv(d0.t1, out_px * d0.Ct1 * 2);
@@ -990,7 +1040,40 @@
   return (size_t)d->splitk * d->N * d->Hout * d->Wout * d->rows_padded * sizeof(float);
 }
 
-extern "C" int es_conv_gemm(const es_gemm_desc* d, void* stream) {
+static const char* subpixel_expand(const es_gemm_desc& d, es_gemm_desc* e) {
+  if (d.x2 || d.C2 || d.t1 || d.t2 || d.Ct1 || d.Ct2 || d.temb || d.residual || d.residual_lo || d.out_lo || d.act != ES_ACT_NONE ||
+      d.gn_part || d.ln_colsum || d.ngroups > 1 || d.x_nmod || d.korder || d.out_scale_dev)
+    return "es_conv_gemm: the sub-pixel form (upsample = 2) is bias only: no x2, tail sources, temb, residual, out_lo, activation, gn_part, ln_colsum, weight groups, x_nmod or korder";
+  if (d.ksize != 3 || d.stride != 1 || d.pad != 1 || d.N < 1 || d.Hsrc < 1 || d.Wsrc < 1 || d.Hout != 2 * d.Hsrc || d.Wout != 2 * d.Wsrc)
+    return "es_conv_gemm: the sub-pixel form (upsample = 2) needs ksize 3, stride 1, pad 1 and a 2 Hsrc x 2 Wsrc output";
+  if (d.C1 < BK || d.C1 % BK || (d.Cout & 7) || d.Cout < 1 || d.bn == 256 || d.Kpad != 4 * d.C1 || !d.w)
+    return "es_conv_gemm: the sub-pixel form (upsample = 2) needs C1 % 64 == 0, Cout % 8 == 0, Kpad = 4 C1 (four packed phases) and no 256-wide tile";
+  const long long Mp = (long long)d.N * d.Hsrc * d.Wsrc;
+  if (Mp % 128 || Mp * 4 >= (1ll << 31)) return "es_conv_gemm: the sub-pixel form (upsample = 2) needs N * Hsrc * Wsrc in whole 128-pixel tiles";
+  *e = d;
+  e->x_nmod = d.N; e->N = 4 * d.N; e->Hout = d.Hsrc; e->Wout = d.Wsrc; e->ksize = 2; e->pad = 1; e->upsample = 2;
+  if (e->bn == 320) { e->bn = 160; e->stages = 2; }
+  e->ngroups = 4;
+  for (int g = 0; g < 4; ++g) {
+    e->mt_end[g] = (int)((g + 1) * (Mp / 128));
+    e->w_g[g] = (const char*)d.w + (size_t)g * d.rows_padded * d.Kpad * 2;
+    e->bias_g[g] = d.bias;
+    e->ln_colsum_g[g] = nullptr;
+  }
+  e->w = e->w_g[0];
+  return nullptr;
+}
+
+extern "C" int es_conv_gemm(const es_gemm_desc* d_in, void* stream) {
+  es_gemm_desc sub_e;
+  const es_gemm_desc* d = d_in;
+  if (d_in->upsample != 0 && d_in->upsample != 1 && d_in->upsample != 2) { es_set_error("es_conv_gemm: upsample must be 0, 1 (nearest-2x, direct) or 2 (nearest-2x, sub-pixel form)"); return -1; }
+  if (d_in->upsample == 2) {
+    if (!d_in->x || !d_in->out) { es_set_error("es_conv_gemm: null pointer"); return -1; }
+    const char* why = subpixel_expand(*d_in, &sub_e);
+    if (why) { es_set_error(why); return -1; }
+    d = &sub_e;
+  }
   const int Ctot = d->C1 + d->C2;
   const int Ktrue = d->ksize * d->ksize * Ctot + (d->t1 ? d->Ct1 + d->Ct2 : 0);
   if (!d->x || !d->out || (d->ngroups <= 1 && !d->w)) { es_set_error("es_conv_gemm: null pointer"); return -1; }
@@ -1022,7 +1105,7 @@
     const char* why = nullptr;
     if (launch_in_chunks(*d, nullptr, &why, true)) { es_set_error(why); return -1; }
   }
-  if (d->ksize != 1 && d->ksize != 3) { es_set_error("es_conv_gemm: ksize must be 1 or 3"); return -1; }
+  if (d->ksize != 1 && d->ksize != 3 && !(d->ksize == 2 && d->upsample == 2)) { es_set_error("es_conv_gemm: ksize must be 1 or 3"); return -1; }
   if (d->t1 && (d->stride != 1 || d->upsample || d->C1 % BK || d->C2 % BK || d->Ct1 % BK || d->Ct2 % BK || d->Ct1 < BK ||
                 (d->Ct2 && !d->t2) || d->ln_colsum || d->Hout != d->Hsrc || d->Wout != d->Wsrc ||
                 false)) {
@@ -1054,7 +1137,7 @@
   if (d->waves == 8 && (d->bn == 320 || d->C1 % BK || d->C2 % BK || d->stages == 3 ||
                         (d->stages == 4 && d->bn != 128))) {
     es_set_error("es_conv_gemm: waves=8 is the 128-pixel tile on 8 waves: 64-aligned channels, 2 stages (4 with bn=128)"); return -1; }
-  ES_PLAN_RECORD(ES_OP_CONV_GEMM, d, sizeof(*d));
+  ES_PLAN_RECORD(ES_OP_CONV_GEMM, d_in, sizeof(*d_in));
   hipStream_t st = (hipStream_t)stream;
   es_gemm_desc dd = *d;
   for (int g = dd.ngroups > 1 ? dd.ngroups : 0; g < 4; ++g) dd.mt_end[g] = 0x7FFFFFFF;
diff --git a/edgestyle_amd/engine.py b/edgestyle_amd/engine.py
--- a/edgestyle_amd/engine.py
+++ b/edgestyle_amd/engine.py
@@ -42,6 +42,13 @@
         pw = ops.pack_weight(self.t(p + ".weight"), None if b is None else b.to(self.device), self.dtype,
                              self.device, geglu=geglu, cin_pad=cin_pad, cout_pad=cout_pad)
         _PACK_CACHE[key] = (weakref.ref(w), None if b is None else weakref.ref(b), pw)
+        return pw
+
+    def conv_up(self, p: str) -> ops.PackedWeight:
+        pw = self.conv(p)
+        if pw.sub is None and pw.ksize == 3 and pw.cin % 64 == 0 and pw.cout % 8 == 0 and not pw.korder \
+                and self.sd[p + ".weight"].shape[1] == pw.cin:
+            pw.sub = ops.pack_weight_subpixel(self.t(p + ".weight"), None, self.dtype, self.device, bias_packed=pw.bias)
         return pw
 
     def conv_tail(self, p: str, pt: str) -> ops.PackedWeight:
@@ -237,7 +244,7 @@
                 a = Transformer(pk, f"up_blocks.{i}.attentions.{j}", heads, g) if cfg.up_has_attn[i] else None
                 blk.append((r, a))
             self.up.append(blk)
-            self.upsample.append(pk.conv(f"up_blocks.{i}.upsamplers.0.conv") if i != n - 1 else None)
+            self.upsample.append(pk.conv_up(f"up_blocks.{i}.upsamplers.0.conv") if i != n - 1 else None)
         self.norm_out = pk.norm("conv_norm_out")
         self.conv_out = pk.conv("conv_out")
         del self.pk
@@ -269,7 +276,7 @@
                 if a is not None:
                     h = a(h, ctx[ci]); ci += 1
             if self.upsample[i] is not None:
-                h = ops.conv_gemm(h, self.upsample[i], upsample=True)
+                h = ops.conv_gemm(h, self.upsample[i], upsample=True, subpixel="auto")
         h = ops.group_norm(h, self.norm_out[0], self.norm_out[1], cfg.norm_num_groups, cfg.norm_eps, True)
         return ops.conv_gemm(h, self.conv_out, out=out)
 
@@ -376,7 +383,7 @@
             for i in range(n):
                 rs = [Resnet(pk, f"decoder.up_blocks.{i}.resnets.{j}", g, eps, None)
                       for j in range(cfg.layers_per_block + 1)]
-                us = pk.conv(f"decoder.up_blocks.{i}.upsamplers.0.conv") if i != n - 1 else None
+                us = pk.conv_up(f"decoder.up_blocks.{i}.upsamplers.0.conv") if i != n - 1 else None
                 self.d_up.append((rs, us))
             self.d_norm = pk.norm("decoder.conv_norm_out")
             self.d_out = pk.conv("decoder.conv_out")
@@ -413,7 +420,7 @@
             for r in rs:
                 h = r(h, None)
             if us is not None:
-                h = ops.conv_gemm(h, us, upsample=True)
+                h = ops.conv_gemm(h, us, upsample=True, subpixel="auto")
         h = ops.group_norm(h, self.d_norm[0], self.d_norm[1], cfg.norm_num_groups, cfg.norm_eps, True)
         return ops.conv_gemm(h, self.d_out)
 
diff --git a/edgestyle_amd/lib.py b/edgestyle_amd/lib.py
--- a/edgestyle_amd/lib.py
+++ b/edgestyle_amd/lib.py
@@ -202,6 +202,8 @@
     "es_load_weights": (C.c_int, [C.POINTER(Weights), C.POINTER(ModelConfig), C.POINTER(CtxGeometry), _I, C.POINTER(_P)]),
     "es_plan_gemm_choice": (C.c_int, [C.c_longlong, _I, _I, _I, C.POINTER(C.c_int), _I, _I, C.POINTER(C.c_int), C.POINTER(C.c_int),
                                       C.POINTER(C.c_int)]),
+    "es_plan_upsample_choice": (C.c_int, [C.c_longlong, _I, _I, _I, C.POINTER(C.c_int), _I, C.POINTER(C.c_int), C.POINTER(C.c_int),
+                                          C.POINTER(C.c_int), C.POINTER(C.c_int)]),
     "es_linear_xs_eligible": (C.c_int, [C.c_longlong, _I, _I, _I, _I, _I, _I]),
     "es_conv_gemm8p_form_ok": (C.c_int, [_I, _I, _I, C.c_longlong, _I]),
     "es_ctx_graph_hazard": (C.c_int, []),
diff --git a/edgestyle_amd/ops.py b/edgestyle_amd/ops.py
--- a/edgestyle_amd/ops.py
+++ b/edgestyle_amd/ops.py
@@ -99,10 +99,12 @@
     ln_eps: float = 1e-5
     ctail: int = 0
     korder: int = 0
+    phases: int = 1
+    sub: Optional["PackedWeight"] = None
 
     @property
     def rows_padded(self):
-        return self.w.shape[0]
+        return self.w.shape[0] // self.phases
 
     @property
     def kpad(self):
@@ -161,6 +163,81 @@
         bp = torch.zeros(rows, dtype=torch.float32, device=device)
         bp[:cout] = b
     return PackedWeight(wp, bp, cout_eff, cp, k, bn, geglu, korder=korder)
+
+
+def fold_subpixel(weight: torch.Tensor) -> torch.Tensor:
+    w = weight.double()
+    cout, cin = w.shape[:2]
+    out = torch.zeros(4, cout, cin, 2, 2, dtype=torch.float64, device=w.device)
+    for py in (0, 1):
+        for px in (0, 1):
+            for ky in range(3):
+                ty = (py + ky + 1) // 2 - py
+                for kx in range(3):
+                    tx = (px + kx + 1) // 2 - px
+                    out[2 * py + px, :, :, ty, tx] += w[:, :, ky, kx]
+    return out
+
+
+def pack_weight_subpixel(weight: torch.Tensor, bias: Optional[torch.Tensor], dtype, device,
+                         bias_packed: Optional[torch.Tensor] = None) -> PackedWeight:
+    weight = weight.to(device=device, dtype=torch.float32)
+    cout, cin, k, _ = weight.shape
+    if k != 3 or cin % BK:
+        raise L.EdgeStyleHipError("pack_weight_subpixel: a 3x3 convolution over a multiple of 64 input channels")
+    f = fold_subpixel(weight).permute(0, 1, 3, 4, 2).reshape(4, cout, 4 * cin)
+    bn = choose_bn(cout)
+    rows = (cout + bn - 1) // bn * bn
+    wp = torch.zeros(4, rows, 4 * cin, dtype=dtype, device=device)
+    wp[:, :cout] = f.float().to(dtype)
+    bp = bias_packed
+    if bp is None and bias is not None:
+        bp = torch.zeros(rows, dtype=torch.float32, device=device)
+        bp[:cout] = bias.to(device=device, dtype=torch.float32)
+    return PackedWeight(wp.reshape(4 * rows, 4 * cin), bp, cout, cin, 3, bn, False, phases=4)
+
+
+def plan_upsample(M: int, pw: "PackedWeight", bns) -> tuple:
+    arr = (C.c_int * len(bns))(*[int(b) for b in bns])
+    sub, bn, sk, st = C.c_int(), C.c_int(), C.c_int(), C.c_int()
+    if L.load().es_plan_upsample_choice(int(M), int(pw.rows_padded), int(pw.cin), int(pw.cout), arr, len(bns),
+                                        C.byref(sub), C.byref(bn), C.byref(sk), C.byref(st)) != 0:
+        raise L.EdgeStyleHipError(f"plan_upsample: rows_padded {pw.rows_padded} fits no N tile")
+    stages = st.value
+    if stages == 4 and not (DEEP_RING and LANE == 0):
+        stages = 2
+    return bool(sub.value), bn.value, sk.value, stages
+
+
+def _conv_gemm_subpixel(x: torch.Tensor, q: PackedWeight, out: torch.Tensor, bn: int, splitk: int, stages: int) -> torch.Tensor:
+    N, H, W, C1 = x.shape
+    M = N * 4 * H * W
+    d = L.GemmDesc()
+    d.x, d.w, d.out = x.data_ptr(), q.w.data_ptr(), out.data_ptr()
+    d.bias = q.bias.data_ptr() if q.bias is not None else None
+    d.N, d.Hsrc, d.Wsrc, d.C1, d.C2 = N, H, W, C1, 0
+    d.Hout, d.Wout, d.Cout = 2 * H, 2 * W, q.cout
+    d.rows_padded, d.Kpad = q.rows_padded, q.kpad
+    d.ksize, d.stride, d.pad, d.upsample = 3, 1, 1, 2
+    d.act, d.splitk, d.bn, d.dtype, d.out_scale = L.ACT_NONE, splitk, bn, _dt(x), 1.0
+    d.stages = stages or FORCE_STAGES
+    if FORCE_WAVES:
+        d.waves = FORCE_WAVES
+    if splitk > 1:
+        d.workspace = _get_workspace(splitk * M * q.rows_padded * 4, x.device).data_ptr()
+    if PROFILE is not None:
+        d.prof = PROFILE.next((2.0 * M * q.cout * 9 * C1, 3, (M, q.cout, 9 * C1, 1, splitk, bn),
+                               dict(N=N, H=H, W=W, C1=C1, C2=0, cout=q.cout, k=3, stride=1, pad=1, upsample=True, geglu=False,
+                                    splitk=splitk, Hout=2 * H, Wout=2 * W, residual=False, temb=False, bn=bn, stages=int(d.stages),
+                                    group_n=None, ctail=0, subpixel=True,
+                                    algorithmic_bytes=int(x.numel() * x.element_size() + q.rows_padded * 9 * C1 * 2
+                                                          + out.numel() * out.element_size()))))
+        dd = L.GemmDesc()
+        C.memmove(C.byref(dd), C.byref(d), C.sizeof(L.GemmDesc))
+        dd.prof = None
+        PROFILE.descs.append(dd)
+    L.check(L.load().es_conv_gemm(C.byref(d), _stream()), "es_conv_gemm")
+    return out
 
 
 def pack_weight_tail(weight: torch.Tensor, tail_weight: torch.Tensor, bias: Optional[torch.Tensor], dtype, device) -> PackedWeight:
@@ -310,6 +387,44 @@
     return bn, sk, stages
 
 
+PLAN_SUBPIX_MARGIN = 0.9
+
+
+def plan_cost_reference(M: int, rows_padded: int, kpad: int, bn: int, sk: int) -> float:
+    nk = kpad // BK
+    bm = {320: 256, 64: 64}.get(bn, BM)
+    resident = {320: PLAN_RESIDENT // 2, 64: 2 * PLAN_RESIDENT}.get(bn, PLAN_RESIDENT)
+    wgs = ((M + bm - 1) // bm) * (rows_padded // bn) * sk
+    if bn == 320:
+        tk = PLAN_T320
+    elif bn == 64:
+        w = wgs / (PLAN_RESIDENT // 2)
+        tk = (PLAN_T64_ALONE + PLAN_T64 * max(0.0, w - 1.0) ** 2) * (1.0 if nk <= 40 else PLAN_T64_LONG)
+    else:
+        tk = (PLAN_T160 if bn == 160 else 1.0) * (PLAN_ALONE if wgs <= PLAN_RESIDENT // 2 else 1.0)
+    rounds = max(wgs / 256.0, 0.9) if bn == 320 else float(-(-wgs // resident))
+    t = rounds * ((nk / sk) * tk + (PLAN_T320_FIX if bn == 320 else PLAN_TFIX))
+    if sk > 1:
+        t += PLAN_RED_FIX + sk * M * rows_padded * 8.0 / PLAN_SLAB_BYTES_PER_UNIT
+    return t
+
+
+def plan_upsample_reference(M: int, rows_padded: int, cin: int, cout: int, bns) -> tuple:
+    kd = (9 * cin + BK - 1) // BK * BK
+    dbn, dsk, dst = plan_gemm_reference(M, rows_padded, kd, False, bns)
+    if M <= 0 or M % 512 or cin < BK or cin % BK or cout % 8:
+        return False, dbn, dsk, dst
+    sb = tuple(b for b in bns if b not in (320, 256))
+    try:
+        sbn, ssk, sst = plan_gemm_reference(M, rows_padded, 4 * cin, False, sb)
+    except L.EdgeStyleHipError:
+        return False, dbn, dsk, dst
+    ts = plan_cost_reference(M, rows_padded, 4 * cin, sbn, ssk)
+    if ts < PLAN_SUBPIX_MARGIN * plan_cost_reference(M, rows_padded, kd, dbn, dsk):
+        return True, sbn, ssk, sst
+    return False, dbn, dsk, dst
+
+
 def choose_launch_bn(M: int, pw: "PackedWeight") -> int:
     return plan_gemm(M, pw.rows_padded, pw.kpad, pw.geglu)[0]
 
@@ -457,7 +572,7 @@
               out_hw=None, splitk: Optional[int] = None, stages: int = 0,
               group_n: Optional[Sequence[int]] = None, tail: Optional[Sequence[torch.Tensor]] = None,
               x_rep: int = 1, wide: bool = False, out_lo: Optional[torch.Tensor] = None, gn_groups: int = 0,
-              gn_part: Optional[torch.Tensor] = None):
+              gn_part: Optional[torch.Tensor] = None, subpixel=False):
     pws = None
     if isinstance(pw, (list, tuple)):
         pws = list(pw)
@@ -507,6 +622,20 @@
         and not (pw.geglu and residual is not None) and not wide and gn_groups == 0 and FORCE_WAVES != 8 \
         and (group_n is None or all((n * Hout * Wout) % 256 == 0 for n in group_n))
     cand = ((256,) if ln256_ok else ()) + ((320,) if big_ok else ()) + (160, 128) + ((64,) if small_ok else ())
+    if subpixel:
+        if not upsample or pw.sub is None:
+            raise L.EdgeStyleHipError("conv_gemm: subpixel needs upsample=True and weights with a sub-pixel pack (pack_weight_subpixel)")
+        plain = (pws is None and k == 3 and stride == 1 and pad == 1 and x2 is None and temb is None and residual is None and not tails
+                 and x_rep == 1 and act == L.ACT_NONE and out_scale == 1.0 and out_scale_dev is None and out_hw is None and gn_groups == 0)
+        if subpixel is True:
+            if not plain:
+                raise L.EdgeStyleHipError("conv_gemm: the sub-pixel form is bias only (no second source, temb, residual, tail, activation, scale)")
+            sbn, ssk, sst = plan_gemm(M, pw.sub.rows_padded, pw.sub.kpad, bns=tuple(b for b in cand if b not in (320, 256)) if FORCE_BN == 0 else (FORCE_BN,))
+            return _conv_gemm_subpixel(x, pw.sub, out, sbn, ssk if splitk is None else splitk, stages or sst)
+        if plain and splitk is None and FORCE_BN == 0 and not _PLAN_TUNING:
+            sub, sbn, ssk, sst = plan_upsample(M, pw, cand)
+            if sub:
+                return _conv_gemm_subpixel(x, pw.sub, out, sbn, ssk, stages or sst)
     bn, auto_splitk, auto_stages = plan_gemm(M, pw.rows_padded, pw.kpad, pw.geglu,
                                              bns=cand if FORCE_BN == 0 else (FORCE_BN,), allow_split=pw.ln_colsum is None)
     if bn == 320 and FORCE_BN == 0 and (auto_splitk if splitk is None else splitk) == 1 and not L.load().es_conv_gemm8p_form_ok(
diff --git a/include/edgestyle_hip.h b/include/edgestyle_hip.h
--- a/include/edgestyle_hip.h
+++ b/include/edgestyle_hip.h
@@ -263,6 +263,8 @@
 int es_plan_gemm_choice(long long M, int rows_padded, int kpad, int geglu, const int* bns, int n_bns, int allow_split,
                         int* bn, int* splitk, int* stages);
 int es_linear_xs_eligible(long long M, int ksize, int kpad, int cin, int ctail, int cout, int geglu);
+int es_plan_upsample_choice(long long M, int rows_padded, int cin, int cout, const int* bns, int n_bns, int* subpixel,
+                            int* bn, int* splitk, int* stages);
 int es_conv_gemm8p_form_ok(int act, int cout, int has_temb, long long out_hw, int has_residual);
 int es_ctx_graph_hazard(void);
 int es_plan_set_dry(int on);
```

New measurement: 2.239 images/s, median of 6. About the same (+0.4%).
